# oval-group/GNN_branching

Measured on NVIDIA B200. Metric: gnn_subdomains_scored_per_sec, higher is better.
Workload: dtype fp16x3 (fp32 accumulate)

## Files before the change

gnn_branching_b200/csrc/gnnb_api.cu:

```cuda
#include <math.h>
#include <stdio.h>
#include <stdlib.h>
#include <string.h>

#include <map>
#include <string>
#include <vector>

#include "gnnb_common.cuh"
#include "gnnb_train.cuh"

using namespace gnnb;

struct gnnb_ctx {
    int device = 0;
    int last_status = 0;
    std::string err;
    int64_t launches = 0;
    int math = GNNB_MATH_TC_FP16X3;
    int chunk = 0;
    int snapshot = 0;
    int fuse = 1;
    int rescore = 0;
    int64_t rescored = 0;
    bool have_gnn = false;
    float* d_gnn = nullptr;
    uint16_t* d_tc = nullptr;
    GnnParams gp{};
    float* d_train = nullptr;
    int64_t n_params = 0;
    size_t po_w[N_LIN] = {0}, po_b[N_LIN] = {0};
    int adam_steps = 0;
    float* train_ws = nullptr;
    size_t train_ws_cap = 0;
    float* kw_ws = nullptr;
    size_t kw_ws_cap = 0;
    int32_t* kw_iscratch = nullptr;
    int kw_iscratch_cap = 0;
    bool have_net = false;
    float* d_net = nullptr;
    std::vector<LayerDev> layers;
    std::vector<PropPlan*> plan_fwd, plan_bwd;
    std::vector<PropPlan*> plan_kw_own;
    std::vector<PropPlan*> plan_kw;
    std::vector<int> n;
    int zero_tap_layer = 0;
    std::vector<LayerTiling> tiling;
    std::vector<RowMap> rowmap;
    int32_t* d_maps = nullptr;
    LayerDev* d_layers = nullptr;
    int32_t* d_hidden_off = nullptr;
    int32_t* d_random_order = nullptr;
    const float** d_ptrs = nullptr;
    std::vector<int> hidden_off;
    int n_hidden = 0;
    std::vector<struct gnnb_queue*> queues;
    int ws_cap = 0;
    bool ws_host_staging = false;
    float* d_ws = nullptr;
    std::vector<float*> mu, relax_f, relax_b;
    std::vector<int32_t*> amb_cnt, amb_base, amb_rows;
    float* nb = nullptr;
    float* ws_scores = nullptr;
    float* ws_best = nullptr;
    int32_t* ws_idx = nullptr;
    struct Staging {
        std::vector<float*> inputs;
        float* mask = nullptr;
        float* best = nullptr;
        int32_t* idx = nullptr;
        float* scores = nullptr;
    } stg[2];
    float* res_best = nullptr;
    int32_t* res_idx = nullptr;
    int64_t res_cap = 0;
    cudaStream_t copy_stream = nullptr;
    cudaEvent_t ev_copied[2] = {nullptr, nullptr}, ev_free[2] = {nullptr, nullptr};
    unsigned long long* d_nan = nullptr;
    int32_t* d_resc = nullptr;
    int resc_cap = 0;
    RowGather* d_gather = nullptr;
    size_t gather_cap = 0;
    std::map<std::string, std::pair<float*, int64_t>> snaps;
    int profile = 0;
    struct Pending { int klass; int64_t rows; cudaEvent_t a, b; };
    std::vector<Pending> pending;
    std::vector<cudaEvent_t> ev_pool;
    double prof_ms[GNNB_K_COUNT] = {0};
    int64_t prof_launches[GNNB_K_COUNT] = {0};
    int64_t prof_rows[GNNB_K_COUNT] = {0};
};

struct gnnb_queue {
    gnnb_ctx* ctx;
    DomainQueue* q;
};

namespace {

int fail(gnnb_ctx* c, int status, const std::string& msg) {
    if (c) { c->last_status = status; c->err = msg; }
    return status;
}

int axis_taps(int i, int ksize, int stride, int pad, int n_out) {
    int t = 0;
    for (int k = 0; k < ksize; ++k) {
        const int a = i + pad - k;
        if (a >= 0 && a % stride == 0 && a / stride < n_out) ++t;
    }
    return t;
}

int first_zero_tap_layer(const std::vector<LayerDev>& layers) {
    for (size_t k = 1; k < layers.size(); ++k) {
        const LayerDev& L = layers[k];
        if (L.kind != GNNB_LAYER_CONV) continue;
        for (int y = 0; y < L.h_in; ++y)
            if (axis_taps(y, L.ksize, L.stride, L.pad, L.h_out) == 0) return (int)k + 1;
        for (int x = 0; x < L.w_in; ++x)
            if (axis_taps(x, L.ksize, L.stride, L.pad, L.w_out) == 0) return (int)k + 1;
    }
    return 0;
}

int check_zero_taps(gnnb_ctx* c) {
    if (!c->zero_tap_layer) return GNNB_OK;
    return fail(c, GNNB_ERR_UNSUPPORTED, "layer " + std::to_string(c->zero_tap_layer) +
                " (conv, stride > kernel) has input positions no tap reaches: the GNN's tap-count normalisation divides by zero");
}

template <class F>
void walk_inputs(const gnnb_frontier& fr, GnnInputs& in, const std::vector<int>& n, F f) {
    const int L = (int)n.size() - 2;
    auto at = [](const float* const* table, int k) { return table ? table[k] : nullptr; };
    for (int k = 0; k <= L + 1; ++k) {
        f(at(fr.lb, k), in.lb[k], (int64_t)n[k]);
        f(at(fr.ub, k), in.ub[k], (int64_t)n[k]);
    }
    for (int k = 0; k < L; ++k) {
        f(at(fr.dual, k), in.dual[k], (int64_t)n[k + 1] * 3);
        f(at(fr.prim_pre, k), in.pre[k], (int64_t)n[k + 1]);
        f(at(fr.prim_post, k), in.post[k], (int64_t)n[k + 1]);
    }
    f(fr.prim_out, in.pout, (int64_t)1);
    f(fr.primal_input, in.pin, (int64_t)n[0]);
    f(fr.wp, in.wp, (int64_t)n[L]);
    f(fr.bp, in.bp, (int64_t)1);
}

int frontier_inputs(gnnb_ctx* ctx, const gnnb_frontier* fr, bool mask, GnnInputs* out) {
    bool ok = !mask || fr->mask;
    walk_inputs(*fr, *out, ctx->n, [&](const float* src, const float*& slot, int64_t) { slot = src; ok = ok && src; });
    return ok ? GNNB_OK : fail(ctx, GNNB_ERR_INVALID, "null frontier array");
}

#define CU(call)                                                                                          \
    do {                                                                                                  \
        cudaError_t e__ = (call);                                                                         \
        if (e__ != cudaSuccess)                                                                           \
            return fail(ctx, GNNB_ERR_CUDA, std::string(#call) + ": " + cudaGetErrorString(e__));         \
    } while (0)

size_t align4(size_t x) { return (x + 3) & ~size_t(3); }

void free_workspace(gnnb_ctx* c) {
    if (c->d_ws) cudaFree(c->d_ws);
    c->d_ws = nullptr;
    c->ws_cap = 0;
    for (auto& kv : c->snaps) cudaFree(kv.second.first);
    c->snaps.clear();
}

int ensure_workspace(gnnb_ctx* ctx, int Bc, bool host_staging) {
    if (ctx->d_ws && ctx->ws_cap >= Bc && (ctx->ws_host_staging || !host_staging)) return GNNB_OK;
    free_workspace(ctx);
    const int L = (int)ctx->layers.size();
    int nmax = 0;
    for (int k = 0; k <= L; ++k) nmax = ctx->n[k] > nmax ? ctx->n[k] : nmax;
    size_t total = 0;
    auto take = [&](size_t elems) { size_t off = total; total += (elems + 63) & ~size_t(63); return off; };
    std::vector<size_t> o_mu(L + 2), o_rf(L + 1), o_rb(L + 1), o_lb(L + 2), o_ub(L + 2), o_du(L), o_pr(L), o_po(L);
    auto wrows = [&](int k) { return (size_t)Bc * (k <= L ? (size_t)ctx->rowmap[k].nslots : 128); };
    for (int k = 0; k <= L + 1; ++k) o_mu[k] = take(wrows(k) * P);
    for (int k = 1; k <= L; ++k) { o_rf[k] = take(wrows(k) * P); o_rb[k] = take(wrows(k) * P); }
    std::vector<size_t> o_ac(L + 1), o_ab(L + 1), o_ar(L + 1);
    for (int k = 1; k <= L; ++k) {
        const size_t rows = wrows(k), nt = rows / 128;
        o_ac[k] = take(nt + 1); o_ab[k] = take(nt + 1); o_ar[k] = take(rows);
    }
    size_t nb_rows = 0;
    for (int k = 0; k <= L; ++k) nb_rows = wrows(k) > nb_rows ? wrows(k) : nb_rows;
    const size_t o_nb = take(nb_rows * P);
    const size_t o_sc = take((size_t)Bc * ctx->n_hidden);
    const size_t o_best = take(Bc), o_idx = take(Bc);
    struct StgOff { std::vector<size_t> inputs; size_t mask, best, idx, sc; } so[2];
    if (host_staging) {
        GnnInputs unused(L);
        for (StgOff& o : so) {
            walk_inputs(gnnb_frontier{}, unused, ctx->n, [&](const float*, const float*&, int64_t per) {
                o.inputs.push_back(take((size_t)Bc * per));
            });
            o.mask = take((size_t)Bc * ctx->n_hidden);
            o.best = take((size_t)Bc * GNNB_TOPK_MAX); o.idx = take((size_t)Bc * GNNB_TOPK_MAX);
            o.sc = take((size_t)Bc * ctx->n_hidden);
        }
    }
    CU(cudaMalloc(&ctx->d_ws, total * sizeof(float)));
    float* base = ctx->d_ws;
    ctx->mu.assign(L + 2, nullptr); ctx->relax_f.assign(L + 1, nullptr); ctx->relax_b.assign(L + 1, nullptr);
    for (int k = 0; k <= L + 1; ++k) ctx->mu[k] = base + o_mu[k];
    for (int k = 1; k <= L; ++k) { ctx->relax_f[k] = base + o_rf[k]; ctx->relax_b[k] = base + o_rb[k]; }
    ctx->amb_cnt.assign(L + 1, nullptr); ctx->amb_base.assign(L + 1, nullptr); ctx->amb_rows.assign(L + 1, nullptr);
    for (int k = 1; k <= L; ++k) {
        ctx->amb_cnt[k] = reinterpret_cast<int32_t*>(base + o_ac[k]);
        ctx->amb_base[k] = reinterpret_cast<int32_t*>(base + o_ab[k]);
        ctx->amb_rows[k] = reinterpret_cast<int32_t*>(base + o_ar[k]);
    }
    ctx->nb = base + o_nb; ctx->ws_scores = base + o_sc; ctx->ws_best = base + o_best;
    ctx->ws_idx = reinterpret_cast<int32_t*>(base + o_idx);
    if (host_staging) {
        for (int i = 0; i < 2; ++i) {
            gnnb_ctx::Staging& g = ctx->stg[i];
            const StgOff& o = so[i];
            g.inputs.clear();
            for (size_t off : o.inputs) g.inputs.push_back(base + off);
            g.mask = base + o.mask;
            g.best = base + o.best; g.idx = reinterpret_cast<int32_t*>(base + o.idx); g.scores = base + o.sc;
        }
        if (!ctx->copy_stream) {
            CU(cudaStreamCreateWithFlags(&ctx->copy_stream, cudaStreamNonBlocking));
            for (int i = 0; i < 2; ++i) {
                CU(cudaEventCreateWithFlags(&ctx->ev_copied[i], cudaEventDisableTiming));
                CU(cudaEventCreateWithFlags(&ctx->ev_free[i], cudaEventDisableTiming));
            }
        }
    }
    ctx->ws_cap = Bc;
    ctx->ws_host_staging = host_staging;
    return GNNB_OK;
}

#define TRY_(expr) do { int s__ = (expr); if (s__ != GNNB_OK) return s__; } while (0)

int snap(gnnb_ctx* ctx, bool on, const std::string& name, const float* src, int64_t numel, cudaStream_t st) {
    if (!on) return GNNB_OK;
    auto it = ctx->snaps.find(name);
    if (it == ctx->snaps.end() || it->second.second < numel) {
        if (it != ctx->snaps.end()) cudaFree(it->second.first);
        float* p = nullptr;
        CU(cudaMalloc(&p, (size_t)numel * sizeof(float)));
        ctx->snaps[name] = std::make_pair(p, numel);
        it = ctx->snaps.find(name);
    }
    it->second.second = numel;
    CU(cudaMemcpyAsync(it->second.first, src, (size_t)numel * sizeof(float), cudaMemcpyDeviceToDevice, st));
    return GNNB_OK;
}

cudaEvent_t prof_event(gnnb_ctx* ctx) {
    if (!ctx->ev_pool.empty()) { cudaEvent_t e = ctx->ev_pool.back(); ctx->ev_pool.pop_back(); return e; }
    cudaEvent_t e = nullptr;
    cudaEventCreate(&e);
    return e;
}

struct ProfScope {
    gnnb_ctx* ctx; cudaStream_t st; cudaEvent_t a = nullptr, b = nullptr; int klass; int64_t rows;
    ProfScope(gnnb_ctx* c, int k, int64_t r, cudaStream_t s) : ctx(c), st(s), klass(k), rows(r) {
        if (ctx->profile) { a = prof_event(ctx); b = prof_event(ctx); cudaEventRecord(a, st); }
    }
    ~ProfScope() {
        if (ctx->profile) { cudaEventRecord(b, st); ctx->pending.push_back({klass, rows, a, b}); }
    }
};

int prof_collect(gnnb_ctx* ctx) {
    if (ctx->pending.empty()) return GNNB_OK;
    CU(cudaDeviceSynchronize());
    for (auto& p : ctx->pending) {
        float ms = 0.f;
        if (cudaEventElapsedTime(&ms, p.a, p.b) == cudaSuccess) {
            ctx->prof_ms[p.klass] += ms;
            ctx->prof_launches[p.klass] += 1;
            ctx->prof_rows[p.klass] += p.rows;
        }
        ctx->ev_pool.push_back(p.a);
        ctx->ev_pool.push_back(p.b);
    }
    ctx->pending.clear();
    return GNNB_OK;
}

int snap_img(gnnb_ctx* ctx, bool on, const std::string& name, const float* img, int k, int Bc, bool piece_major, cudaStream_t st) {
    if (!on) return GNNB_OK;
    const int64_t numel = (int64_t)Bc * ctx->n[k] * P;
    if (ctx->math != GNNB_MATH_TC_FP16X3) return snap(ctx, on, name, img, numel, st);
    TRY_(snap(ctx, on, name, img, numel, st));
    tc_unpack_tile_image(img, ctx->snaps[name].first, ctx->rowmap[k], (int64_t)Bc * ctx->rowmap[k].nslots, piece_major, st);
    return GNNB_OK;
}

#define TRY(expr) do { int s__ = (expr); if (s__ != GNNB_OK) return s__; } while (0)

int run_chunk(gnnb_ctx* ctx, const GnnInputs& in, const float* mask, int Bc, int math, const NanDoms& nd, float* scores, int k,
              float* best_score, int32_t* best_idx, gnnb_winner* winners, cudaStream_t st) {
    const int L = (int)ctx->layers.size();
    const GnnParams& g = ctx->gp;
    const bool tc = math == GNNB_MATH_TC_FP16X3;
    const bool snaps = ctx->snapshot && math == ctx->math;
    int64_t* lc = &ctx->launches;
    auto name = [](const char* fmt, int a, int b) { char buf[64]; snprintf(buf, sizeof buf, fmt, a, b); return std::string(buf); };

    auto R = [&](int k) { return (int64_t)Bc * (tc ? ctx->rowmap[k].nslots : ctx->n[k]); };
    const RowMap nomap{nullptr, 0, 0};
    auto M = [&](int k) { return tc ? ctx->rowmap[k] : nomap; };
    const bool fused = tc && ctx->fuse;

    const bool amb_all = tc && L <= AMB_MAX_LAYERS;
    if (amb_all) {
        ProfScope ps(ctx, GNNB_K_RELAX, 0, st);
        AmbLayers al{};
        al.n = L;
        for (int k = 1; k <= L; ++k) {
            al.lb[k - 1] = in.lb[k]; al.ub[k - 1] = in.ub[k]; al.map[k - 1] = M(k); al.rows[k - 1] = R(k);
            al.cnt[k - 1] = ctx->amb_cnt[k]; al.base[k - 1] = ctx->amb_base[k]; al.out_rows[k - 1] = ctx->amb_rows[k];
        }
        amb_compact_all(al, st, lc);
    }
    {
        std::vector<NodeInputs> nis(L + 1);
        for (int k = 1; k <= L; ++k)
            nis[k] = NodeInputs{in.lb[k], in.ub[k], in.dual[k - 1], in.pre[k - 1], in.post[k - 1], ctx->layers[k - 1].bias_node,
                                ctx->n[k], R(k), ctx->amb_rows[k], ctx->amb_base[k], M(k)};
        if (tc) {
            for (int k0 = 1; k0 <= L; k0 += AMB_MAX_LAYERS) {
                const int nl = (L - k0 + 1) < AMB_MAX_LAYERS ? (L - k0 + 1) : AMB_MAX_LAYERS;
                int64_t nodes = 0;
                for (int k = k0; k < k0 + nl; ++k) {
                    nodes += (int64_t)Bc * ctx->n[k];
                    if (!amb_all) amb_compact(in.lb[k], in.ub[k], M(k), nis[k].rows, ctx->amb_cnt[k], ctx->amb_base[k], ctx->amb_rows[k], st, lc);
                }
                ProfScope ps(ctx, GNNB_K_RELAX, nodes, st);
                tc_relax(g, &nis[k0], &ctx->relax_f[k0], &ctx->relax_b[k0], nl, st, lc);
            }
        }
        for (int k = 1; k <= L; ++k) {
            if (!tc) {
                ProfScope ps(ctx, GNNB_K_RELAX, (int64_t)Bc * ctx->n[k], st);
                simt_relax(g, nis[k], ctx->relax_f[k], ctx->relax_b[k], st, lc);
            }
            TRY(snap(ctx, snaps, name(tc ? "relaxp_f%d" : "relax_f%d", k, 0), ctx->relax_f[k], (int64_t)Bc * ctx->n[k] * P, st));
            TRY(snap(ctx, snaps, name(tc ? "relaxp_b%d" : "relax_b%d", k, 0), ctx->relax_b[k], (int64_t)Bc * ctx->n[k] * P, st));
        }
    }
    {
        ProfScope ps(ctx, GNNB_K_INPUT_EMBED, (int64_t)Bc * ctx->n[0], st);
        if (tc) tc_input_embed(g, in.lb[0], in.pin, in.ub[0], ctx->mu[0], M(0), R(0), st, lc);
        else simt_input_embed(g, in.lb[0], in.pin, in.ub[0], ctx->mu[0], R(0), st, lc);
    }
    TRY(snap_img(ctx, snaps, "mu0_embed", ctx->mu[0], 0, Bc, false, st));

    for (int t = 0; t < g.T; ++t) {
        const bool last = (t == g.T - 1);
        for (int k = 1; k <= L; ++k) {
            const int64_t rows = R(k), nodes = (int64_t)Bc * ctx->n[k];
            if (fused) {
                ProfScope ps(ctx, GNNB_K_LAYER_FWD, nodes, st);
                tc_fused(g, ctx->plan_fwd[k - 1], ctx->mu[k - 1], false, in.lb[k], in.ub[k], ctx->relax_f[k], ctx->amb_base[k],
                         ctx->mu[k], nullptr, M(k), 0, 0, rows, ctx->d_nan, nd, ctx->snapshot ? ctx->nb : nullptr, false, st, lc);
            } else {
                ProfScope ps(ctx, GNNB_K_PROP_FWD, nodes, st);
                if (tc) prop_tc_run(ctx->plan_fwd[k - 1], ctx->mu[k - 1], ctx->nb, Bc, st, lc);
                else prop_forward(ctx->layers[k - 1], ctx->mu[k - 1], ctx->nb, Bc, st, lc);
            }
            TRY(snap_img(ctx, snaps, name("t%d_fwd_nb%d", t, k), ctx->nb, k, Bc, true, st));
            if (!fused) {
                ProfScope ps(ctx, GNNB_K_UPDATE_FWD, nodes, st);
                if (tc) tc_update(g, false, in.lb[k], in.ub[k], ctx->nb, ctx->relax_f[k], ctx->amb_base[k], ctx->mu[k], nullptr, M(k), 0, 0, rows, ctx->d_nan, nd, st, lc);
                else simt_update(g, false, in.lb[k], in.ub[k], ctx->nb, ctx->relax_f[k], ctx->mu[k], nullptr, ctx->n[k], 0, 0, rows, ctx->d_nan, st, lc);
            }
            TRY(snap_img(ctx, snaps, name("t%d_fwd_mu%d", t, k), ctx->mu[k], k, Bc, false, st));
        }
        {
            ProfScope ps(ctx, GNNB_K_OUTPUT, Bc, st);
            output_node(g, in.wp, in.bp, ctx->mu[L], tc, tc ? ctx->rowmap[L].nslots : ctx->n[L], in.lb[L + 1], in.ub[L + 1], in.pout,
                        ctx->mu[L + 1], ctx->n[L], Bc, st, lc);
        }
        TRY(snap(ctx, snaps, name("t%d_mu_out", t, 0), ctx->mu[L + 1], (int64_t)Bc * P, st));
        for (int k = L; k >= 1; --k) {
            const int64_t rows = R(k), nodes = (int64_t)Bc * ctx->n[k];
            float* sc = last ? scores : nullptr;
            float* mu_k = (last && k == 1 && tc && !ctx->snapshot) ? nullptr : ctx->mu[k];
            const bool fused_k = fused && k < L;
            if (fused_k) {
                ProfScope ps(ctx, last ? GNNB_K_LAYER_BWD_SCORE : GNNB_K_LAYER_BWD, nodes, st);
                tc_fused(g, ctx->plan_bwd[k], ctx->mu[k + 1], true, in.lb[k], in.ub[k], ctx->relax_b[k], ctx->amb_base[k],
                         mu_k, sc, M(k), ctx->n_hidden, ctx->hidden_off[k], rows, ctx->d_nan, nd, ctx->snapshot ? ctx->nb : nullptr, false, st, lc);
            } else {
                ProfScope ps(ctx, GNNB_K_PROP_BWD, nodes, st);
                if (k == L && tc) prop_tc_property_backward(in.wp, ctx->mu[L + 1], ctx->nb, ctx->n[L], ctx->rowmap[L].nslots, Bc, st, lc);
                else if (k == L) prop_property_backward(in.wp, ctx->mu[L + 1], ctx->nb, ctx->n[L], Bc, st, lc);
                else if (tc) prop_tc_run(ctx->plan_bwd[k], ctx->mu[k + 1], ctx->nb, Bc, st, lc);
                else prop_backward(ctx->layers[k], ctx->mu[k + 1], ctx->nb, Bc, true, st, lc);
            }
            TRY(snap_img(ctx, snaps, name("t%d_bwd_nb%d", t, k), ctx->nb, k, Bc, true, st));
            if (!fused_k) {
                ProfScope ps(ctx, last ? GNNB_K_UPDATE_BWD_SCORE : GNNB_K_UPDATE_BWD, nodes, st);
                if (tc) tc_update(g, true, in.lb[k], in.ub[k], ctx->nb, ctx->relax_b[k], ctx->amb_base[k], mu_k, sc, M(k), ctx->n_hidden, ctx->hidden_off[k], rows, ctx->d_nan, nd, st, lc);
                else simt_update(g, true, in.lb[k], in.ub[k], ctx->nb, ctx->relax_b[k], ctx->mu[k], sc, ctx->n[k], ctx->n_hidden, ctx->hidden_off[k], rows, ctx->d_nan, st, lc);
            }
            TRY(snap_img(ctx, snaps, name("t%d_bwd_mu%d", t, k), ctx->mu[k], k, Bc, false, st));
        }
        if (!last && fused) {
            ProfScope ps(ctx, GNNB_K_INPUT_UPDATE, (int64_t)Bc * ctx->n[0], st);
            tc_fused(g, ctx->plan_bwd[0], ctx->mu[1], true, in.lb[0], in.ub[0], nullptr, nullptr, ctx->mu[0], nullptr, M(0), 0, 0, R(0),
                     ctx->d_nan, nd, nullptr, true, st, lc);
            TRY(snap_img(ctx, snaps, name("t%d_mu0", t, 0), ctx->mu[0], 0, Bc, false, st));
        } else if (!last) {
            {
                ProfScope ps(ctx, GNNB_K_PROP_BWD, (int64_t)Bc * ctx->n[0], st);
                if (tc) prop_tc_run(ctx->plan_bwd[0], ctx->mu[1], ctx->nb, Bc, st, lc);
                else prop_backward(ctx->layers[0], ctx->mu[1], ctx->nb, Bc, false, st, lc);
            }
            {
                ProfScope ps(ctx, GNNB_K_INPUT_UPDATE, (int64_t)Bc * ctx->n[0], st);
                if (tc) tc_input_update(g, in.lb[0], in.ub[0], ctx->nb, ctx->mu[0], M(0), R(0), st, lc);
                else simt_input_update(g, in.lb[0], in.ub[0], ctx->nb, ctx->mu[0], R(0), st, lc);
            }
            TRY(snap_img(ctx, snaps, name("t%d_mu0", t, 0), ctx->mu[0], 0, Bc, false, st));
        }
    }
    {
        ProfScope ps(ctx, GNNB_K_ARGMAX, Bc, st);
        if (k == 1) masked_argmax(scores, mask, ctx->n_hidden, Bc, best_score, best_idx, winners, st, lc);
        else masked_topk(scores, mask, ctx->n_hidden, Bc, k, best_score, best_idx, st, lc);
    }
    CU(cudaGetLastError());
    return GNNB_OK;
}

int ensure_nan_doms(gnnb_ctx* ctx, int B) {
    if (ctx->resc_cap >= B) return GNNB_OK;
    if (ctx->d_resc) { cudaFree(ctx->d_resc); ctx->d_resc = nullptr; ctx->resc_cap = 0; }
    CU(cudaMalloc(&ctx->d_resc, (1 + 2 * (size_t)B) * sizeof(int32_t)));
    CU(cudaMemset(ctx->d_resc, 0, (1 + 2 * (size_t)B) * sizeof(int32_t)));
    ctx->resc_cap = B;
    return GNNB_OK;
}

int ensure_kw_iscratch(gnnb_ctx* ctx, int B, cudaStream_t st) {
    if (ctx->kw_iscratch_cap >= B) return GNNB_OK;
    if (ctx->kw_iscratch) { CU(cudaStreamSynchronize(st)); cudaFree(ctx->kw_iscratch); ctx->kw_iscratch = nullptr; ctx->kw_iscratch_cap = 0; }
    CU(cudaMalloc(&ctx->kw_iscratch, (3 * (size_t)B + 1) * sizeof(int32_t)));
    ctx->kw_iscratch_cap = B;
    return GNNB_OK;
}

NanDoms nan_doms(gnnb_ctx* ctx) { return NanDoms{ctx->d_resc, ctx->d_resc + 1, ctx->d_resc + 1 + ctx->resc_cap, 0}; }

void reset_nan_doms(gnnb_ctx* ctx, cudaStream_t st) {
    cudaStreamSynchronize(st);
    cudaMemset(ctx->d_resc, 0, (1 + 2 * (size_t)ctx->resc_cap) * sizeof(int32_t));
}

int rescore_flagged(gnnb_ctx* ctx, const gnnb_frontier* in, int chunk, int k, float* best, int32_t* idx, gnnb_winner* winners,
                    float* scores, cudaStream_t st) {
    const bool host = in->mem == GNNB_MEM_HOST;
    const int nh = ctx->n_hidden;
    const NanDoms nd = nan_doms(ctx);
    int32_t count = 0;
    CU(cudaMemcpyAsync(&count, nd.count, sizeof count, cudaMemcpyDeviceToHost, st));
    CU(cudaStreamSynchronize(st));
    ctx->rescored = count;
    if (count == 0) return GNNB_OK;
    std::vector<int32_t> rows;
    if (host) {
        rows.resize(count);
        CU(cudaMemcpyAsync(rows.data(), nd.list, (size_t)count * sizeof(int32_t), cudaMemcpyDeviceToHost, st));
        CU(cudaStreamSynchronize(st));
    }
    CU(cudaMemsetAsync(nd.count, 0, sizeof(int32_t), st));
    CU(cudaMemsetAsync(ctx->d_nan, 0, sizeof(unsigned long long), st));
    gnnb_ctx::Staging& sg = ctx->stg[0];
    std::vector<RowGather> tab;
    GnnInputs cp((int)ctx->layers.size());
    walk_inputs(*in, cp, ctx->n, [&](const float* src, const float*& slot, int64_t per) {
        float* dst = sg.inputs[tab.size()];
        tab.push_back(RowGather{src, dst, per});
        slot = dst;
    });
    tab.push_back(RowGather{in->mask, sg.mask, nh});
    if (!host) {
        if (ctx->gather_cap < tab.size()) {
            if (ctx->d_gather) cudaFree(ctx->d_gather);
            ctx->d_gather = nullptr; ctx->gather_cap = 0;
            CU(cudaMalloc(&ctx->d_gather, tab.size() * sizeof(RowGather)));
            ctx->gather_cap = tab.size();
        }
        CU(cudaMemcpyAsync(ctx->d_gather, tab.data(), tab.size() * sizeof(RowGather), cudaMemcpyHostToDevice, st));
    }
    for (int s0 = 0, Bs = 0; s0 < count; s0 += Bs) {
        Bs = (count - s0) < chunk ? (count - s0) : chunk;
        if (host) {
            for (int i = 0; i < Bs; ++i)
                for (const RowGather& t : tab)
                    CU(cudaMemcpyAsync(t.dst + i * t.per, t.src + rows[s0 + i] * t.per, t.per * sizeof(float), cudaMemcpyHostToDevice, st));
        } else {
            gather_rows(ctx->d_gather, (int)tab.size(), nd.list + s0, Bs, st, &ctx->launches);
        }
        TRY(run_chunk(ctx, cp, sg.mask, Bs, GNNB_MATH_SIMT_FP32, NanDoms{nullptr, nullptr, nullptr, 0}, sg.scores, k, sg.best, sg.idx, nullptr, st));
        scatter_rescored(nd.list + s0, Bs, k, sg.best, sg.idx, sg.scores, nh, best, idx, winners, host ? nullptr : scores, nd.flag, st,
                         &ctx->launches);
        if (host && scores)
            for (int i = 0; i < Bs; ++i)
                CU(cudaMemcpyAsync(scores + (size_t)rows[s0 + i] * nh, sg.scores + (size_t)i * nh, (size_t)nh * sizeof(float),
                                   cudaMemcpyDeviceToHost, st));
    }
    CU(cudaEventRecord(ctx->ev_free[0], st));
    CU(cudaGetLastError());
    return GNNB_OK;
}

int upload_gnn(gnnb_ctx* ctx, const float* const* tensors, int T) {
    std::vector<size_t> o_w(N_LIN), o_b(N_LIN);
    size_t total = 0;
    for (int l = 0; l < N_LIN; ++l) {
        o_w[l] = total; total += align4((size_t)lin_in(l) * lin_out(l));
        o_b[l] = total; total += align4(lin_out(l));
    }
    std::vector<float> blob(total, 0.f);
    for (int l = 0; l < N_LIN; ++l) {
        const int K = lin_in(l), N = lin_out(l);
        const float* W = tensors[2 * l];
        for (int nn = 0; nn < N; ++nn)
            for (int k = 0; k < K; ++k) blob[o_w[l] + (size_t)k * N + nn] = W[(size_t)nn * K + k];
        memcpy(&blob[o_b[l]], tensors[2 * l + 1], sizeof(float) * N);
    }
    std::vector<float> cw((size_t)N_TCLIN * P * P, 0.f), cb((size_t)N_TCLIN * P, 0.f);
    auto compose = [&](int id, int outer, int half, int inner, bool add_outer_bias) {
        const float* Wo = tensors[2 * outer];
        const float* bo = tensors[2 * outer + 1];
        const int Ko = lin_in(outer);
        for (int nn = 0; nn < P; ++nn) {
            double bacc = add_outer_bias ? (double)bo[nn] : 0.0;
            for (int k = 0; k < P; ++k) {
                double acc = 0.0;
                if (inner < 0) acc = Wo[(size_t)nn * Ko + half * P + k];
                else
                    for (int j = 0; j < P; ++j) acc += (double)Wo[(size_t)nn * Ko + half * P + j] * (double)tensors[2 * inner][(size_t)j * P + k];
                cw[((size_t)id * P + nn) * P + k] = (float)acc;
            }
            if (inner >= 0)
                for (int j = 0; j < P; ++j) bacc += (double)Wo[(size_t)nn * Ko + half * P + j] * (double)tensors[2 * inner + 1][j];
            cb[(size_t)id * P + nn] = (float)bacc;
        }
    };
    compose(T_FWD_R, FC4, 0, FC1_1, false);
    compose(T_FWD_C, FC4, 1, FC3_2, true);
    compose(T_BWD_R, BC4, 0, BC2_1, false);
    compose(T_BWD_C, BC4, 1, BC3_1, true);
    compose(T_INP_C, INP_B2, 0, INP_B_1, true);
    compose(T_INP_NB, INP_B2, 1, -1, false);
    std::vector<size_t> o_tc(N_LIN, 0);
    size_t tc_total = 0;
    for (int l = 0; l < N_LIN; ++l)
        if (lin_in(l) >= P && lin_out(l) == P) { o_tc[l] = tc_total; tc_total += (size_t)tc_packed_elems(lin_in(l)); }
    std::vector<size_t> o_tcx(N_TCLIN, 0);
    for (int i = 0; i < N_TCLIN; ++i) { o_tcx[i] = tc_total; tc_total += (size_t)tc_packed_elems(P); }
    std::vector<uint16_t> tcblob(tc_total ? tc_total : 1, 0);
    for (int l = 0; l < N_LIN; ++l)
        if (lin_in(l) >= P && lin_out(l) == P) tc_pack_weight(tensors[2 * l], lin_in(l), &tcblob[o_tc[l]]);
    for (int i = 0; i < N_TCLIN; ++i) tc_pack_weight(&cw[(size_t)i * P * P], P, &tcblob[o_tcx[i]]);
    const size_t o_cb = total;
    total += cb.size();
    blob.resize(total, 0.f);
    memcpy(&blob[o_cb], cb.data(), cb.size() * sizeof(float));
    CU(cudaDeviceSynchronize());
    if (!ctx->d_gnn) CU(cudaMalloc(&ctx->d_gnn, total * sizeof(float)));
    if (!ctx->d_tc) CU(cudaMalloc(&ctx->d_tc, tcblob.size() * sizeof(uint16_t)));
    CU(cudaMemcpy(ctx->d_gnn, blob.data(), total * sizeof(float), cudaMemcpyHostToDevice));
    CU(cudaMemcpy(ctx->d_tc, tcblob.data(), tcblob.size() * sizeof(uint16_t), cudaMemcpyHostToDevice));
    for (int l = 0; l < N_LIN; ++l) {
        ctx->gp.wt[l] = ctx->d_gnn + o_w[l];
        ctx->gp.bias[l] = ctx->d_gnn + o_b[l];
        ctx->gp.tc[l] = (lin_in(l) >= P && lin_out(l) == P) ? ctx->d_tc + o_tc[l] : nullptr;
    }
    for (int i = 0; i < N_TCLIN; ++i) {
        ctx->gp.tcx_w[i] = ctx->d_tc + o_tcx[i];
        ctx->gp.tcx_b[i] = ctx->d_gnn + o_cb + (size_t)i * P;
    }
    ctx->gp.T = T;
    if (!ctx->d_train) {
        size_t np = 0;
        for (int l = 0; l < N_LIN; ++l) {
            ctx->po_w[l] = np; np += align4((size_t)lin_in(l) * lin_out(l));
            ctx->po_b[l] = np; np += align4(lin_out(l));
        }
        ctx->n_params = (int64_t)np;
        CU(cudaMalloc(&ctx->d_train, 4 * np * sizeof(float)));
        CU(cudaMemset(ctx->d_train, 0, 4 * np * sizeof(float)));
        ctx->adam_steps = 0;
    }
    {
        std::vector<float> master((size_t)ctx->n_params, 0.f);
        for (int l = 0; l < N_LIN; ++l) {
            memcpy(&master[ctx->po_w[l]], tensors[2 * l], sizeof(float) * lin_in(l) * lin_out(l));
            memcpy(&master[ctx->po_b[l]], tensors[2 * l + 1], sizeof(float) * lin_out(l));
        }
        CU(cudaMemcpy(ctx->d_train, master.data(), master.size() * sizeof(float), cudaMemcpyHostToDevice));
    }
    ctx->have_gnn = true;
    return GNNB_OK;
}

TrainParams train_params(gnnb_ctx* ctx) {
    TrainParams tp;
    float* grad = ctx->d_train + ctx->n_params;
    for (int l = 0; l < N_LIN; ++l) {
        tp.w[l] = ctx->d_train + ctx->po_w[l]; tp.b[l] = ctx->d_train + ctx->po_b[l];
        tp.dw[l] = grad + ctx->po_w[l]; tp.db[l] = grad + ctx->po_b[l];
    }
    return tp;
}

int download_quarter(gnnb_ctx* ctx, int quarter, float* const* tensors, const int64_t* numels, int n_tensors) {
    if (!ctx || !tensors || !numels) return fail(ctx, GNNB_ERR_INVALID, "null argument");
    if (!ctx->have_gnn) return fail(ctx, GNNB_ERR_STATE, "gnnb_set_gnn_weights must be called first");
    if (n_tensors != 2 * N_LIN) return fail(ctx, GNNB_ERR_INVALID, "expected 52 tensors (weight, bias of 26 linears)");
    for (int l = 0; l < N_LIN; ++l)
        if (numels[2 * l] != (int64_t)lin_in(l) * lin_out(l) || numels[2 * l + 1] != lin_out(l))
            return fail(ctx, GNNB_ERR_INVALID, "tensor " + std::to_string(2 * l) + " has the wrong number of elements");
    CU(cudaSetDevice(ctx->device));
    CU(cudaDeviceSynchronize());
    std::vector<float> host((size_t)ctx->n_params);
    CU(cudaMemcpy(host.data(), ctx->d_train + (size_t)quarter * ctx->n_params, host.size() * sizeof(float), cudaMemcpyDeviceToHost));
    for (int l = 0; l < N_LIN; ++l) {
        memcpy(tensors[2 * l], &host[ctx->po_w[l]], sizeof(float) * lin_in(l) * lin_out(l));
        memcpy(tensors[2 * l + 1], &host[ctx->po_b[l]], sizeof(float) * lin_out(l));
    }
    return GNNB_OK;
}

}

extern "C" {

int gnnb_abi_version(void) { return 1; }

int gnnb_create(gnnb_ctx** out, int device) {
    if (!out) return GNNB_ERR_INVALID;
    *out = nullptr;
    gnnb_ctx* ctx = new gnnb_ctx();
    ctx->device = device;
    cudaError_t e = cudaSetDevice(device);
    if (e != cudaSuccess) { delete ctx; return GNNB_ERR_CUDA; }
    cudaDeviceProp prop;
    e = cudaGetDeviceProperties(&prop, device);
    if (e != cudaSuccess) { delete ctx; return GNNB_ERR_CUDA; }
    if (prop.major != 10) {
        fprintf(stderr, "libgnnb: device %d is sm_%d%d; this library is built for sm_100a (B200) only\n", device, prop.major, prop.minor);
        delete ctx;
        return GNNB_ERR_UNSUPPORTED;
    }
    if (cudaMalloc(&ctx->d_nan, sizeof(unsigned long long)) != cudaSuccess ||
        cudaMemset(ctx->d_nan, 0, sizeof(unsigned long long)) != cudaSuccess ||
        simt_init() != 0 || prop_init(64 * 1024) != 0 || tc_init() != 0 || prop_tc_init() != 0 || kw_init() != 0 || train_init() != 0) {
        fprintf(stderr, "libgnnb: initialisation failed: %s\n", cudaGetErrorString(cudaGetLastError()));
        if (ctx->d_nan) cudaFree(ctx->d_nan);
        delete ctx;
        return GNNB_ERR_CUDA;
    }
    *out = ctx;
    return GNNB_OK;
}

void gnnb_destroy(gnnb_ctx* ctx) {
    if (!ctx) return;
    cudaSetDevice(ctx->device);
    free_workspace(ctx);
    if (ctx->d_gnn) cudaFree(ctx->d_gnn);
    if (ctx->d_tc) cudaFree(ctx->d_tc);
    if (ctx->d_train) cudaFree(ctx->d_train);
    if (ctx->train_ws) cudaFree(ctx->train_ws);
    if (ctx->kw_ws) cudaFree(ctx->kw_ws);
    if (ctx->kw_iscratch) cudaFree(ctx->kw_iscratch);
    if (ctx->d_net) cudaFree(ctx->d_net);
    if (ctx->d_maps) cudaFree(ctx->d_maps);
    if (ctx->d_layers) cudaFree(ctx->d_layers);
    if (ctx->d_hidden_off) cudaFree(ctx->d_hidden_off);
    if (ctx->d_random_order) cudaFree(ctx->d_random_order);
    if (ctx->d_ptrs) cudaFree(ctx->d_ptrs);
    if (ctx->d_nan) cudaFree(ctx->d_nan);
    if (ctx->d_resc) cudaFree(ctx->d_resc);
    if (ctx->d_gather) cudaFree(ctx->d_gather);
    for (PropPlan* p : ctx->plan_fwd) prop_plan_free(p);
    for (PropPlan* p : ctx->plan_bwd) prop_plan_free(p);
    for (PropPlan* p : ctx->plan_kw_own) prop_plan_free(p);
    if (ctx->copy_stream) cudaStreamDestroy(ctx->copy_stream);
    if (ctx->res_best) cudaFree(ctx->res_best);
    if (ctx->res_idx) cudaFree(ctx->res_idx);
    for (int i = 0; i < 2; ++i) { if (ctx->ev_copied[i]) cudaEventDestroy(ctx->ev_copied[i]); if (ctx->ev_free[i]) cudaEventDestroy(ctx->ev_free[i]); }
    for (auto& p : ctx->pending) { cudaEventDestroy(p.a); cudaEventDestroy(p.b); }
    for (auto e : ctx->ev_pool) cudaEventDestroy(e);
    for (gnnb_queue* q : ctx->queues) q->ctx = nullptr;
    delete ctx;
}

int gnnb_set_gnn_weights(gnnb_ctx* ctx, const float* const* tensors, const int64_t* numels, int n_tensors, int T, int p) {
    if (!ctx || !tensors || !numels) return fail(ctx, GNNB_ERR_INVALID, "null argument");
    if (p != P) return fail(ctx, GNNB_ERR_UNSUPPORTED, "embedding size p must be 64");
    if (T < 1) return fail(ctx, GNNB_ERR_INVALID, "T must be >= 1");
    if (n_tensors != 2 * N_LIN) return fail(ctx, GNNB_ERR_INVALID, "expected 52 tensors (weight, bias of 26 linears)");
    for (int l = 0; l < N_LIN; ++l) {
        if (numels[2 * l] != (int64_t)lin_in(l) * lin_out(l) || numels[2 * l + 1] != lin_out(l))
            return fail(ctx, GNNB_ERR_INVALID, "tensor " + std::to_string(2 * l) + " has the wrong number of elements");
    }
    CU(cudaSetDevice(ctx->device));
    return upload_gnn(ctx, tensors, T);
}

int gnnb_set_network(gnnb_ctx* ctx, const gnnb_layer_desc* layers, int n_layers, int c0, int h0, int w0) {
    if (!ctx || !layers || n_layers < 1) return fail(ctx, GNNB_ERR_INVALID, "null argument");
    if (!ctx->queues.empty()) return fail(ctx, GNNB_ERR_STATE, "gnnb_set_network while domain queues of the previous network exist");
    CU(cudaSetDevice(ctx->device));
    std::vector<LayerDev> devs(n_layers);
    std::vector<int> n(n_layers + 2);
    n[0] = c0 * h0 * w0;
    int pc = c0, ph = h0, pw = w0;
    bool flat = false;
    size_t total = 0;
    std::vector<size_t> o_w(n_layers), o_b(n_layers);
    for (int k = 0; k < n_layers; ++k) {
        const gnnb_layer_desc& d = layers[k];
        LayerDev& L = devs[k];
        L.kind = d.kind;
        L.c_in = d.c_in; L.h_in = d.h_in; L.w_in = d.w_in; L.c_out = d.c_out; L.h_out = d.h_out; L.w_out = d.w_out;
        L.ksize = d.ksize; L.stride = d.stride; L.pad = d.pad;
        L.n_in = d.c_in * d.h_in * d.w_in;
        L.n_out = d.c_out * d.h_out * d.w_out;
        if (!d.weight || !d.bias) return fail(ctx, GNNB_ERR_INVALID, "layer weight/bias is null");
        if (L.n_in != n[k]) return fail(ctx, GNNB_ERR_INVALID, "layer " + std::to_string(k) + ": input size does not match the previous layer");
        size_t wn;
        if (d.kind == GNNB_LAYER_CONV) {
            if (flat || d.c_in != pc || d.h_in != ph || d.w_in != pw) return fail(ctx, GNNB_ERR_INVALID, "conv layer input shape mismatch");
            if (d.ksize < 1 || d.stride < 1 || d.pad < 0) return fail(ctx, GNNB_ERR_INVALID, "bad conv geometry");
            if (d.h_out != (d.h_in + 2 * d.pad - d.ksize) / d.stride + 1 || d.w_out != (d.w_in + 2 * d.pad - d.ksize) / d.stride + 1)
                return fail(ctx, GNNB_ERR_INVALID, "conv output shape mismatch");
            if ((d.h_out - 1) * d.stride - 2 * d.pad + d.ksize != d.h_in || (d.w_out - 1) * d.stride - 2 * d.pad + d.ksize != d.w_in)
                return fail(ctx, GNNB_ERR_UNSUPPORTED, "conv geometry needs output_padding in the backward pass");
            if ((size_t)d.c_in * d.ksize * d.ksize * d.c_out * sizeof(float) > 64 * 1024)
                return fail(ctx, GNNB_ERR_UNSUPPORTED, "conv weights exceed the 64 KB shared-memory staging buffer");
            wn = (size_t)d.c_out * d.c_in * d.ksize * d.ksize;
            pc = d.c_out; ph = d.h_out; pw = d.w_out;
        } else if (d.kind == GNNB_LAYER_LINEAR) {
            if (d.h_in != 1 || d.w_in != 1 || d.h_out != 1 || d.w_out != 1) return fail(ctx, GNNB_ERR_INVALID, "linear layers use c_in/c_out only");
            wn = (size_t)L.n_out * L.n_in;
            flat = true;
        } else {
            return fail(ctx, GNNB_ERR_INVALID, "unknown layer kind");
        }
        n[k + 1] = L.n_out;
        o_w[k] = total; total += align4(wn);
        o_b[k] = total; total += align4(L.n_out);
    }
    n[n_layers + 1] = 1;
    std::vector<float> blob(total, 0.f);
    for (int k = 0; k < n_layers; ++k) {
        const gnnb_layer_desc& d = layers[k];
        const LayerDev& L = devs[k];
        const size_t wn = d.kind == GNNB_LAYER_CONV ? (size_t)d.c_out * d.c_in * d.ksize * d.ksize : (size_t)L.n_out * L.n_in;
        memcpy(&blob[o_w[k]], d.weight, wn * sizeof(float));
        const int per = d.kind == GNNB_LAYER_CONV ? d.h_out * d.w_out : 1;
        for (int j = 0; j < L.n_out; ++j) blob[o_b[k] + j] = d.bias[j / per];
    }
    struct Staged {
        float* d_net = nullptr;
        int32_t* d_maps = nullptr;
        LayerDev* d_layers = nullptr;
        int32_t *d_hidden_off = nullptr, *d_random_order = nullptr;
        const float** d_ptrs = nullptr;
        std::vector<PropPlan*> plan_fwd, plan_bwd, plan_kw_own;
        bool keep = false;
        ~Staged() {
            if (keep) return;
            if (d_net) cudaFree(d_net);
            if (d_maps) cudaFree(d_maps);
            if (d_layers) cudaFree(d_layers);
            if (d_hidden_off) cudaFree(d_hidden_off);
            if (d_random_order) cudaFree(d_random_order);
            if (d_ptrs) cudaFree(d_ptrs);
            for (PropPlan* p : plan_fwd) prop_plan_free(p);
            for (PropPlan* p : plan_bwd) prop_plan_free(p);
            for (PropPlan* p : plan_kw_own) prop_plan_free(p);
        }
    } sg;
    CU(cudaMalloc(&sg.d_net, total * sizeof(float)));
    CU(cudaMemcpy(sg.d_net, blob.data(), total * sizeof(float), cudaMemcpyHostToDevice));
    for (int k = 0; k < n_layers; ++k) { devs[k].weight = sg.d_net + o_w[k]; devs[k].bias_node = sg.d_net + o_b[k]; }
    sg.plan_fwd.assign(n_layers, nullptr);
    sg.plan_bwd.assign(n_layers, nullptr);
    sg.plan_kw_own.assign(n_layers, nullptr);
    std::vector<LayerTiling> tiling(n_layers + 1);
    std::vector<RowMap> rowmap(n_layers + 1, RowMap{nullptr, 0, 0});
    tiling[0] = make_tiling(c0, h0, w0);
    for (int k = 0; k < n_layers; ++k)
        tiling[k + 1] = devs[k].kind == GNNB_LAYER_CONV ? make_tiling(devs[k].c_out, devs[k].h_out, devs[k].w_out)
                                                       : make_tiling(devs[k].n_out, 1, 1);
    {
        size_t total_slots = 0;
        for (const LayerTiling& t : tiling) total_slots += t.node_of_slot.size();
        CU(cudaMalloc(&sg.d_maps, total_slots * sizeof(int32_t)));
        size_t off = 0;
        for (int k = 0; k <= n_layers; ++k) {
            const LayerTiling& t = tiling[k];
            CU(cudaMemcpy(sg.d_maps + off, t.node_of_slot.data(), t.node_of_slot.size() * sizeof(int32_t), cudaMemcpyHostToDevice));
            rowmap[k] = RowMap{sg.d_maps + off, n[k], (int)t.node_of_slot.size()};
            off += t.node_of_slot.size();
        }
    }
    for (int k = 0; k < n_layers; ++k) {
        sg.plan_fwd[k] = prop_plan_build(devs[k], layers[k].weight, false, false, tiling[k + 1], tiling[k]);
        sg.plan_bwd[k] = prop_plan_build(devs[k], layers[k].weight, true, k > 0, tiling[k], tiling[k + 1]);
        if (!sg.plan_fwd[k] || !sg.plan_bwd[k]) return fail(ctx, GNNB_ERR_CUDA, "building the propagation plans failed");
        if (k > 0 && devs[k].kind == GNNB_LAYER_CONV) {
            sg.plan_kw_own[k] = prop_plan_build(devs[k], layers[k].weight, true, false, tiling[k], tiling[k + 1]);
            if (!sg.plan_kw_own[k]) return fail(ctx, GNNB_ERR_CUDA, "building the propagation plans failed");
        }
    }
    std::vector<int> hidden_off(n_layers + 2, 0);
    int n_hidden = 0;
    for (int k = 1; k <= n_layers; ++k) { hidden_off[k] = n_hidden; n_hidden += n[k]; }
    CU(cudaMalloc(&sg.d_layers, n_layers * sizeof(LayerDev)));
    CU(cudaMemcpy(sg.d_layers, devs.data(), n_layers * sizeof(LayerDev), cudaMemcpyHostToDevice));
    CU(cudaMalloc(&sg.d_hidden_off, (n_layers + 1) * sizeof(int32_t)));
    CU(cudaMemcpy(sg.d_hidden_off, hidden_off.data() + 1, (n_layers + 1) * sizeof(int32_t), cudaMemcpyHostToDevice));
    CU(cudaMalloc(&sg.d_random_order, n_layers * sizeof(int32_t)));
    CU(cudaMalloc(&sg.d_ptrs, 2 * (n_layers + 2) * sizeof(float*)));
    CU(cudaDeviceSynchronize());
    ctx->have_net = false;
    free_workspace(ctx);
    if (ctx->d_net) cudaFree(ctx->d_net);
    if (ctx->d_maps) cudaFree(ctx->d_maps);
    if (ctx->d_layers) cudaFree(ctx->d_layers);
    if (ctx->d_hidden_off) cudaFree(ctx->d_hidden_off);
    if (ctx->d_random_order) cudaFree(ctx->d_random_order);
    if (ctx->d_ptrs) cudaFree(ctx->d_ptrs);
    for (PropPlan* p : ctx->plan_fwd) prop_plan_free(p);
    for (PropPlan* p : ctx->plan_bwd) prop_plan_free(p);
    for (PropPlan* p : ctx->plan_kw_own) prop_plan_free(p);
    sg.keep = true;
    ctx->d_net = sg.d_net; ctx->d_maps = sg.d_maps; ctx->d_layers = sg.d_layers; ctx->d_hidden_off = sg.d_hidden_off;
    ctx->d_random_order = sg.d_random_order; ctx->d_ptrs = sg.d_ptrs;
    ctx->plan_fwd = sg.plan_fwd; ctx->plan_bwd = sg.plan_bwd; ctx->plan_kw_own = sg.plan_kw_own;
    ctx->plan_kw.assign(n_layers, nullptr);
    for (int k = 0; k < n_layers; ++k) ctx->plan_kw[k] = sg.plan_kw_own[k] ? sg.plan_kw_own[k] : sg.plan_bwd[k];
    ctx->tiling = tiling; ctx->rowmap = rowmap;
    ctx->layers = devs;
    ctx->n = n;
    ctx->zero_tap_layer = first_zero_tap_layer(devs);
    ctx->hidden_off = hidden_off;
    ctx->n_hidden = n_hidden;
    ctx->have_net = true;
    return GNNB_OK;
}

int gnnb_set_option(gnnb_ctx* ctx, const char* key, int64_t value) {
    if (!ctx || !key) return fail(ctx, GNNB_ERR_INVALID, "null argument");
    const std::string k(key);
    if (k == "math") {
        if (value != GNNB_MATH_TC_FP16X3 && value != GNNB_MATH_SIMT_FP32) return fail(ctx, GNNB_ERR_INVALID, "unknown math mode");
        if (value == GNNB_MATH_TC_FP16X3 && !tc_available()) return fail(ctx, GNNB_ERR_UNSUPPORTED, "tensor-core path not built");
        ctx->math = (int)value;
    } else if (k == "chunk") {
        if (value < 0) return fail(ctx, GNNB_ERR_INVALID, "chunk must be >= 0");
        ctx->chunk = (int)value;
    } else if (k == "fuse") {
        ctx->fuse = value ? 1 : 0;
    } else if (k == "snapshot") {
        ctx->snapshot = value ? 1 : 0;
    } else if (k == "profile") {
        ctx->profile = value ? 1 : 0;
    } else if (k == "rescore") {
        ctx->rescore = value ? 1 : 0;
    } else {
        return fail(ctx, GNNB_ERR_INVALID, "unknown option " + k);
    }
    return GNNB_OK;
}

int64_t gnnb_get_option(gnnb_ctx* ctx, const char* key) {
    if (!ctx || !key) return -1;
    const std::string k(key);
    if (k == "math") return ctx->math;
    if (k == "chunk") return ctx->chunk;
    if (k == "snapshot") return ctx->snapshot;
    if (k == "fuse") return ctx->fuse;
    if (k == "profile") return ctx->profile;
    if (k == "rescore") return ctx->rescore;
    if (k == "rescored") return ctx->rescored;
    if (k == "n_hidden") return ctx->n_hidden;
    if (k == "workspace_domains") return ctx->ws_cap;
    if (k.rfind("plan_density_pct_", 0) == 0) {
        const bool bwd = k[17] == 'b';
        const size_t i = (size_t)atoi(k.c_str() + 18);
        const auto& v = bwd ? ctx->plan_bwd : ctx->plan_fwd;
        return i < v.size() ? (int64_t)(100.0 * prop_plan_density(v[i])) : -1;
    }
    return -1;
}

static int score_impl(gnnb_ctx* ctx, const gnnb_frontier* in, int k, float* best_score, int32_t* best_idx, gnnb_winner* winners,
                      float* scores, void* stream) {
    if (!ctx || !in || ((!best_score || !best_idx) && !winners)) return fail(ctx, GNNB_ERR_INVALID, "null argument");
    if (!ctx->have_gnn || !ctx->have_net) return fail(ctx, GNNB_ERR_STATE, "gnnb_set_gnn_weights and gnnb_set_network must be called first");
    if (in->B < 0) return fail(ctx, GNNB_ERR_INVALID, "negative batch");
    ctx->rescored = 0;
    TRY(check_zero_taps(ctx));
    if (in->B == 0) return GNNB_OK;
    GnnInputs cp((int)ctx->layers.size());
    TRY(frontier_inputs(ctx, in, true, &cp));
    CU(cudaSetDevice(ctx->device));
    cudaStream_t st = (cudaStream_t)stream;
    const bool host = in->mem == GNNB_MEM_HOST;
    int chunk = ctx->chunk > 0 ? ctx->chunk : 1024;
    if (chunk > in->B) chunk = in->B;
    const bool resc = ctx->rescore && ctx->math == GNNB_MATH_TC_FP16X3;
    TRY(ensure_workspace(ctx, chunk, host || resc));
    NanDoms nd{nullptr, nullptr, nullptr, 0};
    if (resc) {
        TRY(ensure_nan_doms(ctx, in->B));
        nd = nan_doms(ctx);
    }
    const int64_t n_res = (int64_t)in->B * k;
    if (host && !winners && ctx->res_cap < n_res) {
        if (ctx->res_best) cudaFree(ctx->res_best);
        if (ctx->res_idx) cudaFree(ctx->res_idx);
        ctx->res_best = nullptr; ctx->res_idx = nullptr; ctx->res_cap = 0;
        CU(cudaMalloc(&ctx->res_best, (size_t)n_res * sizeof(float)));
        CU(cudaMalloc(&ctx->res_idx, (size_t)n_res * sizeof(int32_t)));
        ctx->res_cap = n_res;
    }

    int wave = 0, ramp = host ? (chunk < 128 ? chunk : 128) : chunk;
    for (int c0 = 0, Bc = 0; c0 < in->B; c0 += Bc, ++wave) {
        Bc = (in->B - c0) < ramp ? (in->B - c0) : ramp;
        ramp = ramp + ramp / 2 > chunk ? chunk : ramp + ramp / 2;
        gnnb_ctx::Staging& sg = ctx->stg[wave & 1];
        cudaStream_t cs = host ? ctx->copy_stream : st;
        if (host) CU(cudaStreamWaitEvent(cs, ctx->ev_free[wave & 1], 0));
        auto stage = [&](const float* src, float* dst, size_t per_domain) -> const float* {
            const float* p = src + (size_t)c0 * per_domain;
            if (!host) return p;
            cudaMemcpyAsync(dst, p, (size_t)Bc * per_domain * sizeof(float), cudaMemcpyHostToDevice, cs);
            return dst;
        };
        size_t a = 0;
        walk_inputs(*in, cp, ctx->n, [&](const float* src, const float*& slot, int64_t per) {
            slot = stage(src, host ? sg.inputs[a++] : nullptr, per);
        });
        const float* mask = stage(in->mask, sg.mask, ctx->n_hidden);
        CU(cudaGetLastError());
        if (host) {
            CU(cudaEventRecord(ctx->ev_copied[wave & 1], cs));
            CU(cudaStreamWaitEvent(st, ctx->ev_copied[wave & 1], 0));
        }

        float* d_scores = host ? sg.scores : (scores ? scores + (size_t)c0 * ctx->n_hidden : ctx->ws_scores);
        float* d_best = winners ? nullptr : (host ? ctx->res_best : best_score) + (size_t)c0 * k;
        int32_t* d_idx = winners ? nullptr : (host ? ctx->res_idx : best_idx) + (size_t)c0 * k;
        {
            nd.dom0 = c0;
            const int rc = run_chunk(ctx, cp, mask, Bc, ctx->math, nd, d_scores, k, d_best, d_idx, winners ? winners + c0 : nullptr, st);
            if (rc != GNNB_OK) {
                if (host) cudaStreamSynchronize(ctx->copy_stream);
                cudaStreamSynchronize(st);
                if (resc) reset_nan_doms(ctx, st);
                return rc;
            }
        }
        if (host) {
            if (scores)
                CU(cudaMemcpyAsync(scores + (size_t)c0 * ctx->n_hidden, d_scores, (size_t)Bc * ctx->n_hidden * sizeof(float),
                                   cudaMemcpyDeviceToHost, st));
            CU(cudaEventRecord(ctx->ev_free[wave & 1], st));
        }
    }
    if (resc) {
        const int rc = rescore_flagged(ctx, in, chunk, k, winners ? nullptr : (host ? ctx->res_best : best_score),
                                       winners ? nullptr : (host ? ctx->res_idx : best_idx), winners, scores, st);
        if (rc != GNNB_OK) {
            reset_nan_doms(ctx, st);
            return rc;
        }
    }
    if (host) {
        if (!winners) {
            CU(cudaMemcpyAsync(best_score, ctx->res_best, (size_t)n_res * sizeof(float), cudaMemcpyDeviceToHost, st));
            CU(cudaMemcpyAsync(best_idx, ctx->res_idx, (size_t)n_res * sizeof(int32_t), cudaMemcpyDeviceToHost, st));
        }
        return gnnb_check(ctx, stream, nullptr);
    }
    return GNNB_OK;
}

int gnnb_score(gnnb_ctx* ctx, const gnnb_frontier* in, float* best_score, int32_t* best_idx, float* scores, void* stream) {
    if (!best_score || !best_idx) return fail(ctx, GNNB_ERR_INVALID, "null argument");
    return score_impl(ctx, in, 1, best_score, best_idx, nullptr, scores, stream);
}

int gnnb_score_winners(gnnb_ctx* ctx, const gnnb_frontier* in, gnnb_winner* winners, float* scores, void* stream) {
    if (!winners) return fail(ctx, GNNB_ERR_INVALID, "null argument");
    if (in && in->mem == GNNB_MEM_HOST && scores) return fail(ctx, GNNB_ERR_INVALID, "dense scores of a HOST frontier: use gnnb_score");
    return score_impl(ctx, in, 1, nullptr, nullptr, winners, scores, stream);
}

int gnnb_score_topk(gnnb_ctx* ctx, const gnnb_frontier* in, int32_t k, float* top_score, int32_t* top_idx, float* scores, void* stream) {
    if (k < 1 || k > GNNB_TOPK_MAX) return fail(ctx, GNNB_ERR_INVALID, "k must be in [1, GNNB_TOPK_MAX]");
    if (!top_score || !top_idx) return fail(ctx, GNNB_ERR_INVALID, "null argument");
    return score_impl(ctx, in, k, top_score, top_idx, nullptr, scores, stream);
}

int gnnb_topk(gnnb_ctx* ctx, int32_t B, int32_t n, const float* scores, const float* mask, int32_t k, float* top_score,
              int32_t* top_idx, void* stream) {
    if (!ctx) return GNNB_ERR_INVALID;
    if (k < 1 || k > GNNB_TOPK_MAX) return fail(ctx, GNNB_ERR_INVALID, "k must be in [1, GNNB_TOPK_MAX]");
    if (!scores || !top_score || !top_idx) return fail(ctx, GNNB_ERR_INVALID, "null argument");
    if (B < 0 || n < 0) return fail(ctx, GNNB_ERR_INVALID, "negative size");
    if (B == 0) return GNNB_OK;
    CU(cudaSetDevice(ctx->device));
    cudaStream_t st = (cudaStream_t)stream;
    {
        ProfScope ps(ctx, GNNB_K_ARGMAX, B, st);
        masked_topk(scores, mask, n, B, k, top_score, top_idx, st, &ctx->launches);
    }
    CU(cudaGetLastError());
    return GNNB_OK;
}

int gnnb_babsr(gnnb_ctx* ctx, const gnnb_frontier* in, int32_t sparsest_layer, float decision_threshold,
               const int32_t* random_order, const int32_t* icp_counter_in, int32_t* decision, int32_t* icp_counter_out,
               int32_t* kind, float* scores, void* stream) {
    if (!ctx || !in || !random_order || !decision || !icp_counter_out) return fail(ctx, GNNB_ERR_INVALID, "null argument");
    if (!ctx->have_net) return fail(ctx, GNNB_ERR_STATE, "gnnb_set_network must be called first");
    if (in->B < 0) return fail(ctx, GNNB_ERR_INVALID, "negative batch");
    if (in->B == 0) return GNNB_OK;
    if (!in->lb || !in->ub || !in->wp || !in->mask) return fail(ctx, GNNB_ERR_INVALID, "null frontier field");
    const int L = (int)ctx->layers.size(), B = in->B;
    if (L > babsr_max_layers()) return fail(ctx, GNNB_ERR_UNSUPPORTED, "too many layers for the BaBSR kernel");
    CU(cudaSetDevice(ctx->device));
    cudaStream_t st = (cudaStream_t)stream;
    const bool host = in->mem == GNNB_MEM_HOST;
    const std::vector<int>& n = ctx->n;
    int nmax = 0;
    for (int k = 0; k <= L; ++k) nmax = n[k] > nmax ? n[k] : nmax;
    float* tmp = nullptr;
    std::vector<const float*> ptrs(2 * (L + 2), nullptr);
    const float *d_wp = in->wp, *d_mask = in->mask;
    const int32_t* d_cin = icp_counter_in;
    int32_t *d_dec = decision, *d_cout = icp_counter_out, *d_kind = kind;
    float* d_scores = scores;
    if (host) {
        size_t total = 0;
        auto take = [&](size_t elems) { size_t o = total; total += align4(elems); return o; };
        std::vector<size_t> o_lb(L + 2), o_ub(L + 2);
        for (int k = 1; k <= L; ++k) { o_lb[k] = take((size_t)B * n[k]); o_ub[k] = take((size_t)B * n[k]); }
        const size_t o_wp = take((size_t)B * n[L]), o_mask = take((size_t)B * ctx->n_hidden), o_cin = take(B), o_dec = take(2 * (size_t)B),
                     o_cout = take(B), o_kind = take(B), o_sc = take(scores ? (size_t)B * ctx->n_hidden : 0);
        CU(cudaMalloc(&tmp, total * sizeof(float)));
        auto up = [&](size_t off, const void* src, size_t elems) {
            cudaMemcpyAsync(tmp + off, src, elems * sizeof(float), cudaMemcpyHostToDevice, st);
            return tmp + off;
        };
        for (int k = 1; k <= L; ++k) {
            if (!in->lb[k] || !in->ub[k]) { cudaFree(tmp); return fail(ctx, GNNB_ERR_INVALID, "null bound array"); }
            ptrs[k] = up(o_lb[k], in->lb[k], (size_t)B * n[k]);
            ptrs[L + 2 + k] = up(o_ub[k], in->ub[k], (size_t)B * n[k]);
        }
        d_wp = up(o_wp, in->wp, (size_t)B * n[L]);
        d_mask = up(o_mask, in->mask, (size_t)B * ctx->n_hidden);
        d_cin = icp_counter_in ? reinterpret_cast<const int32_t*>(up(o_cin, icp_counter_in, B)) : nullptr;
        d_dec = reinterpret_cast<int32_t*>(tmp + o_dec); d_cout = reinterpret_cast<int32_t*>(tmp + o_cout);
        d_kind = kind ? reinterpret_cast<int32_t*>(tmp + o_kind) : nullptr;
        d_scores = scores ? tmp + o_sc : nullptr;
    } else {
        for (int k = 1; k <= L; ++k) {
            if (!in->lb[k] || !in->ub[k]) return fail(ctx, GNNB_ERR_INVALID, "null bound array");
            ptrs[k] = in->lb[k];
            ptrs[L + 2 + k] = in->ub[k];
        }
    }
    cudaError_t e = cudaMemcpyAsync(ctx->d_ptrs, ptrs.data(), ptrs.size() * sizeof(float*), cudaMemcpyHostToDevice, st);
    if (e == cudaSuccess) e = cudaMemcpyAsync(ctx->d_random_order, random_order, L * sizeof(int32_t), cudaMemcpyHostToDevice, st);
    int rc = 0;
    if (e == cudaSuccess)
        rc = babsr_run(ctx->d_layers, L, ctx->n_hidden, nmax, ctx->d_ptrs, ctx->d_ptrs + (L + 2), d_wp, d_mask, ctx->d_hidden_off,
                       ctx->d_random_order, d_cin, sparsest_layer, decision_threshold, d_dec, d_cout, d_kind, d_scores, B, st,
                       &ctx->launches);
    if (e == cudaSuccess && rc == 0 && host) {
        cudaMemcpyAsync(decision, d_dec, 2 * (size_t)B * sizeof(int32_t), cudaMemcpyDeviceToHost, st);
        cudaMemcpyAsync(icp_counter_out, d_cout, (size_t)B * sizeof(int32_t), cudaMemcpyDeviceToHost, st);
        if (kind) cudaMemcpyAsync(kind, d_kind, (size_t)B * sizeof(int32_t), cudaMemcpyDeviceToHost, st);
        if (scores) cudaMemcpyAsync(scores, d_scores, (size_t)B * ctx->n_hidden * sizeof(float), cudaMemcpyDeviceToHost, st);
        e = cudaStreamSynchronize(st);
    }
    if (tmp) { cudaStreamSynchronize(st); cudaFree(tmp); }
    if (e != cudaSuccess) return fail(ctx, GNNB_ERR_CUDA, std::string("gnnb_babsr: ") + cudaGetErrorString(e));
    if (rc != 0) return fail(ctx, GNNB_ERR_UNSUPPORTED, "a layer is too large for the BaBSR kernel's shared-memory buffers");
    CU(cudaGetLastError());
    return GNNB_OK;
}

int gnnb_score_grad(gnnb_ctx* ctx, const gnnb_frontier* in, int32_t n_terms, const int32_t* term_domain, const int32_t* term_index,
                    const float* term_coeff, float* term_scores, void* stream) {
    if (!ctx || !in || !term_domain || !term_index || !term_coeff) return fail(ctx, GNNB_ERR_INVALID, "null argument");
    if (!ctx->have_gnn || !ctx->have_net) return fail(ctx, GNNB_ERR_STATE, "gnnb_set_gnn_weights and gnnb_set_network must be called first");
    if (in->B < 1 || n_terms < 1) return fail(ctx, GNNB_ERR_INVALID, "need at least one subdomain and one term");
    TRY(check_zero_taps(ctx));
    GnnInputs ti((int)ctx->layers.size());
    TRY(frontier_inputs(ctx, in, false, &ti));
    for (int i = 0; i < n_terms; ++i)
        if (term_domain[i] < 0 || term_domain[i] >= in->B || term_index[i] < 0 || term_index[i] >= ctx->n_hidden)
            return fail(ctx, GNNB_ERR_INVALID, "term " + std::to_string(i) + " is out of range");
    CU(cudaSetDevice(ctx->device));
    cudaStream_t st = (cudaStream_t)stream;
    const int B = in->B;
    float* tmp = nullptr;
    if (in->mem == GNNB_MEM_HOST) {
        size_t total = 0;
        walk_inputs(*in, ti, ctx->n, [&](const float*, const float*&, int64_t per) { total += align4((size_t)B * per); });
        CU(cudaMalloc(&tmp, total * sizeof(float)));
        float* dst = tmp;
        walk_inputs(*in, ti, ctx->n, [&](const float* src, const float*& slot, int64_t per) {
            cudaMemcpyAsync(dst, src, (size_t)B * per * sizeof(float), cudaMemcpyHostToDevice, st);
            slot = dst;
            dst += align4((size_t)B * per);
        });
    }
    cudaMemsetAsync(ctx->d_train + ctx->n_params, 0, (size_t)ctx->n_params * sizeof(float), st);
    std::string err;
    const int rc = train_backward(ctx->gp, train_params(ctx), ctx->layers, ctx->n, ctx->hidden_off, ti, B, n_terms, term_domain, term_index,
                                  term_coeff, term_scores, &ctx->train_ws, &ctx->train_ws_cap, st, &ctx->launches, &err);
    if (tmp) { cudaStreamSynchronize(st); cudaFree(tmp); }
    if (rc != GNNB_OK) return fail(ctx, rc, err);
    return GNNB_OK;
}

// ... 299 lines not shown
```

gnn_branching_b200/csrc/gnnb_common.cuh:

```cuda
#pragma once

#include <cuda_runtime.h>
#include <stdint.h>

#include <string>
#include <vector>

#include "../../include/gnnb.h"

namespace gnnb {

constexpr int P = 64;

enum Lin : int {
    INP_F = 0, INP_F_1, INP_B, INP_B_1, INP_B2, INP_B2_2, FC1, FC1_1, FC3, FC3_2, FC4, FC4_2,
    OUT1, OUT2, OUT3, BC1, BC1_1, BC1_2, BC2, BC2_1, BC3, BC3_1, BC4, BC4_1, FNODE, FSCORE, N_LIN
};

__host__ __device__ constexpr int lin_in(int l) {
    return l == INP_F ? 3 : l == INP_B ? 2 : (l == FC1 || l == BC1) ? 7 : l == OUT1 ? 4
         : (l == INP_B2 || l == FC3 || l == FC4 || l == OUT2 || l == BC3 || l == BC4) ? 2 * P
         : l == BC2 ? 3 * P : P;
}
__host__ __device__ constexpr int lin_out(int l) { return l == FSCORE ? 1 : P; }

enum TcLin : int {
    T_FWD_R = 0,
    T_FWD_C,
    T_BWD_R,
    T_BWD_C,
    T_INP_C,
    T_INP_NB,
    N_TCLIN
};

struct GnnParams {
    const float* wt[N_LIN];
    const float* bias[N_LIN];
    const uint16_t* tc[N_LIN];
    const uint16_t* tcx_w[N_TCLIN];
    const float* tcx_b[N_TCLIN];
    int T;
};

struct LayerDev {
    int kind;
    int c_in, h_in, w_in, c_out, h_out, w_out, ksize, stride, pad;
    int n_in, n_out;
    const float* weight;
    const float* bias_node;
};

struct RowMap {
    const int32_t* node_of_slot;
    int n;
    int nslots;
};
__device__ __forceinline__ int64_t natural_row(const RowMap& m, int64_t grow) {
    const int64_t b = grow / m.nslots;
    const int node = __ldg(m.node_of_slot + (grow - b * m.nslots));
    return node < 0 ? -1 : b * m.n + node;
}
struct LayerTiling {
    std::vector<int32_t> node_of_slot, slot_of_node;
    int ntiles = 0;
};
LayerTiling make_tiling(int C, int H, int W);

struct NodeInputs {
    const float* lb;
    const float* ub;
    const float* dual;
    const float* prim_pre;
    const float* prim_post;
    const float* bias_node;
    int n;
    int64_t rows;
    const int32_t* amb_rows;
    const int32_t* amb_base;
    RowMap map;
};

struct NanDoms {
    int32_t* count;
    int32_t* flag;
    int32_t* list;
    int dom0;
};

void simt_relax(const GnnParams& g, const NodeInputs& in, float* relax_f, float* relax_b, cudaStream_t st, int64_t* launches);
void simt_update(const GnnParams& g, bool backward, const float* lb, const float* ub, const float* nb, const float* relax,
                 float* mu_out, float* scores , int n, int64_t score_stride, int64_t score_off, int64_t rows,
                 unsigned long long* nan_count, cudaStream_t st, int64_t* launches);
void simt_input_embed(const GnnParams& g, const float* lb0, const float* x, const float* ub0, float* mu0, int64_t rows,
                      cudaStream_t st, int64_t* launches);
void simt_input_update(const GnnParams& g, const float* lb0, const float* ub0, const float* nb, float* mu0, int64_t rows,
                       cudaStream_t st, int64_t* launches);

int simt_init();

void tc_relax(const GnnParams& g, const NodeInputs* in, float* const* relax_f, float* const* relax_b, int n_layers, cudaStream_t st,
              int64_t* launches);
void tc_update(const GnnParams& g, bool backward, const float* lb, const float* ub, const float* nb, const float* relax,
               const int32_t* amb_base, float* mu_out, float* scores, RowMap map, int64_t score_stride, int64_t score_off, int64_t rows,
               unsigned long long* nan_count, const NanDoms& nan_doms, cudaStream_t st, int64_t* launches);
struct PropPlan;
void tc_fused(const GnnParams& g, const PropPlan* plan, const float* mu_in, bool backward, const float* lb, const float* ub,
              const float* relax, const int32_t* amb_base, float* mu_out, float* scores, RowMap map, int64_t score_stride, int64_t score_off,
              int64_t rows, unsigned long long* nan_count, const NanDoms& nan_doms, float* nb_dbg, bool input_layer, cudaStream_t st,
              int64_t* launches);
void amb_compact(const float* lb, const float* ub, RowMap map, int64_t rows, int32_t* cnt, int32_t* amb_base, int32_t* amb_rows,
                 cudaStream_t st, int64_t* launches);
constexpr int AMB_MAX_LAYERS = 16;
struct AmbLayers {
    const float* lb[AMB_MAX_LAYERS];
    const float* ub[AMB_MAX_LAYERS];
    RowMap map[AMB_MAX_LAYERS];
    int64_t rows[AMB_MAX_LAYERS];
    int32_t* cnt[AMB_MAX_LAYERS];
    int32_t* base[AMB_MAX_LAYERS];
    int32_t* out_rows[AMB_MAX_LAYERS];
    int tile0[AMB_MAX_LAYERS + 1];
    int n;
};
void amb_compact_all(AmbLayers a, cudaStream_t st, int64_t* launches);
void tc_input_embed(const GnnParams& g, const float* lb0, const float* x, const float* ub0, float* mu0, RowMap map, int64_t rows,
                    cudaStream_t st, int64_t* launches);
void tc_input_update(const GnnParams& g, const float* lb0, const float* ub0, const float* nb, float* mu0, RowMap map, int64_t rows,
                     cudaStream_t st, int64_t* launches);
int64_t tc_pack_weight(const float* w_host, int K, uint16_t* dst_host);
int64_t tc_packed_elems(int K);
int tc_init();
bool tc_available();
void tc_unpack_tile_image(const float* img, float* out, RowMap map, int64_t rows, bool piece_major, cudaStream_t st);

int prop_init(int max_smem_bytes);
void prop_forward(const LayerDev& L, const float* mu_prev, float* nb, int Bc, cudaStream_t st, int64_t* launches);
void prop_backward(const LayerDev& L, const float* mu_next, float* nb, int Bc, bool normalise, cudaStream_t st, int64_t* launches);
void prop_property_backward(const float* wp, const float* mu_out, float* nb, int nL, int Bc, cudaStream_t st, int64_t* launches);
void output_node(const GnnParams& g, const float* wp, const float* bp, const float* mu_L, bool mu_image, int mu_stride, const float* lb_out,
                 const float* ub_out, const float* prim_out, float* mu_out, int nL, int Bc, cudaStream_t st, int64_t* launches);
void masked_argmax(const float* scores, const float* mask, int n_hidden, int Bc, float* best_score, int32_t* best_idx,
                   gnnb_winner* winners, cudaStream_t st, int64_t* launches);
void masked_topk(const float* scores, const float* mask, int n, int Bc, int k, float* top_score, int32_t* top_idx, cudaStream_t st,
                 int64_t* launches);
struct RowGather { const float* src; float* dst; int64_t per; };
struct GnnInputs {
    std::vector<const float*> lb, ub;
    std::vector<const float*> dual, pre, post;
    const float *pout = nullptr, *pin = nullptr, *wp = nullptr, *bp = nullptr;
    explicit GnnInputs(int L) : lb(L + 2), ub(L + 2), dual(L), pre(L), post(L) {}
};
void gather_rows(const RowGather* tab, int n_arrays, const int32_t* rows, int n, cudaStream_t st, int64_t* launches);
void scatter_rescored(const int32_t* rows, int n, int k, const float* sub_best, const int32_t* sub_idx, const float* sub_scores,
                      int n_hidden, float* best_score, int32_t* best_idx, gnnb_winner* winners, float* scores, int32_t* flag,
                      cudaStream_t st, int64_t* launches);

struct PropPlan;
int prop_tc_init();
PropPlan* prop_plan_build(const LayerDev& L, const float* host_weight, bool backward, bool normalise, const LayerTiling& out,
                          const LayerTiling& in);
void prop_plan_free(PropPlan* p);
double prop_plan_density(const PropPlan* p);
void prop_tc_run(const PropPlan* plan, const float* mu_in, float* nb_img, int Bc, cudaStream_t st, int64_t* launches);
void prop_tc_property_backward(const float* wp, const float* mu_out, float* nb_img, int nL, int nslots, int Bc, cudaStream_t st, int64_t* launches);

int babsr_max_layers();
int babsr_run(const LayerDev* d_layers, int L, int n_hidden, int nmax, const float* const* d_lb, const float* const* d_ub,
              const float* wp, const float* mask, const int32_t* d_hidden_off, const int32_t* d_random_order,
              const int32_t* counter_in, int sparsest_layer, float threshold, int32_t* decision, int32_t* counter_out,
              int32_t* kind, float* scores, int B, cudaStream_t st, int64_t* launches);

struct DomainQueue;
int queue_create(int device, const std::vector<int>& n, int n_hidden, int64_t capacity, DomainQueue** out, std::string* err);
void queue_destroy(DomainQueue* q);
const std::string& queue_error(const DomainQueue* q);
int64_t queue_size(const DomainQueue* q);
int64_t queue_capacity(const DomainQueue* q);
int queue_global_lb(DomainQueue* q, float* out, cudaStream_t st);
int queue_add(DomainQueue* q, int B, const float* lower, const float* upper, const float* const* lb, const float* const* ub,
              const int8_t* mask, const int32_t* decision, const uint8_t* keep, int32_t* added, cudaStream_t st, int64_t* launches);
int queue_pick(DomainQueue* q, int max_B, float threshold, bool discard, int32_t* picked, float* lower, float* upper, float* const* lb,
               float* const* ub, int8_t* mask, int32_t* decision, cudaStream_t st, int64_t* launches);
int queue_prune(DomainQueue* q, float threshold, cudaStream_t st, int64_t* launches);
float* queue_stage(DomainQueue* q, size_t bytes);

struct KwTc { const std::vector<PropPlan*>* plans; const std::vector<RowMap>* maps; };
int kw_init();
int kw_bounds(const std::vector<LayerDev>& layers, const std::vector<int>& n, int B, const float* x, float eps, const float* wp, const float* bp,
              const float* const* prov_lb, const float* const* prov_ub, float* const* out_lb, float* const* out_ub, const KwTc* tc, float** ws,
              size_t* ws_cap, cudaStream_t st, int64_t* launches, std::string* err);
int child_bounds(const std::vector<LayerDev>& layers, const std::vector<int>& n, int B, const float* x, float eps, const float* wp, const float* bp,
                 const float* const* parent_lb, const float* const* parent_ub, const int32_t* dec_layer, const int32_t* dec_index,
                 const int32_t* choice, float* const* out_lb, float* const* out_ub, int8_t* const* out_mask, int32_t* second_pass,
                 int32_t* iscratch, const KwTc* tc, float** ws, size_t* ws_cap, cudaStream_t st, int64_t* launches, std::string* err);

int root_bounds(const std::vector<LayerDev>& layers, const std::vector<int>& n, int B, const float* x, float eps, const float* wp, const float* bp,
                float* const* out_lb, float* const* out_ub, int8_t* const* out_mask, int32_t* second_pass, int32_t* iscratch, const KwTc* tc,
                float** ws, size_t* ws_cap, cudaStream_t st, int64_t* launches, std::string* err);

struct Ratio { float r0, r1, beta, amb; };
__device__ __forceinline__ Ratio compute_ratio(float l, float u) {
    Ratio r;
    float lt = l - fmaxf(l, 0.0f);
    float ut = fmaxf(u, 0.0f);
    if (u != u) ut = u;
    if (l != l) lt = l;
    r.r0 = __fdiv_rn(ut, __fsub_rn(ut, lt));
    r.beta = __fmul_rn(__fmul_rn(-1.0f, lt), r.r0);
    r.amb = (r.beta > 0.0f) ? 1.0f : 0.0f;
    r.r1 = __fadd_rn(__fmul_rn(__fsub_rn(1.0f, __fmul_rn(2.0f, __fmul_rn(r.r0, r.amb))), r.amb), r.r0);
    return r;
}

}
```

gnn_branching_b200/csrc/gnnb_prop_tc.cu:

```cuda
#include <algorithm>
#include <functional>
#include <map>
#include <vector>

#include "gnnb_prop_body.cuh"
#include "gnnb_umma.cuh"

namespace gnnb {

using namespace tcx;

struct PropPlan {
    PropPlanDev dev{};
    void* blob = nullptr;
    int nksteps = 0;
    double density = 0.0;
};

namespace prop {

constexpr int PD = 4;
constexpr int W_STAGES = 3, B_STAGES = 4;
constexpr int CHUNK_KS = 4;
constexpr uint32_t W_KS = 8192;
// ... 113 lines not shown
                __syncwarp();
                if (++ws == W_STAGES) { ws = 0; wph ^= 1u; }
#ifdef GNNB_TRACE
                ++n_chunks;
#endif
            }
            if (elect_one()) umma_commit(smem_u32(&tail->acc_full[a]));
            __syncwarp();
        }
#ifdef GNNB_TRACE
        if (rank == 1 && lane == 0) printf("TRACE prop-mma: items %u chunks %d total %lld | wait acc_empty %lld, w_full %lld, b_full %lld\n", it, n_chunks,
                                           clock64() - t_all, t_acc, t_w, t_b);
#endif
    } else if (warp < EPI_WARP0) {
        const int g = warp - GATHER_WARP0;
        const unsigned char* mu_bytes = reinterpret_cast<const unsigned char*>(mu_img);
        uint32_t bs = 0, bph = 0;
#ifdef GNNB_TRACE
        long long g_wait = 0, g_all = clock64(), g0_;
#endif
        for (int64_t item = rank; item < nitems; item += nranks) {
            const int tile = (int)(item % plan.ntiles);
            const int d = (int)(item / plan.ntiles) * PD + g;
            const bool dom_ok = d < Bc;
            const int64_t drow = (int64_t)d * plan.nslots_in;
            const int ks0 = plan.tile_ks0[tile], ks1 = plan.tile_ks0[tile + 1];
            for (int ks = ks0; ks < ks1; ks += 2) {
                const int krow = ks * 16 + lane;
                const int idx = krow < ks1 * 16 ? __ldg(plan.ks_rows + krow) : -1;
#ifdef GNNB_TRACE
                g0_ = clock64();
#endif
                mbar_wait(smem_u32(&tail->b_empty[bs]), bph ^ 1u);
#ifdef GNNB_TRACE
                g_wait += clock64() - g0_;
#endif
                const uint32_t dst0 = b_ring + bs * B_STAGE_BYTES + (uint32_t)g * B_DOM_BYTES;
#pragma unroll
                for (int i = 0; i < 8; ++i) {
                    const int k = i * 4 + (lane >> 3);
                    const int node = __shfl_sync(0xffffffffu, idx, k);
                    const bool ok = dom_ok && node >= 0;
                    const int64_t grow = ok ? drow + node : 0;
                    const uint32_t r = (uint32_t)(grow & (TILE - 1));
                    const uint32_t jp = (uint32_t)(lane & 7);
                    const unsigned char* src = mu_bytes + (grow >> 7) * (int64_t)ABUF + (r >> 3) * 1024u + (r & 7u) * 128u + jp * 16u;
                    const uint32_t dst = dst0 + swz((uint32_t)k, jp ^ (r & 7u));
                    cp_async16(dst, src, ok);
                    cp_async16(dst + B_PLANE_BYTES, src + APLANE, ok);
                }
                cp_async_arrive(smem_u32(&tail->b_full[bs]));
                if (++bs == B_STAGES) { bs = 0; bph ^= 1u; }
            }
        }
#ifdef GNNB_TRACE
        if (rank == 1 && g == 0 && lane == 0) printf("TRACE prop-gather: total %lld, wait b_empty %lld\n", clock64() - g_all, g_wait);
#endif
    } else if (warp < EPI_WARP0 + 8) {
        const int ew = (warp - EPI_WARP0) >> 2;
        const int m = (warp & 3) * 32 + lane;
        const uint32_t tmem = tmem_base + ((uint32_t)((warp & 3) * 32) << 16) + (uint32_t)ew * 256u;
        const uint32_t full = smem_u32(&tail->acc_full[ew]), empty = smem_u32(&tail->acc_empty[ew]);
        uint32_t aph = 0, it = 0;
#ifdef GNNB_TRACE
        long long e_wait = 0, e_work = 0, e0_;
#endif
        for (int64_t item = rank; item < nitems; item += nranks, ++it) {
            if ((int)(it & 1u) != ew) continue;
            const int tile = (int)(item % plan.ntiles);
            const int d0 = (int)(item / plan.ntiles) * PD;
#ifdef GNNB_TRACE
            e0_ = clock64();
#endif
            mbar_wait(full, aph);
            aph ^= 1u;
            tc_fence_after();
#ifdef GNNB_TRACE
            e_wait += clock64() - e0_; e0_ = clock64();
#endif
#pragma unroll 1
            for (int dom = 0; dom < PD; ++dom) {
                if (d0 + dom >= Bc) break;
                unsigned char* img = reinterpret_cast<unsigned char*>(nb_img) +
                                     ((int64_t)(d0 + dom) * plan.ntiles + tile) * (int64_t)ABUF + (uint32_t)m * 16u;
#pragma unroll
                for (int q = 0; q < 4; ++q) {
                    float x[16];
                    tmem_ld16_sync(tmem + (uint32_t)(dom * 64 + q * 16), x);
#pragma unroll
                    for (int h = 0; h < 2; ++h) {
                        uint4 hi, lo;
                        split2(x[h * 8 + 0], x[h * 8 + 1], hi.x, lo.x);
                        split2(x[h * 8 + 2], x[h * 8 + 3], hi.y, lo.y);
                        split2(x[h * 8 + 4], x[h * 8 + 5], hi.z, lo.z);
                        split2(x[h * 8 + 6], x[h * 8 + 7], hi.w, lo.w);
                        const uint32_t off = (uint32_t)(q * 2 + h) * NB_PIECE;
                        *reinterpret_cast<uint4*>(img + off) = hi;
                        *reinterpret_cast<uint4*>(img + APLANE + off) = lo;
                    }
                }
            }
            tc_fence_before();
            mbar_arrive(empty);
#ifdef GNNB_TRACE
            e_work += clock64() - e0_;
#endif
        }
#ifdef GNNB_TRACE
        if (rank == 1 && m == 0) printf("TRACE prop-epi wg %d: wait acc_full %lld, work %lld\n", ew, e_wait, e_work);
#endif
    }
    tc_fence_before();
    __syncthreads();
    if (warp == 0) tmem_dealloc(tmem_base, 512);
}

struct Edge { int in; float w; };
using EdgeFn = std::function<void(int, std::vector<Edge>&)>;

std::vector<std::vector<int>> grid_tiles(int C, int H, int W) {
    const int Cb = std::min(C, TILE), Pp = std::max(1, TILE / Cb);
    int bestY = 1, bestX = 1;
    long bestTiles = -1;
    for (int Yb = 1; Yb <= std::min(H, Pp); ++Yb)
        for (int Xb = 1; Xb <= std::min(W, Pp / Yb); ++Xb) {
            const long tiles = (long)((H + Yb - 1) / Yb) * ((W + Xb - 1) / Xb);
            const bool better = bestTiles < 0 || tiles < bestTiles ||
                                (tiles == bestTiles && std::abs(Yb - Xb) < std::abs(bestY - bestX));
            if (better) { bestTiles = tiles; bestY = Yb; bestX = Xb; }
        }
    std::vector<std::vector<int>> tiles;
    for (int c0 = 0; c0 < C; c0 += Cb)
        for (int y0 = 0; y0 < H; y0 += bestY)
            for (int x0 = 0; x0 < W; x0 += bestX) {
                std::vector<int> rows;
                for (int c = c0; c < std::min(C, c0 + Cb); ++c)
                    for (int y = y0; y < std::min(H, y0 + bestY); ++y)
                        for (int x = x0; x < std::min(W, x0 + bestX); ++x) rows.push_back((c * H + y) * W + x);
                tiles.push_back(rows);
            }
    return tiles;
}

std::vector<std::vector<int>> range_tiles(int n) {
    std::vector<std::vector<int>> tiles;
    for (int r0 = 0; r0 < n; r0 += TILE) {
        std::vector<int> rows;
        for (int r = r0; r < std::min(n, r0 + TILE); ++r) rows.push_back(r);
        tiles.push_back(rows);
    }
    return tiles;
}

PropPlan* build_plan(const LayerTiling& out, const LayerTiling& in, const EdgeFn& edges) {
    std::vector<int32_t> tile_ks0, ks_rows;
    std::vector<uint16_t> ks_w;
    std::vector<Edge> ev;
    std::vector<float> dense;
    double useful = 0.0, issued = 0.0;
    for (int t = 0; t < out.ntiles; ++t) {
        const int32_t* rows = &out.node_of_slot[(size_t)t * TILE];
        std::vector<std::vector<Edge>> row_edges(TILE);
        std::map<int, int> col;
        for (int m = 0; m < TILE; ++m) {
            if (rows[m] < 0) continue;
            ev.clear();
            edges(rows[m], ev);
            for (Edge& e : ev) { e.in = in.slot_of_node[e.in]; col[e.in] = 0; }
            row_edges[m] = ev;
            useful += (double)ev.size();
        }
        int K = 0;
        for (auto& kv : col) kv.second = K++;
        dense.assign((size_t)TILE * K, 0.f);
        for (int m = 0; m < TILE; ++m)
            for (const Edge& e : row_edges[m]) dense[(size_t)m * K + col[e.in]] += e.w;
        const int nks = std::max(1, (K + 15) / 16);
        issued += 128.0 * 16.0 * nks;
        tile_ks0.push_back((int32_t)(ks_rows.size() / 16));
        const size_t r0 = ks_rows.size(), w0 = ks_w.size();
        ks_rows.resize(r0 + (size_t)nks * 16, -1);
        for (const auto& kv : col) ks_rows[r0 + kv.second] = kv.first;
        ks_w.resize(w0 + (size_t)nks * 4096, 0);
        for (int m = 0; m < TILE; ++m)
            for (int k = 0; k < K; ++k) {
                const float x = dense[(size_t)m * K + k];
                if (x == 0.f) continue;
                uint16_t hi, lo;
                split_host(x, hi, lo);
                const int j = k / 16, pce = (k % 16) / 8, e = k % 8;
                const size_t el = w0 + (size_t)j * 4096 + (size_t)pce * 1024 + (size_t)m * 8 + e;
                ks_w[el] = hi;
                ks_w[el + 2048] = lo;
            }
    }
    tile_ks0.push_back((int32_t)(ks_rows.size() / 16));
    PropPlan* p = new PropPlan();
    p->nksteps = (int)(ks_rows.size() / 16);
    p->density = issued > 0 ? useful / issued : 0.0;
    const size_t b_tk = tile_ks0.size() * 4, b_kr = ks_rows.size() * 4, b_kw = ks_w.size() * sizeof(uint16_t);
    auto up = [](size_t x) { return (x + 255) & ~size_t(255); };
    const size_t total = up(b_tk) + up(b_kr) + up(b_kw);
    if (cudaMalloc(&p->blob, total) != cudaSuccess) { delete p; return nullptr; }
    unsigned char* d = reinterpret_cast<unsigned char*>(p->blob);
    size_t off = 0;
    auto put = [&](const void* src, size_t bytes) {
        void* dst = d + off;
        cudaMemcpy(dst, src, bytes, cudaMemcpyHostToDevice);
        off += up(bytes);
        return dst;
    };
    p->dev.ks_w = reinterpret_cast<const uint16_t*>(put(ks_w.data(), b_kw));
    p->dev.tile_ks0 = reinterpret_cast<const int32_t*>(put(tile_ks0.data(), b_tk));
    p->dev.ks_rows = reinterpret_cast<const int32_t*>(put(ks_rows.data(), b_kr));
    p->dev.ntiles = out.ntiles;
    p->dev.nslots_in = (int)in.node_of_slot.size();
    p->dev.nslots_out = (int)out.node_of_slot.size();
    if (cudaGetLastError() != cudaSuccess) { cudaFree(p->blob); delete p; return nullptr; }
    return p;
}

}

LayerTiling make_tiling(int C, int H, int W) {
    const std::vector<std::vector<int>> tiles = (H == 1 && W == 1) ? range_tiles(C) : grid_tiles(C, H, W);
    LayerTiling t;
    t.ntiles = (int)tiles.size();
    t.node_of_slot.assign((size_t)t.ntiles * TILE, -1);
    t.slot_of_node.assign((size_t)C * H * W, -1);
    for (int i = 0; i < t.ntiles; ++i)
        for (size_t m = 0; m < tiles[i].size(); ++m) {
            t.node_of_slot[(size_t)i * TILE + m] = tiles[i][m];
            t.slot_of_node[tiles[i][m]] = i * TILE + (int)m;
        }
    return t;
}

int prop_tc_init() {
    return cudaFuncSetAttribute(k_tc_prop, cudaFuncAttributeMaxDynamicSharedMemorySize, (int)prop::PROP_SMEM);
}

PropPlan* prop_plan_build(const LayerDev& L, const float* w, bool backward, bool normalise, const LayerTiling& out,
                          const LayerTiling& in) {
    const int k = L.ksize, s = L.stride, p = L.pad;
    if (L.kind == GNNB_LAYER_CONV) {
        const int hw_in = L.h_in * L.w_in, hw_out = L.h_out * L.w_out;
        if (!backward) {
            EdgeFn f = [=](int node, std::vector<Edge>& ev) {
                const int co = node / hw_out, y = (node % hw_out) / L.w_out, x = node % L.w_out;
                for (int ci = 0; ci < L.c_in; ++ci)
                    for (int ky = 0; ky < k; ++ky) {
                        const int yy = y * s + ky - p;
                        if (yy < 0 || yy >= L.h_in) continue;
                        for (int kx = 0; kx < k; ++kx) {
                            const int xx = x * s + kx - p;
                            if (xx < 0 || xx >= L.w_in) continue;
                            ev.push_back({ci * hw_in + yy * L.w_in + xx, w[((co * L.c_in + ci) * k + ky) * k + kx]});
                        }
                    }
            };
            return build_plan(out, in, f);
        }
        EdgeFn f = [=](int node, std::vector<Edge>& ev) {
            const int ci = node / hw_in, yi = (node % hw_in) / L.w_in, xi = node % L.w_in;
            int taps = 0;
            const size_t first = ev.size();
            for (int ky = 0; ky < k; ++ky) {
                const int ty = yi + p - ky;
                if (ty < 0 || ty % s != 0 || ty / s >= L.h_out) continue;
                for (int kx = 0; kx < k; ++kx) {
                    const int tx = xi + p - kx;
                    if (tx < 0 || tx % s != 0 || tx / s >= L.w_out) continue;
                    ++taps;
                    for (int co = 0; co < L.c_out; ++co)
                        ev.push_back({co * hw_out + (ty / s) * L.w_out + tx / s, w[((co * L.c_in + ci) * k + ky) * k + kx]});
                }
            }
            if (normalise && taps > 0)
                for (size_t i = first; i < ev.size(); ++i) ev[i].w = ev[i].w / (float)taps;
        };
        return build_plan(out, in, f);
    }
    if (!backward) {
        EdgeFn f = [=](int node, std::vector<Edge>& ev) {
            for (int i = 0; i < L.n_in; ++i) ev.push_back({i, w[(size_t)node * L.n_in + i]});
        };
        return build_plan(out, in, f);
    }
    EdgeFn f = [=](int node, std::vector<Edge>& ev) {
        for (int o = 0; o < L.n_out; ++o) ev.push_back({o, w[(size_t)o * L.n_in + node]});
    };
    return build_plan(out, in, f);
}

void prop_plan_free(PropPlan* p) {
    if (!p) return;
    if (p->blob) cudaFree(p->blob);
    delete p;
}

double prop_plan_density(const PropPlan* p) { return p ? p->density : 0.0; }
const PropPlanDev& prop_plan_dev(const PropPlan* p) { return p->dev; }
double prop_plan_ksteps_per_tile(const PropPlan* p) { return p->dev.ntiles > 0 ? (double)p->nksteps / p->dev.ntiles : 1.0; }

void prop_tc_run(const PropPlan* plan, const float* mu_img, float* nb_img, int Bc, cudaStream_t st, int64_t* launches) {
    const int64_t nitems = (int64_t)plan->dev.ntiles * ((Bc + prop::PD - 1) / prop::PD);
    const int grid = (int)(nitems < 1 ? 1 : (nitems < 148 ? nitems : 148));
    launch_pdl(k_tc_prop, grid, prop::PROP_THREADS, prop::PROP_SMEM, st, plan->dev,
               reinterpret_cast<const uint16_t*>(mu_img), reinterpret_cast<uint16_t*>(nb_img), Bc);
    ++*launches;
}

namespace {
__global__ void k_property_backward_img(const float* __restrict__ wp, const float* __restrict__ mu_out,
                                        uint16_t* __restrict__ nb_img, int nL, int nslots, int64_t total8) {
    for (int64_t i = (int64_t)blockIdx.x * blockDim.x + threadIdx.x; i < total8; i += (int64_t)gridDim.x * blockDim.x) {
        const int chunk = (int)(i & 7);
        const int64_t row = i >> 3;
        const int64_t b = row / nslots;
        const int node = (int)(row - b * nslots);
        const float w = node < nL ? wp[b * nL + node] * ASCALE : 0.f;
        const float4 m0 = *reinterpret_cast<const float4*>(mu_out + b * P + chunk * 8);
        const float4 m1 = *reinterpret_cast<const float4*>(mu_out + b * P + chunk * 8 + 4);
        uint4 hi, lo;
        split2(w * m0.x, w * m0.y, hi.x, lo.x);
        split2(w * m0.z, w * m0.w, hi.y, lo.y);
        split2(w * m1.x, w * m1.y, hi.z, lo.z);
        split2(w * m1.z, w * m1.w, hi.w, lo.w);
        unsigned char* img = reinterpret_cast<unsigned char*>(nb_img) + (row / TILE) * (int64_t)ABUF;
        const uint32_t off = (uint32_t)chunk * NB_PIECE + (uint32_t)(row % TILE) * 16u;
        *reinterpret_cast<uint4*>(img + off) = hi;
        *reinterpret_cast<uint4*>(img + APLANE + off) = lo;
    }
}
}

void prop_tc_property_backward(const float* wp, const float* mu_out, float* nb_img, int nL, int nslots, int Bc, cudaStream_t st, int64_t* launches) {
    const int64_t total8 = (int64_t)Bc * nslots * 8;
    const int64_t blocks = (total8 + 255) / 256;
    k_property_backward_img<<<(unsigned)(blocks < 1 ? 1 : (blocks < 148 * 16 ? blocks : 148 * 16)), 256, 0, st>>>(
        wp, mu_out, reinterpret_cast<uint16_t*>(nb_img), nL, nslots, total8);
    ++*launches;
}

}
```

gnn_branching_b200/csrc/gnnb_tc.cu:

```cuda
#include "gnnb_prop_body.cuh"
#include "gnnb_umma.cuh"

namespace gnnb {
namespace {

using namespace tcx;

constexpr uint32_t ACOL = 0, DCOL = 64, WG_COLS = 128;

struct WG {
    uint32_t land;
    uint32_t mbar_mma, mbar_tma;
    uint32_t ph_mma, ph_tma;
    uint32_t tmem;
    uint32_t tmem0;
    uint32_t acol;
    int t;
    int bar_threads;
    int wg;
    bool lead_warp;
};

__device__ __forceinline__ void wg_barrier(const WG& c) { named_bar(1 + c.wg, c.bar_threads); }

// ... 319 lines not shown
    auto fetch_row = [&](int64_t it) {
        nrow_n = -1; l_n = 0.f; u_n = 1.f; slot0_n = 0;
        if (it >= nitems) return;
        const int d = (int)(it / tiles_per_dom) * NWG + c.wg;
        if (d >= a.Bc) return;
        const int64_t tl_ = (int64_t)d * tiles_per_dom + it % tiles_per_dom;
        nrow_n = natural_row(map, tl_ * TILE + c.t);
        if (nrow_n >= 0) { l_n = ldg1_now(lb + nrow_n); u_n = ldg1_now(ub + nrow_n); }
        slot0_n = __ldg(amb_base + tl_);
    };
    fetch_row(rank);
    for (int64_t item = rank; item < nitems; item += nranks) {
        const int dom = (int)(item / tiles_per_dom) * NWG + c.wg;
        const int64_t nrow = nrow_n;
        const float l = l_n, u = u_n;
        const int slot0 = slot0_n;
        if (dom >= a.Bc) {
            fetch_row(item + nranks);
            continue;
        }
        const int64_t tile = (int64_t)dom * tiles_per_dom + item % tiles_per_dom;
        const int64_t row0 = tile * TILE, grow = row0 + c.t;
        request_nb(c, nb_img + (size_t)tile * (ABUF / 2));
        fetch_row(item + nranks);
        const Ratio q = compute_ratio(l, u);
        const float gate = (q.r0 != 0.0f) ? 1.0f : 0.0f;
        const bool amb = (q.amb != 0.0f) && nrow >= 0;
        const unsigned bal = __ballot_sync(0xffffffffu, amb);
        if ((c.t & 31) == 0) tl.wcnt[c.wg][c.t >> 5] = __popc(bal);
        GNNB_TR(0);
        gemm_ss(c, W + UPD_W3, W + UPD_W3 + 2 * WPLANE, 128, 0);
        GNNB_TR(1);
        if (c.t == 0 && item + nranks < nitems) {
            const int64_t nitem = item + nranks;
            const int ndom = (int)(nitem / tiles_per_dom) * NWG + c.wg;
            if (ndom < a.Bc) prefetch_l2(nb_img + (size_t)((int64_t)ndom * tiles_per_dom + nitem % tiles_per_dom) * (ABUF / 2), ABUF);
        }
        int slot = slot0 + __popc(bal & ((1u << (c.t & 31)) - 1u));
#pragma unroll
        for (int w = 0; w < 3; ++w) slot += (w < (c.t >> 5)) ? tl.wcnt[c.wg][w] : 0;
        const float* rt = rlx + (size_t)(slot >> 7) * (TILE * P) + (size_t)(slot & (TILE - 1)) * 4;
        if (amb) {
#pragma unroll
            for (int i = 0; i < 16; ++i) asm volatile("prefetch.global.L2 [%0];" ::"l"(rt + (size_t)i * (TILE * 4)));
        }
#pragma unroll
        for (int qd = 0; qd < 4; ++qd) {
            float a[16], b[16], bb[16];
            {
                uint32_t ra[16], rb[16];
                tmem_ld16(c.tmem + qd * 16, ra);
                tmem_ld16(c.tmem + 64 + qd * 16, rb);
                tmem_wait16(ra, a);
                tmem_wait16(rb, b);
            }
            lds16(tl.bias[0] + qd * 16, bb);
#pragma unroll
            for (int j = 0; j < 16; ++j) a[j] = relu_nan(fmaf(q.r0, a[j], fmaf(q.r1, b[j], bb[j])));
            a_store16(c, qd, a);
        }
        GNNB_TR(2);
        gemm_ts_start(c, W + UPD_WC, W + UPD_WC + WPLANE, 64, DCOL);
        float4 rx[16];
        {
#pragma unroll
            for (int i = 0; i < 16; ++i) rx[i] = amb ? ldg4_now(rt + (size_t)i * (TILE * 4)) : make_float4(0.f, 0.f, 0.f, 0.f);
        }
        gemm_finish(c);
        GNNB_TR(3);
#pragma unroll
        for (int qd = 0; qd < 4; ++qd) {
            float v[16], bb[16];
            tmem_ld16_sync(c.tmem + DCOL + qd * 16, v);
            lds16(tl.bias[1] + qd * 16, bb);
#pragma unroll
            for (int h = 0; h < 4; ++h) {
                const float4 x = rx[qd * 4 + h];
                v[h * 4 + 0] = relu_nan(v[h * 4 + 0] + x.x + bb[h * 4 + 0]);
                v[h * 4 + 1] = relu_nan(v[h * 4 + 1] + x.y + bb[h * 4 + 1]);
                v[h * 4 + 2] = relu_nan(v[h * 4 + 2] + x.z + bb[h * 4 + 2]);
                v[h * 4 + 3] = relu_nan(v[h * 4 + 3] + x.w + bb[h * 4 + 3]);
            }
            a_store16(c, qd, v);
        }
        GNNB_TR(4);
        gemm_ts(c, W + UPD_W42, W + UPD_W42 + WPLANE, 64, DCOL);
        GNNB_TR(5);
        if (scores == nullptr) {
            bad |= nan_watch(a.nan_doms, dom, epilogue_to_mu<false>(c, DCOL, tl.bias[2], gate, nrow >= 0));
            commit_tile(c, mu_out + (size_t)tile * (ABUF / 2));
        } else {
            bad |= nan_watch(a.nan_doms, dom, epilogue_to_mu<true>(c, DCOL, tl.bias[2], gate, nrow >= 0, mu_out != nullptr));
            if (mu_out != nullptr) commit_tile(c, mu_out + (size_t)tile * (ABUF / 2));
            gemm_ts(c, W + UPD_FN, W + UPD_FN + WPLANE, 64, DCOL);
            float sc = 0.f;
#pragma unroll
            for (int qd = 0; qd < 4; ++qd) {
                float v[16], bb[16], ww[16];
                tmem_ld16_sync(c.tmem + DCOL + qd * 16, v);
                lds16(tl.bias[3] + qd * 16, bb);
                lds16(tl.vec + qd * 16, ww);
#pragma unroll
                for (int j = 0; j < 16; ++j) sc = fmaf(relu_nan(v[j] + bb[j]), ww[j], sc);
            }
            if (nrow >= 0) scores[(nrow / map.n) * score_stride + score_off + (nrow % map.n)] = fmaf(sc, AINV, bscore);
        }
        GNNB_TR(6);
        GNNB_TR_NEXT();
    }
    GNNB_TR_PRINT("update[top gemm1 epi1 gemm2 epi2 gemm3 epi3]", 7);
    if (bad) atomicAdd(a.nan_count, 1ULL);
    if (c.t == 0) bulk_wait_all();
    cta_teardown(s);
}

__global__ void __launch_bounds__(128 * NWG, 1) k_tc_update(UpdArgs a) {
    update_body(a, smem_dyn(), (int)blockIdx.x, (int)gridDim.x, true);
}

namespace fz {
constexpr int PD = 2;
constexpr int CW = 2;
constexpr int NS_MAX = 8;
constexpr uint32_t W_KS = 8192;
constexpr uint32_t B_ROWS = 16;
constexpr uint32_t B_DOM = B_ROWS * 128;
constexpr uint32_t B_PLANE = PD * B_DOM;
constexpr uint32_t B_STAGE = 2 * B_PLANE;
constexpr uint32_t STAGE = W_KS + B_STAGE;
constexpr uint32_t STG_PLANE = 32 * 128;
constexpr uint32_t STG_WARP = 2 * STG_PLANE;
constexpr uint32_t STG_BYTES = CW * 4 * STG_WARP;
constexpr uint32_t INF_WN = 0, INF_WI = 2 * WPLANE, INF_B22 = 4 * WPLANE;
constexpr int THREADS = 768;
constexpr int GATHER_WARP0 = 2, GATHER_WARPS = 6, CHAIN_WARP0 = 8;
constexpr uint32_t ACC_COL = 0, ACC_WIN = PD * 64, D_COL = 256, D_WIN = 128;

struct Tail {
    float bias[4][P];
    float vec[P];
    uint64_t wts, full[NS_MAX], empty[NS_MAX], acc_full[2], acc_empty[2], mma[CW];
    uint32_t tmem_slot;
    int32_t wcnt[2 * CW][4];
};
constexpr size_t smem_for(uint32_t wbytes, int staging, int n_stages) {
    return 1024 + wbytes + (size_t)staging * (STG_BYTES / 2) + (size_t)n_stages * STAGE + sizeof(Tail);
}
constexpr size_t SMEM_MAX = 232448;
}

struct FusedArgs {
    UpdArgs u;
    PropPlanDev plan;
    const uint16_t* mu_in;
    uint16_t* nb_dbg;
    int n_stages;
    int mma_group;
    int input_layer;
};

__device__ __forceinline__ void tmem_ld32_sync(uint32_t taddr, float (&v0)[16], float (&v1)[16]) {
    uint32_t r0[16], r1[16];
    tmem_ld16(taddr, r0);
    tmem_ld16(taddr + 16, r1);
    tmem_wait16(r0, v0);
    tmem_wait16(r1, v1);
}

__device__ __forceinline__ void split16(const float (&v)[16], uint32_t (&w)[16]) {
#pragma unroll
    for (int i = 0; i < 8; ++i) split2(v[2 * i], v[2 * i + 1], w[i], w[8 + i]);
}
__device__ __forceinline__ void sts128(uint32_t addr, uint32_t a, uint32_t b, uint32_t c, uint32_t d) {
    asm volatile("st.shared.v4.b32 [%0], {%1, %2, %3, %4};" ::"r"(addr), "r"(a), "r"(b), "r"(c), "r"(d) : "memory");
}

#ifdef GNNB_TRACE
__device__ long long g_e3_trace[4];
#define E3TR(i) do { if (blockIdx.x == 1 && threadIdx.x == fz::CHAIN_WARP0 * 32) { const long long n_ = clock64(); g_e3_trace[i] += n_ - e3t_; e3t_ = n_; } } while (0)
#else
#define E3TR(i) do {} while (0)
#endif
struct NoOp { __device__ __forceinline__ void operator()() const {} };
template <bool TO_A, class Between = NoOp>
__device__ __forceinline__ bool epilogue_to_mu_pair(const WG& c, int h, int pair_bar, uint32_t dcol, const float* __restrict__ bias_s,
                                                    float rowscale, bool valid, unsigned char* img, uint32_t stage, Between between = Between()) {
    bool bad = false;
#ifdef GNNB_TRACE
    long long e3t_ = clock64();
#endif
    const uint32_t rl = (uint32_t)c.t & 31u;
    const bool issuer = h == 0 && rl == 0;
    unsigned char* dst = img + ((uint32_t)c.t >> 5) * fz::STG_PLANE;
    uint32_t lo[TO_A ? 16 : 1];
    if (img != nullptr) {
        if (issuer) bulk_wait_read();
        named_bar(pair_bar, 64);
    }
    E3TR(0);
    {
        float v0[16], v1[16];
        tmem_ld32_sync(c.tmem + dcol + h * 32, v0, v1);
        E3TR(1);
#pragma unroll
        for (int qq = 0; qq < 2; ++qq) {
            float (&v)[16] = qq ? v1 : v0;
            const int q = 2 * h + qq;
            float bb[16];
            lds16(bias_s + q * 16, bb);
#pragma unroll
            for (int j = 0; j < 16; ++j) {
                v[j] = (v[j] + bb[j]) * rowscale;
                bad |= (v[j] != v[j]);
            }
            uint32_t w[16];
            split16(v, w);
            if (img != nullptr) {
                const uint32_t o0 = stage + swz(rl, (uint32_t)(2 * q)), o1 = stage + swz(rl, (uint32_t)(2 * q + 1));
                sts128(o0, w[0], w[1], w[2], w[3]);
                sts128(o1, w[4], w[5], w[6], w[7]);
                if (!TO_A) {
                    sts128(o0 + fz::STG_PLANE, w[8], w[9], w[10], w[11]);
                    sts128(o1 + fz::STG_PLANE, w[12], w[13], w[14], w[15]);
                }
            }
            if (TO_A) {
#pragma unroll
                for (int i = 0; i < 8; ++i) lo[qq * 8 + i] = w[8 + i];
                tmem_st16(c.tmem + c.acol + 16 * q, w);
            }
        }
    }
    E3TR(2);
    if (!TO_A) between();
    if (img != nullptr) {
        fence_proxy_async();
        named_bar(pair_bar, 64);
        if (!TO_A) {
            if (issuer) {
                bulk_s2g_nocommit(dst, stage, fz::STG_PLANE);
                bulk_s2g_nocommit(dst + APLANE, stage + fz::STG_PLANE, fz::STG_PLANE);
                bulk_commit();
            }
        } else {
            if (issuer) { bulk_s2g(dst, stage, fz::STG_PLANE); bulk_wait_read(); }
            named_bar(pair_bar, 64);
#pragma unroll
            for (int qq = 0; qq < 2; ++qq) {
                const int q = 2 * h + qq;
                sts128(stage + swz(rl, (uint32_t)(2 * q)), lo[qq * 8], lo[qq * 8 + 1], lo[qq * 8 + 2], lo[qq * 8 + 3]);
                sts128(stage + swz(rl, (uint32_t)(2 * q + 1)), lo[qq * 8 + 4], lo[qq * 8 + 5], lo[qq * 8 + 6], lo[qq * 8 + 7]);
            }
            fence_proxy_async();
            named_bar(pair_bar, 64);
            if (issuer) bulk_s2g(dst + APLANE, stage, fz::STG_PLANE);
        }
    }
    E3TR(3);
    return bad && valid;
}

struct ItemCursor {
    int pair, tile, dq, dr, ntiles, npairs;
    __device__ __forceinline__ ItemCursor(int rank, int nranks, int ntiles_, int npairs_)
        : pair(rank / ntiles_), tile(rank % ntiles_), dq(nranks / ntiles_), dr(nranks % ntiles_), ntiles(ntiles_), npairs(npairs_) {}
    __device__ __forceinline__ bool valid() const { return pair < npairs; }
    __device__ __forceinline__ void next() {
        tile += dr; pair += dq;
        if (tile >= ntiles) { tile -= ntiles; ++pair; }
    }
};

template <bool INPUT_LAYER>
__device__ __forceinline__ void fused_body(const FusedArgs& fa) {
    using namespace fz;
    const UpdArgs& a = fa.u;
    const GnnParams& g = a.g;
    const PropPlanDev& plan = fa.plan;
    const bool with_score = a.scores != nullptr;
    const uint32_t wbytes = with_score ? UPD_WBYTES : UPD_FN;
    const int NS = fa.n_stages;
    unsigned char* base = smem_dyn();
    base += (1024u - (smem_u32(base) & 1023u)) & 1023u;
    const uint32_t stg_warp = a.mu_out == nullptr ? 0u : (with_score ? STG_PLANE : STG_WARP), stg_bytes = CW * 4 * stg_warp;
    const uint32_t W = smem_u32(base), stg = W + wbytes, ring = stg + stg_bytes;
    fz::Tail* tl = reinterpret_cast<fz::Tail*>(base + wbytes + stg_bytes + (size_t)NS * STAGE);
    const int warp = uniform((int)(threadIdx.x >> 5)), lane = threadIdx.x & 31;
    if (threadIdx.x == 0) {
        mbar_init(smem_u32(&tl->wts), 1);
        for (int i = 0; i < NS; ++i) { mbar_init(smem_u32(&tl->full[i]), 1 + 32); mbar_init(smem_u32(&tl->empty[i]), 1); }
        for (int i = 0; i < 2; ++i) { mbar_init(smem_u32(&tl->acc_full[i]), 1); mbar_init(smem_u32(&tl->acc_empty[i]), PD); }
        for (int i = 0; i < CW; ++i) mbar_init(smem_u32(&tl->mma[i]), 1);
        fence_mbar_init();
    }
    __syncwarp();
    if (warp == 0) tmem_alloc(smem_u32(&tl->tmem_slot), 512);
    tc_fence_before();
    __syncthreads();
    tc_fence_after();
    const uint32_t tmem_base = tl->tmem_slot;
    const int l3 = a.backward ? BC3 : FC3, l4b = a.backward ? BC4_1 : FC4_2, lc = a.backward ? T_BWD_C : T_FWD_C;
    constexpr bool inp = INPUT_LAYER;
    if (threadIdx.x == 0) {
        const uint32_t mb = smem_u32(&tl->wts);
        if (!inp) {
            mbar_expect_tx(mb, wbytes);
            bulk_g2s(W + UPD_W3, g.tc[l3], 4 * WPLANE, mb);
            bulk_g2s(W + UPD_WC, g.tcx_w[lc], 2 * WPLANE, mb);
            bulk_g2s(W + UPD_W42, g.tc[l4b], 2 * WPLANE, mb);
            if (with_score) bulk_g2s(W + UPD_FN, g.tc[FNODE], 2 * WPLANE, mb);
        } else {
            mbar_expect_tx(mb, 6 * WPLANE);
            bulk_g2s(W + INF_WN, g.tcx_w[T_INP_NB], 2 * WPLANE, mb);
            bulk_g2s(W + INF_WI, g.tcx_w[T_INP_C], 2 * WPLANE, mb);
            bulk_g2s(W + INF_B22, g.tc[INP_B2_2], 2 * WPLANE, mb);
        }
    }
    if (!inp) {
        copy_vec(tl->bias[0], g.bias[l3], P); copy_vec(tl->bias[1], g.tcx_b[lc], P); copy_vec(tl->bias[2], g.bias[l4b], P);
        copy_vec(tl->bias[3], g.bias[FNODE], P); copy_vec(tl->vec, g.wt[FSCORE], P, 1.0f);
    } else {
        copy_vec(tl->bias[0], g.tcx_b[T_INP_C], P); copy_vec(tl->bias[1], g.bias[INP_B2_2], P); copy_vec(tl->bias[2], g.bias[INP_B], P);
        copy_vec(tl->bias[3], g.wt[INP_B], 2 * P);
    }
    __syncthreads();
    pdl_trigger(); pdl_wait();

    const int ntiles = plan.ntiles, npairs = (a.Bc + PD - 1) / PD;
    const int rank = (int)blockIdx.x, nranks = (int)gridDim.x;

    if (warp == 0) {
        if (lane == 0) {
            uint32_t slot = 0, ph = 0;
            for (ItemCursor cur(rank, nranks, ntiles, npairs); cur.valid(); cur.next()) {
                const int ks0 = plan.tile_ks0[cur.tile], ks1 = plan.tile_ks0[cur.tile + 1];
                for (int ks = ks0; ks < ks1; ++ks) {
                    mbar_wait(smem_u32(&tl->empty[slot]), ph ^ 1u);
                    const uint32_t full = smem_u32(&tl->full[slot]);
                    mbar_expect_tx(full, W_KS);
                    bulk_g2s(ring + slot * STAGE, plan.ks_w + (size_t)ks * (W_KS / 2), W_KS, full);
                    if (++slot == (uint32_t)NS) { slot = 0; ph ^= 1u; }
                }
            }
        }
    } else if (warp == 1) {
        const uint32_t idesc = (1u << 4) | (1u << 16) | ((uint32_t)(PD * 64 >> 3) << 17) | ((uint32_t)(TILE >> 4) << 24);
        uint32_t t = 0, it = 0, slot = 0, ph = 0;
        const int group = fa.mma_group;
        const uint64_t d_a_hi = make_desc_nosw(ring, NB_PIECE, 128u), d_a_lo = make_desc_nosw(ring + W_KS / 2, NB_PIECE, 128u);
        const uint64_t d_b_hi = make_desc_mn(ring + W_KS, B_DOM), d_b_lo = make_desc_mn(ring + W_KS + B_PLANE, B_DOM);
        uint32_t lag_slot0 = 0, lag_slot1 = 0, lag_ph0 = 0, lag_ph1 = 0;
        bool have_lag = false, have_prev = false;
#ifdef GNNB_TRACE
        long long t_acc = 0, t_b = 0, t_lag = 0, t_all = clock64(), t0_;
#define FTR_BEGIN() t0_ = clock64()
#define FTR_END(x) x += clock64() - t0_
#else
#define FTR_BEGIN()
#define FTR_END(x)
#endif
        for (ItemCursor cur(rank, nranks, ntiles, npairs); cur.valid(); cur.next(), ++it) {
            const int ks0 = uniform(plan.tile_ks0[cur.tile]), ks1 = uniform(plan.tile_ks0[cur.tile + 1]);
            const uint32_t buf = it & 1u, bufph = (it >> 1) & 1u;
            FTR_BEGIN();
            mbar_wait(smem_u32(&tl->acc_empty[buf]), bufph ^ 1u);
            FTR_END(t_acc);
            tc_fence_after();
            const uint32_t d = (tmem_base & 0x0000FFFFu) + ACC_COL + buf * ACC_WIN;
            uint32_t accum = 0;
            for (int ks = ks0; ks < ks1;) {
                const int n = ks1 - ks < group ? ks1 - ks : group;
                FTR_BEGIN();
                if (have_lag) mbar_wait(smem_u32(&tl->empty[lag_slot0]), lag_ph0);
                FTR_END(t_lag);
                lag_slot0 = lag_slot1; lag_ph0 = lag_ph1; have_lag = have_prev;
                for (int i = 0; i < n; ++i, ++t) {
                    FTR_BEGIN();
                    mbar_wait(smem_u32(&tl->full[slot]), ph);
                    FTR_END(t_b);
                    tc_fence_after();
                    const uint64_t soff = (uint64_t)(slot * (STAGE >> 4));
                    const uint64_t a_hi = d_a_hi + soff, a_lo = d_a_lo + soff, b_hi = d_b_hi + soff, b_lo = d_b_lo + soff;
                    if (elect_one()) {
                        umma(d, a_hi, b_hi, idesc, accum);
                        umma(d, a_lo, b_hi, idesc, 1u);
                        umma(d, a_hi, b_lo, idesc, 1u);
                        umma_commit(smem_u32(&tl->empty[slot]));
                    }
                    __syncwarp();
                    accum = 1u;
                    lag_slot1 = slot; lag_ph1 = ph;
                    if (++slot == (uint32_t)NS) { slot = 0; ph ^= 1u; }
                }
                have_prev = true;
                ks += n;
            }
            if (elect_one()) umma_commit(smem_u32(&tl->acc_full[buf]));
            __syncwarp();
        }
#ifdef GNNB_TRACE
        if (rank == 1 && lane == 0) printf("TRACE fused-mma: items %u ksteps %u total %lld | wait acc_empty %lld, lag %lld, stage full %lld\n", it, t,
                                           clock64() - t_all, t_acc, t_lag, t_b);
#endif
    } else if (warp >= GATHER_WARP0 && warp < GATHER_WARP0 + GATHER_WARPS) {
        const int gw = warp - GATHER_WARP0;
        const int GW = GATHER_WARPS < NS ? GATHER_WARPS : NS;
        const unsigned char* mu_bytes = reinterpret_cast<const unsigned char*>(fa.mu_in);
#ifdef GNNB_TRACE
        long long g_wait = 0, g_all = clock64();
#endif
        uint32_t slot = 0, ph = 0;
        int turn = 0;
        for (ItemCursor cur(rank, nranks, ntiles, npairs); cur.valid(); cur.next()) {
            const int ks0 = __ldg(plan.tile_ks0 + cur.tile), ks1 = __ldg(plan.tile_ks0 + cur.tile + 1);
            const int dm0 = cur.pair * PD;
            const uint32_t jp = (uint32_t)(lane & 7);
            const unsigned char* base0 = mu_bytes + (int64_t)dm0 * (plan.nslots_in >> 7) * (int64_t)ABUF + jp * 16u;
            const uint32_t sz0 = dm0 < a.Bc ? 16u : 0u, sz1 = dm0 + 1 < a.Bc ? 16u : 0u;
            const unsigned char* base1 = sz1 ? base0 + (int64_t)(plan.nslots_in >> 7) * (int64_t)ABUF : base0;
            for (int ks = ks0; ks < ks1; ++ks) {
                const uint32_t slot_ = slot, ph_ = ph;
                const bool mine = turn == gw;
                if (++slot == (uint32_t)NS) { slot = 0; ph ^= 1u; }
                if (++turn == GW) turn = 0;
                if (!mine) continue;
                const int idx = __ldg(plan.ks_rows + (size_t)ks * 16 + (lane & 15));
                const int off = idx < 0 ? -1 : (idx << 7) + ((idx >> 7) << 14);
#ifdef GNNB_TRACE
                const long long g0_ = clock64();
#endif
                mbar_wait(smem_u32(&tl->empty[slot_]), ph_ ^ 1u);
#ifdef GNNB_TRACE
                g_wait += clock64() - g0_;
#endif
                const uint32_t dst0 = ring + slot_ * STAGE + W_KS;
#pragma unroll
                for (int q = 0; q < 4; ++q) {
                    const int k = q * 4 + (lane >> 3);
                    const int o = __shfl_sync(0xffffffffu, off, k);
                    const bool ok = o >= 0;
                    const uint32_t oo = ok ? (uint32_t)o : 0u, r7 = (oo >> 7) & 7u;
                    const uint32_t dst = dst0 + swz((uint32_t)k, jp ^ r7);
                    const uint32_t z0 = ok ? sz0 : 0u, z1 = ok ? sz1 : 0u;
                    cp_async16_sz(dst, base0 + oo, z0);
                    cp_async16_sz(dst + B_PLANE, base0 + oo + APLANE, z0);
                    cp_async16_sz(dst + B_DOM, base1 + oo, z1);
                    cp_async16_sz(dst + B_DOM + B_PLANE, base1 + oo + APLANE, z1);
                }
                cp_async_arrive(smem_u32(&tl->full[slot_]));
            }
        }
#ifdef GNNB_TRACE
        if (rank == 1 && gw == 0 && lane == 0) printf("TRACE fused-gather: total %lld, wait stage empty %lld\n", clock64() - g_all, g_wait);
#endif
    } else if (warp >= CHAIN_WARP0) {
        const float* __restrict__ lb = a.lb;
        const float* __restrict__ ub = a.ub;
        const float* __restrict__ rlx = a.rlx;
        const int32_t* __restrict__ amb_base = a.amb_base;
        float* __restrict__ scores = a.scores;
        const RowMap map = a.map;
        const float bscore = g.bias[FSCORE][0];
        const int cw = warp - CHAIN_WARP0;
        const int j = uniform(cw >> 3), h = uniform((cw >> 2) & 1);
        WG c;
        c.wg = j;
        c.bar_threads = 256;
        c.lead_warp = (cw & 7) == 0;
        c.t = threadIdx.x & 127;
        c.land = 0;
        c.mbar_mma = smem_u32(&tl->mma[j]);
        c.mbar_tma = 0;
        c.ph_mma = 0;
        c.ph_tma = 0;
        c.acol = ACC_COL;
        c.tmem0 = (uint32_t)uniform((int)tmem_base) & 0x0000FFFFu;
        c.tmem = tmem_base + ((uint32_t)((c.t >> 5) * 32) << 16);
        const uint32_t D = D_COL + D_WIN * (uint32_t)j;
        const int pw = j * 4 + (cw & 3);
        const uint32_t stage = stg + (uint32_t)pw * stg_warp;
        const int pair_bar = 3 + pw;
        const int Q0 = 2 * h;
        mbar_wait(smem_u32(&tl->wts), 0);
        bool bad = false;
        int node_n = -1, node_nn = -1;
        float l_n = 0.f, u_n = 1.f;
        int slot0_n = 0;
        auto fetch_node = [&](const ItemCursor& cu) -> int {
            if (!cu.valid() || cu.pair * PD + j >= a.Bc) return -1;
            return ldgi_now(map.node_of_slot + cu.tile * TILE + c.t);
        };
        auto fetch_bounds = [&](const ItemCursor& cu, int node_) {
            node_n = node_; l_n = 0.f; u_n = 1.f; slot0_n = 0;
            if (!cu.valid()) return;
            const int d_ = cu.pair * PD + j;
            if (d_ >= a.Bc) return;
            if (node_ >= 0) { l_n = ldg1_now(lb + (int64_t)d_ * map.n + node_); u_n = ldg1_now(ub + (int64_t)d_ * map.n + node_); }
            if (amb_base != nullptr) slot0_n = ldgi_now(amb_base + (int64_t)d_ * ntiles + cu.tile);
        };
        ItemCursor cur(rank, nranks, ntiles, npairs), cur1 = cur, cur2 = cur;
        cur1.next();
        cur2.next(); cur2.next();
        fetch_bounds(cur, fetch_node(cur));
        node_nn = fetch_node(cur1);
        uint32_t it = 0;
#ifdef GNNB_TRACE
        long long c_wait = 0, c_ph[8] = {0, 0, 0, 0, 0, 0, 0, 0}, c_all = clock64(), c0_;
        int c_tiles = 0;
#define CTR(i) do { const long long n_ = clock64(); c_ph[i] += n_ - c0_; c0_ = n_; } while (0)
#else
#define CTR(i) do {} while (0)
#endif
        auto start_item = [&](const ItemCursor& cu, uint32_t it_, int node_, float l_, float u_) -> bool {
            const uint32_t buf = it_ & 1u, bufph = (it_ >> 1) & 1u;
            const int dom_ = cu.pair * PD + j;
#ifdef GNNB_TRACE
            const long long w0_ = clock64();
#endif
            mbar_wait(smem_u32(&tl->acc_full[buf]), bufph);
#ifdef GNNB_TRACE
            c_wait += clock64() - w0_;
#endif
            tc_fence_after();
            if (dom_ >= a.Bc) {
                if (h == 0 && c.t == 0) mbar_arrive(smem_u32(&tl->acc_empty[buf]));
                return false;
            }
            const int64_t tile = (int64_t)dom_ * ntiles + cu.tile;
            c.acol = ACC_COL + buf * ACC_WIN + 64u * (uint32_t)j;
            {
                unsigned char* dbg = fa.nb_dbg ? reinterpret_cast<unsigned char*>(fa.nb_dbg) + tile * (int64_t)ABUF + (uint32_t)c.t * 16u : nullptr;
                float v0[16], v1[16];
                tmem_ld32_sync(c.tmem + c.acol + h * 32, v0, v1);
#pragma unroll
                for (int qq = 0; qq < 2; ++qq) {
                    const int qd = Q0 + qq;
                    uint32_t w[16];
                    split16(qq ? v1 : v0, w);
                    tmem_st16(c.tmem + c.acol + 16 * qd, w);
                    if (dbg != nullptr) {
#pragma unroll
                        for (int hh = 0; hh < 2; ++hh) {
                            const uint32_t off = (uint32_t)(qd * 2 + hh) * NB_PIECE;
                            *reinterpret_cast<uint4*>(dbg + off) = make_uint4(w[4 * hh], w[4 * hh + 1], w[4 * hh + 2], w[4 * hh + 3]);
                            *reinterpret_cast<uint4*>(dbg + APLANE + off) = make_uint4(w[8 + 4 * hh], w[8 + 4 * hh + 1], w[8 + 4 * hh + 2], w[8 + 4 * hh + 3]);
                        }
                    }
                }
            }
            if (inp) {
                {
                    const float* w0 = &tl->bias[3][0];
#pragma unroll
                    for (int qq = 0; qq < 2; ++qq) {
                        const int qd = Q0 + qq;
                        float o[16], wl[16], wu[16];
                        lds16(tl->bias[2] + qd * 16, o);
                        lds16(w0 + qd * 16, wl);
                        lds16(w0 + P + qd * 16, wu);
#pragma unroll
                        for (int i = 0; i < 16; ++i) o[i] = relu_nan(fmaf(node_ >= 0 ? l_ : 0.f, wl[i], fmaf(node_ >= 0 ? u_ : 0.f, wu[i], o[i])));
                        uint32_t w[16];
                        split16(o, w);
                        tmem_st16(c.tmem + D + 64 + 16 * qd, w);
                    }
                }
                gemm_sync(c);
                if (c.lead_warp) {
                    tc_fence_after();
                    if (elect_one()) {
                        WG c2 = c;
                        c2.acol = D + 64;
                        issue_ts(c, W + INF_WN, W + INF_WN + WPLANE, 64, D, false);
                        issue_ts(c2, W + INF_WI, W + INF_WI + WPLANE, 64, D, true);
                        umma_commit(c.mbar_mma);
                    }
                    __syncwarp();
                }
            } else {
                gemm_ts_start(c, W + UPD_W3, W + UPD_W3 + 2 * WPLANE, 128, D);
            }
            return true;
        };
        bool have = cur.valid() ? start_item(cur, 0, node_n, l_n, u_n) : false;
        for (; cur.valid(); cur.next(), cur1.next(), cur2.next(), ++it) {
            const uint32_t buf = it & 1u;
            const uint32_t acc_empty = smem_u32(&tl->acc_empty[buf]);
            const int dom = cur.pair * PD + j;
            const int node = node_n;
            const float l = l_n, u = u_n;
            const int slot0 = slot0_n;
            fetch_bounds(cur1, node_nn);
            node_nn = fetch_node(cur2);
            auto advance = [&]() { have = cur1.valid() ? start_item(cur1, it + 1, node_n, l_n, u_n) : false; };
            if (!have) {
                advance();
                continue;
            }
            const int64_t tile = (int64_t)dom * ntiles + cur.tile;
#ifdef GNNB_TRACE
            c0_ = clock64(); ++c_tiles;
#endif
            const Ratio q = compute_ratio(l, u);
            const float gate = (q.r0 != 0.0f) ? 1.0f : 0.0f;
            const bool amb = (q.amb != 0.0f) && node >= 0;
            const unsigned bal = __ballot_sync(0xffffffffu, amb);
            if ((c.t & 31) == 0) tl->wcnt[j * 2 + h][c.t >> 5] = __popc(bal);
            unsigned char* img = a.mu_out ? reinterpret_cast<unsigned char*>(a.mu_out) + tile * (int64_t)ABUF : nullptr;
            if (inp) {
                gemm_finish(c);
                if (h == 0 && c.t == 0) mbar_arrive(acc_empty);
                c.acol = D + 64;
                CTR(1);
                {
                    float v0[16], v1[16];
                    tmem_ld32_sync(c.tmem + D + h * 32, v0, v1);
#pragma unroll
                    for (int qq = 0; qq < 2; ++qq) {
                        float (&v)[16] = qq ? v1 : v0;
                        const int qd = Q0 + qq;
                        float bb[16];
                        lds16(tl->bias[0] + qd * 16, bb);
#pragma unroll
                        for (int i = 0; i < 16; ++i) v[i] = relu_nan(v[i] + bb[i]);
                        a_store16(c, qd, v);
                    }
                }
                CTR(2);
                gemm_ts_start(c, W + INF_B22, W + INF_B22 + WPLANE, 64, D);
                gemm_finish(c);
                CTR(3);
                bad |= nan_watch(a.nan_doms, dom, epilogue_to_mu_pair<false>(c, h, pair_bar, D, tl->bias[1], 1.0f, node >= 0, img, stage, advance));
                CTR(6);
                continue;
            }
            gemm_finish(c);
            if (h == 0 && c.t == 0) mbar_arrive(acc_empty);
            c.acol = D + 64;
            CTR(1);
#pragma unroll
            for (int qq = 0; qq < 2; ++qq) {
                const int qd = Q0 + qq;
                float x[16], y[16], bb[16];
                {
                    uint32_t ra[16], rb[16];
                    tmem_ld16(c.tmem + D + qd * 16, ra);
                    tmem_ld16(c.tmem + D + 64 + qd * 16, rb);
                    tmem_wait16(ra, x);
                    tmem_wait16(rb, y);
                }
                lds16(tl->bias[0] + qd * 16, bb);
#pragma unroll
                for (int i = 0; i < 16; ++i) x[i] = relu_nan(fmaf(q.r0, x[i], fmaf(q.r1, y[i], bb[i])));
                a_store16(c, qd, x);
            }
            CTR(2);
            gemm_ts_start(c, W + UPD_WC, W + UPD_WC + WPLANE, 64, D);
            int slot = slot0 + __popc(bal & ((1u << (c.t & 31)) - 1u));
#pragma unroll
            for (int w = 0; w < 3; ++w) slot += (w < (c.t >> 5)) ? tl->wcnt[j * 2 + h][w] : 0;
            const float* rt = rlx + (size_t)(slot >> 7) * (TILE * P) + (size_t)(slot & (TILE - 1)) * 4 + (size_t)(8 * h) * (TILE * 4);
            float4 rx[8];
#pragma unroll
            for (int i = 0; i < 8; ++i) rx[i] = amb ? ldg4_now(rt + (size_t)i * (TILE * 4)) : make_float4(0.f, 0.f, 0.f, 0.f);
            gemm_finish(c);
            CTR(3);
            {
                float v0[16], v1[16];
                tmem_ld32_sync(c.tmem + D + h * 32, v0, v1);
#pragma unroll
                for (int qq = 0; qq < 2; ++qq) {
                    float (&v)[16] = qq ? v1 : v0;
                    const int qd = Q0 + qq;
                    float bb[16];
                    lds16(tl->bias[1] + qd * 16, bb);
#pragma unroll
                    for (int hh = 0; hh < 4; ++hh) {
                        const float4 x = rx[qq * 4 + hh];
                        v[hh * 4 + 0] = relu_nan(v[hh * 4 + 0] + x.x + bb[hh * 4 + 0]);
                        v[hh * 4 + 1] = relu_nan(v[hh * 4 + 1] + x.y + bb[hh * 4 + 1]);
                        v[hh * 4 + 2] = relu_nan(v[hh * 4 + 2] + x.z + bb[hh * 4 + 2]);
                        v[hh * 4 + 3] = relu_nan(v[hh * 4 + 3] + x.w + bb[hh * 4 + 3]);
                    }
                    a_store16(c, qd, v);
                }
            }
            CTR(4);
            gemm_ts_start(c, W + UPD_W42, W + UPD_W42 + WPLANE, 64, D);
            gemm_finish(c);
            CTR(5);
            if (!with_score) {
                bad |= nan_watch(a.nan_doms, dom, epilogue_to_mu_pair<false>(c, h, pair_bar, D, tl->bias[2], gate, node >= 0, img, stage, advance));
            } else {
                bad |= nan_watch(a.nan_doms, dom, epilogue_to_mu_pair<true>(c, h, pair_bar, D, tl->bias[2], gate, node >= 0, img, stage));
                gemm_ts_start(c, W + UPD_FN, W + UPD_FN + WPLANE, 64, D);
                gemm_finish(c);
                float sc = 0.f;
                {
                    float v0[16], v1[16];
                    tmem_ld32_sync(c.tmem + D + h * 32, v0, v1);
#pragma unroll
                    for (int qq = 0; qq < 2; ++qq) {
                        const int qd = Q0 + qq;
                        float bb[16], ww[16];
                        lds16(tl->bias[3] + qd * 16, bb);
                        lds16(tl->vec + qd * 16, ww);
#pragma unroll
                        for (int i = 0; i < 16; ++i) sc = fmaf(relu_nan((qq ? v1 : v0)[i] + bb[i]), ww[i], sc);
                    }
                }
                if (h == 1) {
                    tmem_st1(c.tmem + D + 64, __float_as_uint(sc));
                    tmem_st_wait();
                }
                tc_fence_before();
                wg_barrier(c);
                tc_fence_after();
                if (h == 0) {
                    sc += __uint_as_float(tmem_ld1_sync(c.tmem + D + 64));
                    if (node >= 0) scores[(int64_t)dom * a.score_stride + a.score_off + node] = fmaf(sc, AINV, bscore);
                }
                advance();
            }
            CTR(6);
        }
#ifdef GNNB_TRACE
        if (rank == 1 && threadIdx.x == CHAIN_WARP0 * 32)
            printf("TRACE fused-chain wg0: tiles %d total %lld | wait acc_full %lld | per tile: convert %lld gemm1 %lld epi1 %lld gemm2 %lld epi2 %lld gemm3 %lld epi3 %lld\n",
                   c_tiles, clock64() - c_all, c_wait, c_ph[0] / max(c_tiles, 1), c_ph[1] / max(c_tiles, 1), c_ph[2] / max(c_tiles, 1), c_ph[3] / max(c_tiles, 1),
                   c_ph[4] / max(c_tiles, 1), c_ph[5] / max(c_tiles, 1), c_ph[6] / max(c_tiles, 1));
        if (rank == 1 && threadIdx.x == CHAIN_WARP0 * 32) {
            printf("TRACE fused-e3 (cumulative over launches): wait prev store %lld, tmem load %lld, compute + stage %lld, fence + issue %lld\n",
                   g_e3_trace[0], g_e3_trace[1], g_e3_trace[2], g_e3_trace[3]);
        }
#endif
        if (bad) atomicAdd(a.nan_count, 1ULL);
        if (h == 0 && (c.t & 31) == 0) bulk_wait_all();
    }
    tc_fence_before();
    __syncthreads();
    if (warp == 0) tmem_dealloc(tmem_base, 512);
}

__global__ void __launch_bounds__(fz::THREADS, 1) k_tc_fused(FusedArgs fa) { fused_body<false>(fa); }
__global__ void __launch_bounds__(fz::THREADS, 1) k_tc_fused_input(FusedArgs fa) { fused_body<true>(fa); }

constexpr uint32_t RLX_FR = 0, RLX_BC11 = 2 * WPLANE, RLX_BC12 = 4 * WPLANE, RLX_BC2 = 6 * WPLANE, RLX_BR = 12 * WPLANE;
constexpr uint32_t RLX_WBYTES = 14 * WPLANE;

struct RelaxLayers {
    NodeInputs in[AMB_MAX_LAYERS];
    float* rlx_f[AMB_MAX_LAYERS];
    float* rlx_b[AMB_MAX_LAYERS];
    int n;
};

__global__ void __launch_bounds__(128 * NWG, 1) k_tc_relax(GnnParams g, const __grid_constant__ RelaxLayers rl) {
    const uint16_t* const wsrc[5] = {g.tcx_w[T_FWD_R], g.tc[BC1_1], g.tc[BC1_2], g.tc[BC2], g.tcx_w[T_BWD_R]};
    const uint32_t woff[5] = {RLX_FR, RLX_BC11, RLX_BC12, RLX_BC2, RLX_BR};
    const uint32_t wlen[5] = {2 * WPLANE, 2 * WPLANE, 2 * WPLANE, 6 * WPLANE, 2 * WPLANE};
    CtaSetup s = cta_setup<false, 5>(smem_dyn(), RLX_WBYTES, wsrc, woff, wlen);
    Tail& tl = *s.tail;
    copy_vec(tl.bias[0], g.tcx_b[T_FWD_R], P); copy_vec(tl.bias[1], g.bias[BC1_1], P); copy_vec(tl.bias[2], g.bias[BC1_2], P);
    copy_vec(tl.bias[3], g.bias[BC2], P); copy_vec(tl.bias[4], g.tcx_b[T_BWD_R], P);
    copy_vec(tl.w_small[0], g.wt[FC1], 7 * P); copy_vec(tl.w_small[1], g.wt[BC1], 7 * P);
    copy_vec(tl.bias[5], g.bias[FC1], P); copy_vec(tl.vec, g.bias[BC1], P);
    __syncthreads();
    mbar_wait(smem_u32(&tl.mbar[0]), 0);
    pdl_trigger(); pdl_wait();
    WG c = make_wg(s, RLX_WBYTES);
    const uint32_t W = s.w;
    int tile0[AMB_MAX_LAYERS + 1];
    tile0[0] = 0;
#pragma unroll 1
    for (int k = 0; k < rl.n; ++k) {
        const int namb_k = __ldg(rl.in[k].amb_base + (rl.in[k].rows + TILE - 1) / TILE);
        tile0[k + 1] = tile0[k] + (namb_k + TILE - 1) / TILE;
    }
    const int total_tiles = tile0[rl.n];
    int k = 0;
    for (int gt = (int)blockIdx.x * NWG + c.wg; gt < total_tiles; gt += (int)gridDim.x * NWG) {
        while (gt >= tile0[k + 1]) ++k;
        const NodeInputs& in = rl.in[k];
        float* __restrict__ rlx_f = rl.rlx_f[k];
        float* __restrict__ rlx_b = rl.rlx_b[k];
        const int64_t tile = gt - tile0[k];
        const int64_t namb = __ldg(in.amb_base + (in.rows + TILE - 1) / TILE);
        const int64_t slot = tile * TILE + c.t;
        float l = 0.f, u = 1.f, d1 = 0.f, d2 = 0.f, pp = 0.f, po = 0.f, bs = 0.f;
        if (slot < namb) {
            const int64_t grow = natural_row(in.map, __ldg(in.amb_rows + slot));
            l = in.lb[grow]; u = in.ub[grow];
            d1 = in.dual[grow * 3 + 1]; d2 = in.dual[grow * 3 + 2];
            pp = in.prim_pre[grow]; po = in.prim_post[grow];
            bs = in.bias_node[grow % in.map.n];
        }
        const Ratio q = compute_ratio(l, u);
        {
            const float feat[7] = {q.beta, l, u, d1 - d2, pp, po, bs};
            first_layer_to_a<7>(c, feat, tl.w_small[0], tl.bias[5]);
        }
        gemm_ts(c, W + RLX_FR, W + RLX_FR + WPLANE, 64, DCOL);
        epilogue_to_rlx(c, DCOL, tl.bias[0], q.amb, rlx_f + (size_t)tile * (TILE * P));
        {
            const float feat[7] = {l, u, q.beta, -d2 + d1, po, pp, bs};
            first_layer_to_a<7>(c, feat, tl.w_small[1], tl.vec);
        }
        gemm_ts(c, W + RLX_BC11, W + RLX_BC11 + WPLANE, 64, DCOL);
        epilogue_to_a<true>(c, DCOL, tl.bias[1]);
        gemm_ts(c, W + RLX_BC12, W + RLX_BC12 + WPLANE, 64, DCOL);
        epilogue_to_a<false>(c, DCOL, tl.bias[2]);
        float acc[64];
        gemm_ts(c, W + RLX_BC2, W + RLX_BC2 + 3 * WPLANE, 64, DCOL);
#pragma unroll
        for (int qd = 0; qd < 4; ++qd) {
            float v[16], bb[16];
            tmem_ld16_sync(c.tmem + DCOL + qd * 16, v);
            lds16(tl.bias[3] + qd * 16, bb);
#pragma unroll
            for (int j = 0; j < 16; ++j) acc[qd * 16 + j] = v[j] + bb[j];
        }
        gemm_ts(c, W + RLX_BC2 + WPLANE, W + RLX_BC2 + 4 * WPLANE, 64, DCOL);
        {
            const float nd2 = -d2;
#pragma unroll
            for (int qd = 0; qd < 4; ++qd) {
                float v[16];
                tmem_ld16_sync(c.tmem + DCOL + qd * 16, v);
#pragma unroll
                for (int j = 0; j < 16; ++j) acc[qd * 16 + j] = fmaf(nd2, v[j], acc[qd * 16 + j]);
            }
        }
        gemm_ts(c, W + RLX_BC2 + 2 * WPLANE, W + RLX_BC2 + 5 * WPLANE, 64, DCOL);
#pragma unroll
        for (int qd = 0; qd < 4; ++qd) {
            float v[16];
            tmem_ld16_sync(c.tmem + DCOL + qd * 16, v);
#pragma unroll
            for (int j = 0; j < 16; ++j) v[j] = relu_nan(fmaf(d1, v[j], acc[qd * 16 + j]));
            a_store16(c, qd, v);
        }
        gemm_ts(c, W + RLX_BR, W + RLX_BR + WPLANE, 64, DCOL);
        epilogue_to_rlx(c, DCOL, tl.bias[4], q.amb, rlx_b + (size_t)tile * (TILE * P));
    }
    cta_teardown(s);
}

constexpr uint32_t EMB_WBYTES = 2 * WPLANE;

__global__ void __launch_bounds__(128 * NWG, 1) k_tc_input_embed(GnnParams g, const float* __restrict__ lb0,
                                                                 const float* __restrict__ x, const float* __restrict__ ub0,
                                                                 uint16_t* __restrict__ mu0, RowMap map, int64_t rows) {
    const uint16_t* const wsrc[1] = {g.tc[INP_F_1]};
    const uint32_t woff[1] = {0};
    const uint32_t wlen[1] = {2 * WPLANE};
    CtaSetup s = cta_setup<true, 1>(smem_dyn(), EMB_WBYTES, wsrc, woff, wlen);
    Tail& tl = *s.tail;
    copy_vec(tl.bias[0], g.bias[INP_F_1], P); copy_vec(tl.bias[5], g.bias[INP_F], P); copy_vec(tl.w_small[0], g.wt[INP_F], 3 * P);
    __syncthreads();
    mbar_wait(smem_u32(&tl.mbar[0]), 0);
    pdl_trigger(); pdl_wait();
    WG c = make_wg(s, EMB_WBYTES);
    const int64_t ntiles = (rows + TILE - 1) / TILE;
    for (int64_t tile = (int64_t)blockIdx.x * NWG + c.wg; tile < ntiles; tile += (int64_t)gridDim.x * NWG) {
        const int64_t row0 = tile * TILE, grow = row0 + c.t;
        float feat[3] = {0.f, 0.f, 0.f};
        const int64_t nrow = grow < rows ? natural_row(map, grow) : -1;
        if (nrow >= 0) { feat[0] = lb0[nrow]; feat[1] = x[nrow]; feat[2] = ub0[nrow]; }
        first_layer_to_a<3>(c, feat, tl.w_small[0], tl.bias[5]);
        if (c.t == 0) bulk_wait_read();
        gemm_ts(c, s.w, s.w + WPLANE, 64, DCOL);
        epilogue_to_mu<false>(c, DCOL, tl.bias[0], 1.0f, nrow >= 0);
        commit_tile(c, mu0 + (size_t)tile * (ABUF / 2));
    }
    if (c.t == 0) bulk_wait_all();
    cta_teardown(s);
}

constexpr uint32_t INU_WI = 0, INU_WN = 2 * WPLANE, INU_B22 = 4 * WPLANE, INU_WBYTES = 6 * WPLANE;

__global__ void __launch_bounds__(128 * NWG, 1) k_tc_input_update(GnnParams g, const float* __restrict__ lb0,
                                                                  const float* __restrict__ ub0, const uint16_t* __restrict__ nb_img,
                                                                  uint16_t* __restrict__ mu0, RowMap map, int64_t rows) {
    const uint16_t* const wsrc[3] = {g.tcx_w[T_INP_C], g.tcx_w[T_INP_NB], g.tc[INP_B2_2]};
    const uint32_t woff[3] = {INU_WI, INU_WN, INU_B22};
    const uint32_t wlen[3] = {2 * WPLANE, 2 * WPLANE, 2 * WPLANE};
    CtaSetup s = cta_setup<true, 3>(smem_dyn(), INU_WBYTES, wsrc, woff, wlen);
    Tail& tl = *s.tail;
    copy_vec(tl.bias[0], g.tcx_b[T_INP_C], P); copy_vec(tl.bias[1], g.bias[INP_B2_2], P);
    copy_vec(tl.bias[5], g.bias[INP_B], P); copy_vec(tl.w_small[0], g.wt[INP_B], 2 * P);
    __syncthreads();
    mbar_wait(smem_u32(&tl.mbar[0]), 0);
    pdl_trigger(); pdl_wait();
    WG c = make_wg(s, INU_WBYTES);
    const uint32_t W = s.w;
// ... 51 lines not shown
    const __half* lo = hi + APLANE / 2;
    for (int j = 0; j < 8; ++j) out[nrow * P + chunk * 8 + j] = (__half2float(hi[j]) + __half2float(lo[j])) * AINV;
}

__device__ __forceinline__ bool row_is_ambiguous(const float* __restrict__ lb, const float* __restrict__ ub, const RowMap& map,
                                                 int64_t row, int64_t rows) {
    const int64_t nrow = row < rows ? natural_row(map, row) : -1;
    return nrow >= 0 && compute_ratio(lb[nrow], ub[nrow]).amb != 0.0f;
}
__global__ void __launch_bounds__(TILE) k_amb_count(const float* __restrict__ lb, const float* __restrict__ ub, RowMap map,
                                                    int64_t rows, int32_t* __restrict__ cnt) {
    const int64_t row = (int64_t)blockIdx.x * TILE + threadIdx.x;
    const bool amb = row_is_ambiguous(lb, ub, map, row, rows);
    const int total = __syncthreads_count(amb);
    if (threadIdx.x == 0) cnt[blockIdx.x] = total;
}
__global__ void __launch_bounds__(1024) k_amb_scan(const int32_t* __restrict__ cnt, int32_t* __restrict__ base, int n) {
    __shared__ int32_t part[1024];
    const int per = (n + 1023) / 1024, lo = threadIdx.x * per, hi = min(n, lo + per);
    int32_t sum = 0;
    for (int i = lo; i < hi; ++i) sum += cnt[i];
    part[threadIdx.x] = sum;
    __syncthreads();
    for (int off = 1; off < 1024; off <<= 1) {
        const int32_t v = threadIdx.x >= off ? part[threadIdx.x - off] : 0;
        __syncthreads();
        part[threadIdx.x] += v;
        __syncthreads();
    }
    int32_t run = part[threadIdx.x] - sum;
    for (int i = lo; i < hi; ++i) { base[i] = run; run += cnt[i]; }
    if (threadIdx.x == 1023) base[n] = part[1023];
}
__global__ void __launch_bounds__(TILE) k_amb_fill(const float* __restrict__ lb, const float* __restrict__ ub, RowMap map,
                                                   int64_t rows, const int32_t* __restrict__ base, int32_t* __restrict__ amb_rows) {
    __shared__ int32_t wc[4];
    const int64_t row = (int64_t)blockIdx.x * TILE + threadIdx.x;
    const bool amb = row_is_ambiguous(lb, ub, map, row, rows);
    const unsigned bal = __ballot_sync(0xffffffffu, amb);
    const int lane = threadIdx.x & 31, warp = threadIdx.x >> 5;
    if (lane == 0) wc[warp] = __popc(bal);
    __syncthreads();
    int slot = base[blockIdx.x] + __popc(bal & ((1u << lane) - 1u));
    for (int w = 0; w < warp; ++w) slot += wc[w];
    if (amb) amb_rows[slot] = (int32_t)row;
}

__device__ __forceinline__ int amb_layer_of(const AmbLayers& a, int tile) {
    int k = 0;
    while (k + 1 < a.n && tile >= a.tile0[k + 1]) ++k;
    return k;
}
__global__ void __launch_bounds__(TILE) k_amb_count_all(AmbLayers a) {
    const int k = amb_layer_of(a, (int)blockIdx.x), tile = (int)blockIdx.x - a.tile0[k];
    const int64_t row = (int64_t)tile * TILE + threadIdx.x;
    const bool amb = row_is_ambiguous(a.lb[k], a.ub[k], a.map[k], row, a.rows[k]);
    const int total = __syncthreads_count(amb);
    if (threadIdx.x == 0) a.cnt[k][tile] = total;
}
__global__ void __launch_bounds__(1024) k_amb_scan_all(AmbLayers a) {
    __shared__ int32_t part[1024];
    const int k = blockIdx.x, n = a.tile0[k + 1] - a.tile0[k];
    const int32_t* __restrict__ cnt = a.cnt[k];
    int32_t* __restrict__ base = a.base[k];
    const int per = (n + 1023) / 1024, lo = threadIdx.x * per, hi = min(n, lo + per);
    int32_t sum = 0;
    for (int i = lo; i < hi; ++i) sum += cnt[i];
    part[threadIdx.x] = sum;
    __syncthreads();
    for (int off = 1; off < 1024; off <<= 1) {
        const int32_t v = threadIdx.x >= off ? part[threadIdx.x - off] : 0;
        __syncthreads();
        part[threadIdx.x] += v;
        __syncthreads();
    }
    int32_t run = part[threadIdx.x] - sum;
    for (int i = lo; i < hi; ++i) { base[i] = run; run += cnt[i]; }
    if (threadIdx.x == 1023) base[n] = part[1023];
}
__global__ void __launch_bounds__(TILE) k_amb_fill_all(AmbLayers a) {
    __shared__ int32_t wc[4];
    const int k = amb_layer_of(a, (int)blockIdx.x), tile = (int)blockIdx.x - a.tile0[k];
    const int64_t row = (int64_t)tile * TILE + threadIdx.x;
    const bool amb = row_is_ambiguous(a.lb[k], a.ub[k], a.map[k], row, a.rows[k]);
    const unsigned bal = __ballot_sync(0xffffffffu, amb);
    const int lane = threadIdx.x & 31, warp = threadIdx.x >> 5;
    if (lane == 0) wc[warp] = __popc(bal);
    __syncthreads();
    int slot = a.base[k][tile] + __popc(bal & ((1u << lane) - 1u));
    for (int w = 0; w < warp; ++w) slot += wc[w];
    if (amb) a.out_rows[k][slot] = (int32_t)row;
}

}

void amb_compact_all(AmbLayers a, cudaStream_t st, int64_t* launches) {
    a.tile0[0] = 0;
    for (int k = 0; k < a.n; ++k) a.tile0[k + 1] = a.tile0[k] + (int)((a.rows[k] + TILE - 1) / TILE);
    k_amb_count_all<<<a.tile0[a.n], TILE, 0, st>>>(a);
    k_amb_scan_all<<<a.n, 1024, 0, st>>>(a);
    k_amb_fill_all<<<a.tile0[a.n], TILE, 0, st>>>(a);
    *launches += 3;
}

void amb_compact(const float* lb, const float* ub, RowMap map, int64_t rows, int32_t* cnt, int32_t* amb_base, int32_t* amb_rows,
                 cudaStream_t st, int64_t* launches) {
    const int ntiles = (int)((rows + TILE - 1) / TILE);
    k_amb_count<<<ntiles, TILE, 0, st>>>(lb, ub, map, rows, cnt);
    k_amb_scan<<<1, 1024, 0, st>>>(cnt, amb_base, ntiles);
    k_amb_fill<<<ntiles, TILE, 0, st>>>(lb, ub, map, rows, amb_base, amb_rows);
    *launches += 3;
}

bool tc_available() { return true; }

int tc_init() {
    cudaError_t e;
    if ((e = cudaFuncSetAttribute(k_tc_update, cudaFuncAttributeMaxDynamicSharedMemorySize, (int)smem_bytes(UPD_WBYTES, true))) != cudaSuccess) return e;
    if ((e = cudaFuncSetAttribute(k_tc_fused, cudaFuncAttributeMaxDynamicSharedMemorySize, (int)fz::SMEM_MAX)) != cudaSuccess) return e;
    if ((e = cudaFuncSetAttribute(k_tc_fused_input, cudaFuncAttributeMaxDynamicSharedMemorySize, (int)fz::SMEM_MAX)) != cudaSuccess) return e;
    if ((e = cudaFuncSetAttribute(k_tc_relax, cudaFuncAttributeMaxDynamicSharedMemorySize, (int)smem_bytes(RLX_WBYTES, false))) != cudaSuccess) return e;
    if ((e = cudaFuncSetAttribute(k_tc_input_embed, cudaFuncAttributeMaxDynamicSharedMemorySize, (int)smem_bytes(EMB_WBYTES, true))) != cudaSuccess) return e;
    if ((e = cudaFuncSetAttribute(k_tc_input_update, cudaFuncAttributeMaxDynamicSharedMemorySize, (int)smem_bytes(INU_WBYTES, true))) != cudaSuccess) return e;
    return 0;
}

int64_t tc_packed_elems(int K) { return (int64_t)2 * (K / 64) * 64 * 64; }

int64_t tc_pack_weight(const float* w, int K, uint16_t* dst) {
    const int nblk = K / 64;
    for (int n = 0; n < 64; ++n)
        for (int k = 0; k < K; ++k) {
            uint16_t hi, lo;
            split_host(w[(size_t)n * K + k], hi, lo);
            const int kb = k / 64, kk = k % 64;
            const size_t e = (size_t)(swz((uint32_t)n, (uint32_t)(kk / 8)) + (kk % 8) * 2) / 2;
            dst[(size_t)kb * 4096 + e] = hi;
            dst[(size_t)(nblk + kb) * 4096 + e] = lo;
        }
    return tc_packed_elems(K);
}

void tc_relax(const GnnParams& g, const NodeInputs* in, float* const* relax_f, float* const* relax_b, int n_layers, cudaStream_t st,
              int64_t* launches) {
    RelaxLayers rl;
    rl.n = n_layers;
    int64_t rows = 0;
    for (int k = 0; k < n_layers; ++k) { rl.in[k] = in[k]; rl.rlx_f[k] = relax_f[k]; rl.rlx_b[k] = relax_b[k]; rows += in[k].rows; }
    launch_pdl(k_tc_relax, grid_for(rows), 128 * NWG, smem_bytes(RLX_WBYTES, false), st, g, rl);
    ++*launches;
}

namespace {
UpdArgs make_upd_args(const GnnParams& g, bool backward, const float* lb, const float* ub, const float* nb, const float* relax,
                      const int32_t* amb_base, float* mu_out, float* scores, RowMap map, int64_t score_stride, int64_t score_off,
                      int64_t rows, unsigned long long* nan_count, const NanDoms& nan_doms) {
    UpdArgs a;
    a.g = g; a.backward = backward ? 1 : 0; a.lb = lb; a.ub = ub; a.nb_img = reinterpret_cast<const uint16_t*>(nb); a.rlx = relax;
    a.amb_base = amb_base; a.mu_out = reinterpret_cast<uint16_t*>(mu_out); a.scores = scores; a.map = map;
    a.score_stride = score_stride; a.score_off = score_off; a.Bc = (int)(rows / map.nslots); a.nan_count = nan_count;
    a.nan_doms = nan_doms;
    return a;
}
}

void tc_update(const GnnParams& g, bool backward, const float* lb, const float* ub, const float* nb, const float* relax,
               const int32_t* amb_base, float* mu_out, float* scores, RowMap map, int64_t score_stride, int64_t score_off, int64_t rows,
               unsigned long long* nan_count, const NanDoms& nan_doms, cudaStream_t st, int64_t* launches) {
    const UpdArgs a = make_upd_args(g, backward, lb, ub, nb, relax, amb_base, mu_out, scores, map, score_stride, score_off, rows, nan_count,
                                    nan_doms);
    const int64_t nitems = (int64_t)(map.nslots / TILE) * ((a.Bc + NWG - 1) / NWG);
    launch_pdl(k_tc_update, (int)(nitems < 1 ? 1 : (nitems < 148 ? nitems : 148)), 128 * NWG, smem_bytes(UPD_WBYTES, true), st, a);
    ++*launches;
}

void tc_fused(const GnnParams& g, const PropPlan* plan, const float* mu_in, bool backward, const float* lb, const float* ub,
              const float* relax, const int32_t* amb_base, float* mu_out, float* scores, RowMap map, int64_t score_stride, int64_t score_off,
              int64_t rows, unsigned long long* nan_count, const NanDoms& nan_doms, float* nb_dbg, bool input_layer, cudaStream_t st,
              int64_t* launches) {
    FusedArgs fa;
    fa.input_layer = input_layer ? 1 : 0;
    fa.u = make_upd_args(g, backward, lb, ub, nullptr, relax, amb_base, mu_out, scores, map, score_stride, score_off, rows, nan_count,
                         nan_doms);
    fa.plan = prop_plan_dev(plan);
    fa.mu_in = reinterpret_cast<const uint16_t*>(mu_in);
    fa.nb_dbg = reinterpret_cast<uint16_t*>(nb_dbg);
    const uint32_t wbytes = scores ? UPD_WBYTES : UPD_FN;
    const int staging = mu_out == nullptr ? 0 : (scores ? 1 : 2);
    const int ns = (int)((fz::SMEM_MAX - fz::smem_for(wbytes, staging, 0)) / fz::STAGE);
    fa.n_stages = ns > fz::NS_MAX ? fz::NS_MAX : ns;
    fa.mma_group = prop_plan_ksteps_per_tile(plan) >= 48.0 ? 4 : 2;
    if (fa.mma_group > fa.n_stages / 2) fa.mma_group = fa.n_stages / 2;
    const int64_t nitems = (int64_t)fa.plan.ntiles * ((fa.u.Bc + fz::PD - 1) / fz::PD);
    launch_pdl(input_layer ? k_tc_fused_input : k_tc_fused, (int)(nitems < 1 ? 1 : (nitems < 148 ? nitems : 148)), fz::THREADS,
               fz::smem_for(wbytes, staging, fa.n_stages), st, fa);
    ++*launches;
}

void tc_input_embed(const GnnParams& g, const float* lb0, const float* x, const float* ub0, float* mu0, RowMap map, int64_t rows,
                    cudaStream_t st, int64_t* launches) {
    launch_pdl(k_tc_input_embed, grid_for(rows), 128 * NWG, smem_bytes(EMB_WBYTES, true), st, g, lb0, x, ub0, reinterpret_cast<uint16_t*>(mu0), map, rows);
    ++*launches;
}

void tc_input_update(const GnnParams& g, const float* lb0, const float* ub0, const float* nb, float* mu0, RowMap map, int64_t rows,
                     cudaStream_t st, int64_t* launches) {
    launch_pdl(k_tc_input_update, grid_for(rows), 128 * NWG, smem_bytes(INU_WBYTES, true), st,
               g, lb0, ub0, reinterpret_cast<const uint16_t*>(nb), reinterpret_cast<uint16_t*>(mu0), map, (int64_t)rows);
    ++*launches;
}

void tc_unpack_tile_image(const float* img, float* out, RowMap map, int64_t rows, bool piece_major, cudaStream_t st) {
    const int64_t n = rows * 8;
    k_unpack_tile_image<<<(unsigned)((n + 255) / 256), 256, 0, st>>>(reinterpret_cast<const uint16_t*>(img), out, map, rows, piece_major ? 1 : 0);
}

}
```

Measured before the change: 274,400.

## Specialise propagation plans to skip hidden nodes observed dead across batches

Adds a dead-node guard kernel that, on every chunk, checks which hidden nodes have a zero relaxation ratio in all domains. The dead set is read back asynchronously and used to build specialised live-only propagation plans and row maps. The fused kernels switch to the reduced plan unless the guard sees a node come alive, in which case they fall back to the full plan. Dead nodes get a constant score written directly. This cuts MMA work on inactive nodes but adds a guard kernel, host readback, plan rebuilds and extra workspace rows, and its correctness depends on the guard fallback behaving properly.

```diff
diff --git a/gnn_branching_b200/csrc/gnnb_api.cu b/gnn_branching_b200/csrc/gnnb_api.cu
--- a/gnn_branching_b200/csrc/gnnb_api.cu
+++ b/gnn_branching_b200/csrc/gnnb_api.cu
@@ -3,6 +3,7 @@
 #include <stdlib.h>
 #include <string.h>
 
+#include <algorithm>
 #include <map>
 #include <string>
 #include <vector>
@@ -48,6 +49,23 @@
     std::vector<LayerTiling> tiling;
     std::vector<RowMap> rowmap;
     int32_t* d_maps = nullptr;
+    std::vector<float> host_net;
+    std::vector<size_t> host_w_off;
+    struct Spec {
+        std::vector<RowMap> rowmap;
+        int32_t* d_maps = nullptr;
+        uint8_t* d_dead = nullptr;
+        std::vector<uint8_t> dead;
+        std::vector<PropPlan*> fwd, bwd, fwd_live, bwd_live;
+    };
+    Spec* spec = nullptr;
+    int64_t spec_gen = 0;
+    int32_t* d_guard = nullptr;
+    int32_t* h_guard = nullptr;
+    int guard_cap = 0;
+    cudaEvent_t ev_guard = nullptr;
+    int64_t rb_gen = -2;
+    int rb_waves = 0;
     LayerDev* d_layers = nullptr;
     int32_t* d_hidden_off = nullptr;
     int32_t* d_random_order = nullptr;
@@ -103,6 +121,73 @@
     return status;
 }
 
+void free_spec(gnnb_ctx* c) {
+    if (!c->spec) return;
+    gnnb_ctx::Spec* s = c->spec;
+    for (auto* v : {&s->fwd, &s->bwd, &s->fwd_live, &s->bwd_live})
+        for (PropPlan* p : *v) prop_plan_free(p);
+    if (s->d_maps) cudaFree(s->d_maps);
+    if (s->d_dead) cudaFree(s->d_dead);
+    delete s;
+    c->spec = nullptr;
+}
+
+bool build_spec(gnnb_ctx* ctx, std::vector<uint8_t> dead) {
+    const int L = (int)ctx->layers.size();
+    for (int k = 1; k < L; ++k) {
+        uint8_t* d = dead.data() + ctx->hidden_off[k];
+        int live = 0;
+        for (int i = 0; i < ctx->n[k]; ++i) live += d[i] ? 0 : 1;
+        if ((live + 127) / 128 >= ctx->tiling[k].ntiles) std::fill(d, d + ctx->n[k], 0);
+    }
+    std::vector<LayerTiling> full(L + 1), live(L + 1);
+    full[0] = live[0] = ctx->tiling[0];
+    full[L] = live[L] = ctx->tiling[L];
+    for (int k = 1; k < L; ++k) {
+        const LayerDev& d = ctx->layers[k - 1];
+        const bool conv = d.kind == GNNB_LAYER_CONV;
+        if (std::none_of(dead.begin() + ctx->hidden_off[k], dead.begin() + ctx->hidden_off[k] + ctx->n[k], [](uint8_t x) { return x != 0; })) {
+            full[k] = live[k] = ctx->tiling[k];
+            continue;
+        }
+        make_live_tiling(conv ? d.c_out : d.n_out, conv ? d.h_out : 1, conv ? d.w_out : 1, dead.data() + ctx->hidden_off[k], &full[k], &live[k]);
+    }
+    gnnb_ctx::Spec* s = new gnnb_ctx::Spec();
+    s->dead = dead;
+    s->rowmap = ctx->rowmap;
+    s->fwd.assign(L, nullptr); s->bwd.assign(L, nullptr); s->fwd_live.assign(L, nullptr); s->bwd_live.assign(L, nullptr);
+    auto bad = [&]() { for (auto* v : {&s->fwd, &s->bwd, &s->fwd_live, &s->bwd_live}) for (PropPlan* p : *v) prop_plan_free(p);
+                             if (s->d_maps) cudaFree(s->d_maps); if (s->d_dead) cudaFree(s->d_dead); delete s;
+                             cudaGetLastError(); return false; };
+    size_t slots = 0;
+    for (int k = 1; k < L; ++k) slots += full[k].node_of_slot.size();
+    if (cudaMalloc(&s->d_maps, slots * sizeof(int32_t)) != cudaSuccess || cudaMalloc(&s->d_dead, dead.size()) != cudaSuccess ||
+        cudaMemcpy(s->d_dead, dead.data(), dead.size(), cudaMemcpyHostToDevice) != cudaSuccess)
+        return bad();
+    size_t off = 0;
+    for (int k = 1; k < L; ++k) {
+        const std::vector<int32_t>& m = full[k].node_of_slot;
+        if (cudaMemcpy(s->d_maps + off, m.data(), m.size() * sizeof(int32_t), cudaMemcpyHostToDevice) != cudaSuccess)
+            return bad();
+        s->rowmap[k] = RowMap{s->d_maps + off, ctx->n[k], (int)m.size()};
+        off += m.size();
+    }
+    for (int k = 0; k < L; ++k) {
+        const float* w = ctx->host_net.data() + ctx->host_w_off[k];
+        const LayerTiling &t0 = ctx->tiling[k], &t1 = ctx->tiling[k + 1];
+        s->fwd[k] = prop_plan_build(ctx->layers[k], w, false, false, full[k + 1], full[k], t1, t0);
+        s->fwd_live[k] = prop_plan_build(ctx->layers[k], w, false, false, live[k + 1], live[k], t1, t0);
+        s->bwd[k] = prop_plan_build(ctx->layers[k], w, true, k > 0, full[k], full[k + 1], t0, t1);
+        s->bwd_live[k] = prop_plan_build(ctx->layers[k], w, true, k > 0, live[k], live[k + 1], t0, t1);
+        if (!s->fwd[k] || !s->fwd_live[k] || !s->bwd[k] || !s->bwd_live[k])
+            return bad();
+    }
+    free_spec(ctx);
+    ctx->spec = s;
+    ++ctx->spec_gen;
+    return true;
+}
+
 int axis_taps(int i, int ksize, int stride, int pad, int n_out) {
     int t = 0;
     for (int k = 0; k < ksize; ++k) {
@@ -181,7 +266,7 @@
     size_t total = 0;
     auto take = [&](size_t elems) { size_t off = total; total += (elems + 63) & ~size_t(63); return off; };
     std::vector<size_t> o_mu(L + 2), o_rf(L + 1), o_rb(L + 1), o_lb(L + 2), o_ub(L + 2), o_du(L), o_pr(L), o_po(L);
-    auto wrows = [&](int k) { return (size_t)Bc * (k <= L ? (size_t)ctx->rowmap[k].nslots : 128); };
+    auto wrows = [&](int k) { return (size_t)Bc * (k <= L ? (size_t)ctx->rowmap[k].nslots + (k >= 1 && k < L ? 128 : 0) : 128); };
     for (int k = 0; k <= L + 1; ++k) o_mu[k] = take(wrows(k) * P);
     for (int k = 1; k <= L; ++k) { o_rf[k] = take(wrows(k) * P); o_rb[k] = take(wrows(k) * P); }
     std::vector<size_t> o_ac(L + 1), o_ab(L + 1), o_ar(L + 1);
@@ -303,6 +388,11 @@
 
 #define TRY(expr) do { int s__ = (expr); if (s__ != GNNB_OK) return s__; } while (0)
 
+bool guarded(const gnnb_ctx* ctx) {
+    const int L = (int)ctx->layers.size();
+    return ctx->math == GNNB_MATH_TC_FP16X3 && ctx->fuse && !ctx->snapshot && L >= 2 && L - 1 <= AMB_MAX_LAYERS;
+}
+
 int run_chunk(gnnb_ctx* ctx, const GnnInputs& in, const float* mask, int Bc, int math, const NanDoms& nd, float* scores, int k,
               float* best_score, int32_t* best_idx, gnnb_winner* winners, cudaStream_t st) {
     const int L = (int)ctx->layers.size();
@@ -312,10 +402,32 @@
     int64_t* lc = &ctx->launches;
     auto name = [](const char* fmt, int a, int b) { char buf[64]; snprintf(buf, sizeof buf, fmt, a, b); return std::string(buf); };
 
-    auto R = [&](int k) { return (int64_t)Bc * (tc ? ctx->rowmap[k].nslots : ctx->n[k]); };
+    const bool guard = math == ctx->math && guarded(ctx);
+    const gnnb_ctx::Spec* sp = guard ? ctx->spec : nullptr;
+    const std::vector<RowMap>& maps = sp ? sp->rowmap : ctx->rowmap;
+    auto R = [&](int k) { return (int64_t)Bc * (tc ? maps[k].nslots : ctx->n[k]); };
     const RowMap nomap{nullptr, 0, 0};
-    auto M = [&](int k) { return tc ? ctx->rowmap[k] : nomap; };
+    auto M = [&](int k) { return tc ? maps[k] : nomap; };
     const bool fused = tc && ctx->fuse;
+    auto PF = [&](int k) { return sp ? sp->fwd[k] : ctx->plan_fwd[k]; };
+    auto PB = [&](int k) { return sp ? sp->bwd[k] : ctx->plan_bwd[k]; };
+    auto PFL = [&](int k) { return sp ? sp->fwd_live[k] : nullptr; };
+    auto PBL = [&](int k) { return sp ? sp->bwd_live[k] : nullptr; };
+
+    if (guard) {
+        ProfScope ps(ctx, GNNB_K_RELAX, 0, st);
+        CU(cudaMemsetAsync(ctx->d_guard, 0, sizeof(int32_t), st));
+        DeadGuard dg{};
+        dg.g = g;
+        dg.nl = L - 1;
+        for (int k = 1; k < L; ++k) { dg.lb[k - 1] = in.lb[k]; dg.ub[k - 1] = in.ub[k]; dg.off[k - 1] = ctx->hidden_off[k]; }
+        dg.off[L - 1] = ctx->hidden_off[L];
+        dg.Bc = Bc;
+        dg.dead = sp ? sp->d_dead : nullptr;
+        dg.guard = ctx->d_guard; dg.failed = ctx->d_guard + 1; dg.acc = ctx->d_guard + 2;
+        dg.scores = scores; dg.score_stride = ctx->n_hidden;
+        tc_dead_guard(dg, st, lc);
+    }
 
     const bool amb_all = tc && L <= AMB_MAX_LAYERS;
     if (amb_all) {
@@ -367,7 +479,7 @@
             const int64_t rows = R(k), nodes = (int64_t)Bc * ctx->n[k];
             if (fused) {
                 ProfScope ps(ctx, GNNB_K_LAYER_FWD, nodes, st);
-                tc_fused(g, ctx->plan_fwd[k - 1], ctx->mu[k - 1], false, in.lb[k], in.ub[k], ctx->relax_f[k], ctx->amb_base[k],
+                tc_fused(g, PF(k - 1), PFL(k - 1), ctx->d_guard, ctx->mu[k - 1], false, in.lb[k], in.ub[k], ctx->relax_f[k], ctx->amb_base[k],
                          ctx->mu[k], nullptr, M(k), 0, 0, rows, ctx->d_nan, nd, ctx->snapshot ? ctx->nb : nullptr, false, st, lc);
             } else {
                 ProfScope ps(ctx, GNNB_K_PROP_FWD, nodes, st);
@@ -384,7 +496,7 @@
         }
         {
             ProfScope ps(ctx, GNNB_K_OUTPUT, Bc, st);
-            output_node(g, in.wp, in.bp, ctx->mu[L], tc, tc ? ctx->rowmap[L].nslots : ctx->n[L], in.lb[L + 1], in.ub[L + 1], in.pout,
+            output_node(g, in.wp, in.bp, ctx->mu[L], tc, tc ? maps[L].nslots : ctx->n[L], in.lb[L + 1], in.ub[L + 1], in.pout,
                         ctx->mu[L + 1], ctx->n[L], Bc, st, lc);
         }
         TRY(snap(ctx, snaps, name("t%d_mu_out", t, 0), ctx->mu[L + 1], (int64_t)Bc * P, st));
@@ -395,11 +507,11 @@
             const bool fused_k = fused && k < L;
             if (fused_k) {
                 ProfScope ps(ctx, last ? GNNB_K_LAYER_BWD_SCORE : GNNB_K_LAYER_BWD, nodes, st);
-                tc_fused(g, ctx->plan_bwd[k], ctx->mu[k + 1], true, in.lb[k], in.ub[k], ctx->relax_b[k], ctx->amb_base[k],
+                tc_fused(g, PB(k), PBL(k), ctx->d_guard, ctx->mu[k + 1], true, in.lb[k], in.ub[k], ctx->relax_b[k], ctx->amb_base[k],
                          mu_k, sc, M(k), ctx->n_hidden, ctx->hidden_off[k], rows, ctx->d_nan, nd, ctx->snapshot ? ctx->nb : nullptr, false, st, lc);
             } else {
                 ProfScope ps(ctx, GNNB_K_PROP_BWD, nodes, st);
-                if (k == L && tc) prop_tc_property_backward(in.wp, ctx->mu[L + 1], ctx->nb, ctx->n[L], ctx->rowmap[L].nslots, Bc, st, lc);
+                if (k == L && tc) prop_tc_property_backward(in.wp, ctx->mu[L + 1], ctx->nb, ctx->n[L], maps[L].nslots, Bc, st, lc);
                 else if (k == L) prop_property_backward(in.wp, ctx->mu[L + 1], ctx->nb, ctx->n[L], Bc, st, lc);
                 else if (tc) prop_tc_run(ctx->plan_bwd[k], ctx->mu[k + 1], ctx->nb, Bc, st, lc);
                 else prop_backward(ctx->layers[k], ctx->mu[k + 1], ctx->nb, Bc, true, st, lc);
@@ -414,7 +526,7 @@
         }
         if (!last && fused) {
             ProfScope ps(ctx, GNNB_K_INPUT_UPDATE, (int64_t)Bc * ctx->n[0], st);
-            tc_fused(g, ctx->plan_bwd[0], ctx->mu[1], true, in.lb[0], in.ub[0], nullptr, nullptr, ctx->mu[0], nullptr, M(0), 0, 0, R(0),
+            tc_fused(g, PB(0), PBL(0), ctx->d_guard, ctx->mu[1], true, in.lb[0], in.ub[0], nullptr, nullptr, ctx->mu[0], nullptr, M(0), 0, 0, R(0),
                      ctx->d_nan, nd, nullptr, true, st, lc);
             TRY(snap_img(ctx, snaps, name("t%d_mu0", t, 0), ctx->mu[0], 0, Bc, false, st));
         } else if (!last) {
@@ -697,6 +809,10 @@
     for (PropPlan* p : ctx->plan_fwd) prop_plan_free(p);
     for (PropPlan* p : ctx->plan_bwd) prop_plan_free(p);
     for (PropPlan* p : ctx->plan_kw_own) prop_plan_free(p);
+    free_spec(ctx);
+    if (ctx->d_guard) cudaFree(ctx->d_guard);
+    if (ctx->h_guard) cudaFreeHost(ctx->h_guard);
+    if (ctx->ev_guard) cudaEventDestroy(ctx->ev_guard);
     if (ctx->copy_stream) cudaStreamDestroy(ctx->copy_stream);
     if (ctx->res_best) cudaFree(ctx->res_best);
     if (ctx->res_idx) cudaFree(ctx->res_idx);
@@ -820,11 +936,11 @@
         }
     }
     for (int k = 0; k < n_layers; ++k) {
-        sg.plan_fwd[k] = prop_plan_build(devs[k], layers[k].weight, false, false, tiling[k + 1], tiling[k]);
-        sg.plan_bwd[k] = prop_plan_build(devs[k], layers[k].weight, true, k > 0, tiling[k], tiling[k + 1]);
+        sg.plan_fwd[k] = prop_plan_build(devs[k], layers[k].weight, false, false, tiling[k + 1], tiling[k], tiling[k + 1], tiling[k]);
+        sg.plan_bwd[k] = prop_plan_build(devs[k], layers[k].weight, true, k > 0, tiling[k], tiling[k + 1], tiling[k], tiling[k + 1]);
         if (!sg.plan_fwd[k] || !sg.plan_bwd[k]) return fail(ctx, GNNB_ERR_CUDA, "building the propagation plans failed");
         if (k > 0 && devs[k].kind == GNNB_LAYER_CONV) {
-            sg.plan_kw_own[k] = prop_plan_build(devs[k], layers[k].weight, true, false, tiling[k], tiling[k + 1]);
+            sg.plan_kw_own[k] = prop_plan_build(devs[k], layers[k].weight, true, false, tiling[k], tiling[k + 1], tiling[k], tiling[k + 1]);
             if (!sg.plan_kw_own[k]) return fail(ctx, GNNB_ERR_CUDA, "building the propagation plans failed");
         }
     }
@@ -849,6 +965,9 @@
     for (PropPlan* p : ctx->plan_fwd) prop_plan_free(p);
     for (PropPlan* p : ctx->plan_bwd) prop_plan_free(p);
     for (PropPlan* p : ctx->plan_kw_own) prop_plan_free(p);
+    if (ctx->d_guard) cudaFree(ctx->d_guard);
+    if (ctx->h_guard) cudaFreeHost(ctx->h_guard);
+    ctx->d_guard = nullptr; ctx->h_guard = nullptr; ctx->guard_cap = 0;
     sg.keep = true;
     ctx->d_net = sg.d_net; ctx->d_maps = sg.d_maps; ctx->d_layers = sg.d_layers; ctx->d_hidden_off = sg.d_hidden_off;
     ctx->d_random_order = sg.d_random_order; ctx->d_ptrs = sg.d_ptrs;
@@ -856,6 +975,10 @@
     ctx->plan_kw.assign(n_layers, nullptr);
     for (int k = 0; k < n_layers; ++k) ctx->plan_kw[k] = sg.plan_kw_own[k] ? sg.plan_kw_own[k] : sg.plan_bwd[k];
     ctx->tiling = tiling; ctx->rowmap = rowmap;
+    free_spec(ctx);
+    ctx->rb_gen = -2;
+    ctx->host_net = std::move(blob);
+    ctx->host_w_off = o_w;
     ctx->layers = devs;
     ctx->n = n;
     ctx->zero_tap_layer = first_zero_tap_layer(devs);
@@ -899,6 +1022,11 @@
     if (k == "profile") return ctx->profile;
     if (k == "rescore") return ctx->rescore;
     if (k == "rescored") return ctx->rescored;
+    if (k == "specialised") {
+        if (ctx->rb_gen < 0) return 0;
+        if (cudaEventSynchronize(ctx->ev_guard) != cudaSuccess) return -1;
+        return ctx->rb_waves - ctx->h_guard[0];
+    }
     if (k == "n_hidden") return ctx->n_hidden;
     if (k == "workspace_domains") return ctx->ws_cap;
     if (k.rfind("plan_density_pct_", 0) == 0) {
@@ -927,6 +1055,23 @@
     if (chunk > in->B) chunk = in->B;
     const bool resc = ctx->rescore && ctx->math == GNNB_MATH_TC_FP16X3;
     TRY(ensure_workspace(ctx, chunk, host || resc));
+    const bool guard = guarded(ctx);
+    const int n_guard = guard ? ctx->hidden_off[ctx->layers.size()] : 0;
+    if (guard) {
+        if (ctx->guard_cap < n_guard) {
+            CU(cudaDeviceSynchronize());
+            if (ctx->d_guard) cudaFree(ctx->d_guard);
+            if (ctx->h_guard) cudaFreeHost(ctx->h_guard);
+            ctx->d_guard = nullptr; ctx->h_guard = nullptr; ctx->guard_cap = 0; ctx->rb_gen = -2;
+            CU(cudaMalloc(&ctx->d_guard, (2 + (size_t)n_guard) * sizeof(int32_t)));
+            CU(cudaMallocHost(&ctx->h_guard, (1 + (size_t)n_guard) * sizeof(int32_t)));
+            if (!ctx->ev_guard) CU(cudaEventCreateWithFlags(&ctx->ev_guard, cudaEventDisableTiming));
+            ctx->guard_cap = n_guard;
+        }
+        CU(cudaMemsetAsync(ctx->d_guard + 1, 0, sizeof(int32_t), st));
+        CU(cudaMemsetAsync(ctx->d_guard + 2, 1, (size_t)n_guard * sizeof(int32_t), st));
+    }
+    const int64_t gen = ctx->spec ? ctx->spec_gen : -1;
     NanDoms nd{nullptr, nullptr, nullptr, 0};
     if (resc) {
         TRY(ensure_nan_doms(ctx, in->B));
@@ -993,6 +1138,19 @@
             reset_nan_doms(ctx, st);
             return rc;
         }
+    }
+    if (guard) {
+        if (ctx->rb_gen >= -1 && cudaEventQuery(ctx->ev_guard) == cudaSuccess &&
+            (!ctx->spec || (ctx->rb_gen == ctx->spec_gen && ctx->h_guard[0] > 0))) {
+            std::vector<uint8_t> dead(n_guard);
+            for (int i = 0; i < n_guard; ++i) dead[i] = ctx->h_guard[1 + i] != 0 && (!ctx->spec || ctx->spec->dead[i]);
+            if (ctx->spec) CU(cudaStreamSynchronize(st));
+            build_spec(ctx, dead);
+        }
+        CU(cudaMemcpyAsync(ctx->h_guard, ctx->d_guard + 1, (1 + (size_t)n_guard) * sizeof(int32_t), cudaMemcpyDeviceToHost, st));
+        CU(cudaEventRecord(ctx->ev_guard, st));
+        ctx->rb_gen = gen;
+        ctx->rb_waves = gen >= 0 ? wave : 0;
     }
     if (host) {
         if (!winners) {
diff --git a/gnn_branching_b200/csrc/gnnb_common.cuh b/gnn_branching_b200/csrc/gnnb_common.cuh
--- a/gnn_branching_b200/csrc/gnnb_common.cuh
+++ b/gnn_branching_b200/csrc/gnnb_common.cuh
@@ -66,6 +66,7 @@
     int ntiles = 0;
 };
 LayerTiling make_tiling(int C, int H, int W);
+void make_live_tiling(int C, int H, int W, const uint8_t* dead, LayerTiling* full, LayerTiling* live);
 
 struct NodeInputs {
     const float* lb;
@@ -105,10 +106,10 @@
                const int32_t* amb_base, float* mu_out, float* scores, RowMap map, int64_t score_stride, int64_t score_off, int64_t rows,
                unsigned long long* nan_count, const NanDoms& nan_doms, cudaStream_t st, int64_t* launches);
 struct PropPlan;
-void tc_fused(const GnnParams& g, const PropPlan* plan, const float* mu_in, bool backward, const float* lb, const float* ub,
-              const float* relax, const int32_t* amb_base, float* mu_out, float* scores, RowMap map, int64_t score_stride, int64_t score_off,
-              int64_t rows, unsigned long long* nan_count, const NanDoms& nan_doms, float* nb_dbg, bool input_layer, cudaStream_t st,
-              int64_t* launches);
+void tc_fused(const GnnParams& g, const PropPlan* plan, const PropPlan* plan_live, const int32_t* guard, const float* mu_in, bool backward,
+              const float* lb, const float* ub, const float* relax, const int32_t* amb_base, float* mu_out, float* scores, RowMap map,
+              int64_t score_stride, int64_t score_off, int64_t rows, unsigned long long* nan_count, const NanDoms& nan_doms, float* nb_dbg,
+              bool input_layer, cudaStream_t st, int64_t* launches);
 void amb_compact(const float* lb, const float* ub, RowMap map, int64_t rows, int32_t* cnt, int32_t* amb_base, int32_t* amb_rows,
                  cudaStream_t st, int64_t* launches);
 constexpr int AMB_MAX_LAYERS = 16;
@@ -124,6 +125,20 @@
     int n;
 };
 void amb_compact_all(AmbLayers a, cudaStream_t st, int64_t* launches);
+struct DeadGuard {
+    GnnParams g;
+    const float* lb[AMB_MAX_LAYERS];
+    const float* ub[AMB_MAX_LAYERS];
+    int off[AMB_MAX_LAYERS + 1];
+    int nl, Bc, per_y;
+    const uint8_t* dead;
+    int32_t* acc;
+    int32_t* guard;
+    int32_t* failed;
+    float* scores;
+    int64_t score_stride;
+};
+void tc_dead_guard(const DeadGuard& dg, cudaStream_t st, int64_t* launches);
 void tc_input_embed(const GnnParams& g, const float* lb0, const float* x, const float* ub0, float* mu0, RowMap map, int64_t rows,
                     cudaStream_t st, int64_t* launches);
 void tc_input_update(const GnnParams& g, const float* lb0, const float* ub0, const float* nb, float* mu0, RowMap map, int64_t rows,
@@ -159,7 +174,7 @@
 struct PropPlan;
 int prop_tc_init();
 PropPlan* prop_plan_build(const LayerDev& L, const float* host_weight, bool backward, bool normalise, const LayerTiling& out,
-                          const LayerTiling& in);
+                          const LayerTiling& in, const LayerTiling& ref_out, const LayerTiling& ref_in);
 void prop_plan_free(PropPlan* p);
 double prop_plan_density(const PropPlan* p);
 void prop_tc_run(const PropPlan* plan, const float* mu_in, float* nb_img, int Bc, cudaStream_t st, int64_t* launches);
diff --git a/gnn_branching_b200/csrc/gnnb_prop_tc.cu b/gnn_branching_b200/csrc/gnnb_prop_tc.cu
--- a/gnn_branching_b200/csrc/gnnb_prop_tc.cu
+++ b/gnn_branching_b200/csrc/gnnb_prop_tc.cu
@@ -289,35 +289,71 @@
     return tiles;
 }
 
-PropPlan* build_plan(const LayerTiling& out, const LayerTiling& in, const EdgeFn& edges) {
+PropPlan* build_plan(const LayerTiling& out, const LayerTiling& in, const EdgeFn& edges, const LayerTiling& ref_out,
+                     const LayerTiling& ref_in) {
     std::vector<int32_t> tile_ks0, ks_rows;
     std::vector<uint16_t> ks_w;
     std::vector<Edge> ev;
     std::vector<float> dense;
     double useful = 0.0, issued = 0.0;
+    std::map<int, std::vector<int>> lay_node;
+    std::map<int, std::map<int, int>> lay_pos;
+    auto layout = [&](int R) {
+        if (lay_node.count(R)) return;
+        std::map<int, int> col;
+        for (int m = 0; m < TILE; ++m) {
+            const int node = ref_out.node_of_slot[(size_t)R * TILE + m];
+            if (node < 0) continue;
+            ev.clear();
+            edges(node, ev);
+            for (const Edge& e : ev) col[ref_in.slot_of_node[e.in]] = e.in;
+        }
+        std::vector<int>& nodes = lay_node[R];
+        std::map<int, int>& pos = lay_pos[R];
+        for (const auto& kv : col) { pos[kv.second] = (int)nodes.size(); nodes.push_back(kv.second); }
+    };
     for (int t = 0; t < out.ntiles; ++t) {
         const int32_t* rows = &out.node_of_slot[(size_t)t * TILE];
         std::vector<std::vector<Edge>> row_edges(TILE);
-        std::map<int, int> col;
+        std::vector<int> ref_of_row(TILE, -1), refs;
         for (int m = 0; m < TILE; ++m) {
             if (rows[m] < 0) continue;
-            ev.clear();
-            edges(rows[m], ev);
-            for (Edge& e : ev) { e.in = in.slot_of_node[e.in]; col[e.in] = 0; }
-            row_edges[m] = ev;
-            useful += (double)ev.size();
-        }
-        int K = 0;
-        for (auto& kv : col) kv.second = K++;
+            const int R = ref_out.slot_of_node[rows[m]] / TILE;
+            ref_of_row[m] = R;
+            if (std::find(refs.begin(), refs.end(), R) == refs.end()) { refs.push_back(R); layout(R); }
+            edges(rows[m], row_edges[m]);
+        }
+        std::map<std::pair<int, int>, int> step_of;
+        std::vector<std::pair<int, int>> steps;
+        for (int R : refs) {
+            std::vector<char> used((lay_node[R].size() + 15) / 16, 0);
+            for (int m = 0; m < TILE; ++m)
+                if (ref_of_row[m] == R)
+                    for (const Edge& e : row_edges[m])
+                        if (in.slot_of_node[e.in] >= 0) { used[lay_pos[R][e.in] / 16] = 1; useful += 1.0; }
+            for (int j = 0; j < (int)used.size(); ++j)
+                if (used[j]) { step_of[{R, j}] = (int)steps.size(); steps.push_back({R, j}); }
+        }
+        const int nks = std::max(1, (int)steps.size());
+        const int K = nks * 16;
         dense.assign((size_t)TILE * K, 0.f);
         for (int m = 0; m < TILE; ++m)
-            for (const Edge& e : row_edges[m]) dense[(size_t)m * K + col[e.in]] += e.w;
-        const int nks = std::max(1, (K + 15) / 16);
+            for (const Edge& e : row_edges[m]) {
+                const int pos = lay_pos[ref_of_row[m]][e.in];
+                const auto it = step_of.find({ref_of_row[m], pos / 16});
+                if (it != step_of.end()) dense[(size_t)m * K + it->second * 16 + pos % 16] += e.w;
+            }
         issued += 128.0 * 16.0 * nks;
         tile_ks0.push_back((int32_t)(ks_rows.size() / 16));
         const size_t r0 = ks_rows.size(), w0 = ks_w.size();
-        ks_rows.resize(r0 + (size_t)nks * 16, -1);
-        for (const auto& kv : col) ks_rows[r0 + kv.second] = kv.first;
+        ks_rows.resize(r0 + (size_t)K, -1);
+        for (size_t s = 0; s < steps.size(); ++s) {
+            const std::vector<int>& nodes = lay_node[steps[s].first];
+            for (int q = 0; q < 16; ++q) {
+                const size_t k = (size_t)steps[s].second * 16 + q;
+                if (k < nodes.size()) ks_rows[r0 + s * 16 + q] = in.slot_of_node[nodes[k]];
+            }
+        }
         ks_w.resize(w0 + (size_t)nks * 4096, 0);
         for (int m = 0; m < TILE; ++m)
             for (int k = 0; k < K; ++k) {
@@ -357,14 +393,11 @@
     return p;
 }
 
-}
-
-LayerTiling make_tiling(int C, int H, int W) {
-    const std::vector<std::vector<int>> tiles = (H == 1 && W == 1) ? range_tiles(C) : grid_tiles(C, H, W);
+LayerTiling tiling_of(const std::vector<std::vector<int>>& tiles, int n) {
     LayerTiling t;
     t.ntiles = (int)tiles.size();
     t.node_of_slot.assign((size_t)t.ntiles * TILE, -1);
-    t.slot_of_node.assign((size_t)C * H * W, -1);
+    t.slot_of_node.assign((size_t)n, -1);
     for (int i = 0; i < t.ntiles; ++i)
         for (size_t m = 0; m < tiles[i].size(); ++m) {
             t.node_of_slot[(size_t)i * TILE + m] = tiles[i][m];
@@ -373,12 +406,37 @@
     return t;
 }
 
+std::vector<std::vector<int>> layer_tiles(int C, int H, int W) { return (H == 1 && W == 1) ? range_tiles(C) : grid_tiles(C, H, W); }
+
+}
+
+LayerTiling make_tiling(int C, int H, int W) { return tiling_of(layer_tiles(C, H, W), C * H * W); }
+
+void make_live_tiling(int C, int H, int W, const uint8_t* dead, LayerTiling* full, LayerTiling* live) {
+    std::vector<int> order[2];
+    for (const std::vector<int>& t : layer_tiles(C, H, W))
+        for (int node : t) order[dead[node] ? 1 : 0].push_back(node);
+    std::vector<std::vector<int>> tiles;
+    int nlive = 0;
+    for (int d = 0; d < 2; ++d) {
+        for (size_t r0 = 0; r0 < order[d].size(); r0 += TILE)
+            tiles.emplace_back(order[d].begin() + r0, order[d].begin() + std::min(order[d].size(), r0 + TILE));
+        if (d == 0) nlive = (int)tiles.size();
+    }
+    if (nlive == 0) nlive = 1;
+    *full = tiling_of(tiles, C * H * W);
+    *live = *full;
+    live->ntiles = nlive;
+    for (int node = 0; node < C * H * W; ++node)
+        if (dead[node]) live->slot_of_node[node] = -1;
+}
+
 int prop_tc_init() {
     return cudaFuncSetAttribute(k_tc_prop, cudaFuncAttributeMaxDynamicSharedMemorySize, (int)prop::PROP_SMEM);
 }
 
 PropPlan* prop_plan_build(const LayerDev& L, const float* w, bool backward, bool normalise, const LayerTiling& out,
-                          const LayerTiling& in) {
+                          const LayerTiling& in, const LayerTiling& ref_out, const LayerTiling& ref_in) {
     const int k = L.ksize, s = L.stride, p = L.pad;
     if (L.kind == GNNB_LAYER_CONV) {
         const int hw_in = L.h_in * L.w_in, hw_out = L.h_out * L.w_out;
@@ -396,7 +454,7 @@
                         }
                     }
             };
-            return build_plan(out, in, f);
+            return build_plan(out, in, f, ref_out, ref_in);
         }
         EdgeFn f = [=](int node, std::vector<Edge>& ev) {
             const int ci = node / hw_in, yi = (node % hw_in) / L.w_in, xi = node % L.w_in;
@@ -416,18 +474,18 @@
             if (normalise && taps > 0)
                 for (size_t i = first; i < ev.size(); ++i) ev[i].w = ev[i].w / (float)taps;
         };
-        return build_plan(out, in, f);
+        return build_plan(out, in, f, ref_out, ref_in);
     }
     if (!backward) {
         EdgeFn f = [=](int node, std::vector<Edge>& ev) {
             for (int i = 0; i < L.n_in; ++i) ev.push_back({i, w[(size_t)node * L.n_in + i]});
         };
-        return build_plan(out, in, f);
+        return build_plan(out, in, f, ref_out, ref_in);
     }
     EdgeFn f = [=](int node, std::vector<Edge>& ev) {
         for (int o = 0; o < L.n_out; ++o) ev.push_back({o, w[(size_t)o * L.n_in + node]});
     };
-    return build_plan(out, in, f);
+    return build_plan(out, in, f, ref_out, ref_in);
 }
 
 void prop_plan_free(PropPlan* p) {
diff --git a/gnn_branching_b200/csrc/gnnb_tc.cu b/gnn_branching_b200/csrc/gnnb_tc.cu
--- a/gnn_branching_b200/csrc/gnnb_tc.cu
+++ b/gnn_branching_b200/csrc/gnnb_tc.cu
@@ -495,6 +495,8 @@
 struct FusedArgs {
     UpdArgs u;
     PropPlanDev plan;
+    PropPlanDev plan_live;
+    const int32_t* guard;
     const uint16_t* mu_in;
     uint16_t* nb_dbg;
     int n_stages;
@@ -619,7 +621,6 @@
     using namespace fz;
     const UpdArgs& a = fa.u;
     const GnnParams& g = a.g;
-    const PropPlanDev& plan = fa.plan;
     const bool with_score = a.scores != nullptr;
     const uint32_t wbytes = with_score ? UPD_WBYTES : UPD_FN;
     const int NS = fa.n_stages;
@@ -669,19 +670,22 @@
     __syncthreads();
     pdl_trigger(); pdl_wait();
 
-    const int ntiles = plan.ntiles, npairs = (a.Bc + PD - 1) / PD;
+    const bool live = fa.guard != nullptr && *fa.guard == 0;
+#define PLAN(f) (live ? fa.plan_live.f : fa.plan.f)
+    const int ntiles = PLAN(ntiles), npairs = (a.Bc + PD - 1) / PD;
+#define TSTRIDE (a.map.nslots >> 7)
     const int rank = (int)blockIdx.x, nranks = (int)gridDim.x;
 
     if (warp == 0) {
         if (lane == 0) {
             uint32_t slot = 0, ph = 0;
             for (ItemCursor cur(rank, nranks, ntiles, npairs); cur.valid(); cur.next()) {
-                const int ks0 = plan.tile_ks0[cur.tile], ks1 = plan.tile_ks0[cur.tile + 1];
+                const int ks0 = PLAN(tile_ks0)[cur.tile], ks1 = PLAN(tile_ks0)[cur.tile + 1];
                 for (int ks = ks0; ks < ks1; ++ks) {
                     mbar_wait(smem_u32(&tl->empty[slot]), ph ^ 1u);
                     const uint32_t full = smem_u32(&tl->full[slot]);
                     mbar_expect_tx(full, W_KS);
-                    bulk_g2s(ring + slot * STAGE, plan.ks_w + (size_t)ks * (W_KS / 2), W_KS, full);
+                    bulk_g2s(ring + slot * STAGE, PLAN(ks_w) + (size_t)ks * (W_KS / 2), W_KS, full);
                     if (++slot == (uint32_t)NS) { slot = 0; ph ^= 1u; }
                 }
             }
@@ -703,7 +707,7 @@
 #define FTR_END(x)
 #endif
         for (ItemCursor cur(rank, nranks, ntiles, npairs); cur.valid(); cur.next(), ++it) {
-            const int ks0 = uniform(plan.tile_ks0[cur.tile]), ks1 = uniform(plan.tile_ks0[cur.tile + 1]);
+            const int ks0 = uniform(PLAN(tile_ks0)[cur.tile]), ks1 = uniform(PLAN(tile_ks0)[cur.tile + 1]);
             const uint32_t buf = it & 1u, bufph = (it >> 1) & 1u;
             FTR_BEGIN();
             mbar_wait(smem_u32(&tl->acc_empty[buf]), bufph ^ 1u);
@@ -755,19 +759,19 @@
         uint32_t slot = 0, ph = 0;
         int turn = 0;
         for (ItemCursor cur(rank, nranks, ntiles, npairs); cur.valid(); cur.next()) {
-            const int ks0 = __ldg(plan.tile_ks0 + cur.tile), ks1 = __ldg(plan.tile_ks0 + cur.tile + 1);
+            const int ks0 = __ldg(PLAN(tile_ks0) + cur.tile), ks1 = __ldg(PLAN(tile_ks0) + cur.tile + 1);
             const int dm0 = cur.pair * PD;
             const uint32_t jp = (uint32_t)(lane & 7);
-            const unsigned char* base0 = mu_bytes + (int64_t)dm0 * (plan.nslots_in >> 7) * (int64_t)ABUF + jp * 16u;
+            const unsigned char* base0 = mu_bytes + (int64_t)dm0 * (PLAN(nslots_in) >> 7) * (int64_t)ABUF + jp * 16u;
             const uint32_t sz0 = dm0 < a.Bc ? 16u : 0u, sz1 = dm0 + 1 < a.Bc ? 16u : 0u;
-            const unsigned char* base1 = sz1 ? base0 + (int64_t)(plan.nslots_in >> 7) * (int64_t)ABUF : base0;
+            const unsigned char* base1 = sz1 ? base0 + (int64_t)(PLAN(nslots_in) >> 7) * (int64_t)ABUF : base0;
             for (int ks = ks0; ks < ks1; ++ks) {
                 const uint32_t slot_ = slot, ph_ = ph;
                 const bool mine = turn == gw;
                 if (++slot == (uint32_t)NS) { slot = 0; ph ^= 1u; }
                 if (++turn == GW) turn = 0;
                 if (!mine) continue;
-                const int idx = __ldg(plan.ks_rows + (size_t)ks * 16 + (lane & 15));
+                const int idx = __ldg(PLAN(ks_rows) + (size_t)ks * 16 + (lane & 15));
                 const int off = idx < 0 ? -1 : (idx << 7) + ((idx >> 7) << 14);
 #ifdef GNNB_TRACE
                 const long long g0_ = clock64();
@@ -839,7 +843,7 @@
             const int d_ = cu.pair * PD + j;
             if (d_ >= a.Bc) return;
             if (node_ >= 0) { l_n = ldg1_now(lb + (int64_t)d_ * map.n + node_); u_n = ldg1_now(ub + (int64_t)d_ * map.n + node_); }
-            if (amb_base != nullptr) slot0_n = ldgi_now(amb_base + (int64_t)d_ * ntiles + cu.tile);
+            if (amb_base != nullptr) slot0_n = ldgi_now(amb_base + (int64_t)d_ * TSTRIDE + cu.tile);
         };
         ItemCursor cur(rank, nranks, ntiles, npairs), cur1 = cur, cur2 = cur;
         cur1.next();
@@ -869,7 +873,7 @@
                 if (h == 0 && c.t == 0) mbar_arrive(smem_u32(&tl->acc_empty[buf]));
                 return false;
             }
-            const int64_t tile = (int64_t)dom_ * ntiles + cu.tile;
+            const int64_t tile = (int64_t)dom_ * TSTRIDE + cu.tile;
             c.acol = ACC_COL + buf * ACC_WIN + 64u * (uint32_t)j;
             {
                 unsigned char* dbg = fa.nb_dbg ? reinterpret_cast<unsigned char*>(fa.nb_dbg) + tile * (int64_t)ABUF + (uint32_t)c.t * 16u : nullptr;
@@ -940,7 +944,7 @@
                 advance();
                 continue;
             }
-            const int64_t tile = (int64_t)dom * ntiles + cur.tile;
+            const int64_t tile = (int64_t)dom * TSTRIDE + cur.tile;
 #ifdef GNNB_TRACE
             c0_ = clock64(); ++c_tiles;
 #endif
@@ -1084,6 +1088,9 @@
     __syncthreads();
     if (warp == 0) tmem_dealloc(tmem_base, 512);
 }
+
+#undef PLAN
+#undef TSTRIDE
 
 __global__ void __launch_bounds__(fz::THREADS, 1) k_tc_fused(FusedArgs fa) { fused_body<false>(fa); }
 __global__ void __launch_bounds__(fz::THREADS, 1) k_tc_fused_input(FusedArgs fa) { fused_body<true>(fa); }
@@ -1441,6 +1448,36 @@
 }
 
 namespace {
+__global__ void __launch_bounds__(256) k_dead_guard(DeadGuard dg) {
+    __shared__ float zscore;
+    if (threadIdx.x == 0 && dg.dead != nullptr) {
+        const float* bf = dg.g.bias[FNODE];
+        const float* wf = dg.g.wt[FSCORE];
+        float half[2] = {0.f, 0.f};
+        for (int h = 0; h < 2; ++h)
+            for (int i = 32 * h; i < 32 * h + 32; ++i) half[h] = fmaf(relu_nan(0.f + bf[i] * ASCALE), wf[i] * 1.0f, half[h]);
+        zscore = fmaf(half[0] + half[1], AINV, dg.g.bias[FSCORE][0]);
+    }
+    __syncthreads();
+    const int h = blockIdx.x * blockDim.x + threadIdx.x;
+    if (h >= dg.off[dg.nl]) return;
+    int k = 0;
+    while (h >= dg.off[k + 1]) ++k;
+    const int node = h - dg.off[k], n = dg.off[k + 1] - dg.off[k];
+    const bool dead = dg.dead != nullptr && dg.dead[h] != 0;
+    bool live = false;
+    const int b1 = min(dg.Bc, (int)(blockIdx.y + 1) * dg.per_y);
+    for (int b = blockIdx.y * dg.per_y; b < b1; ++b) {
+        const Ratio q = compute_ratio(__ldg(dg.lb[k] + (int64_t)b * n + node), __ldg(dg.ub[k] + (int64_t)b * n + node));
+        live |= !(q.r0 == 0.0f);
+        if (dead) dg.scores[(int64_t)b * dg.score_stride + h] = zscore;
+    }
+    if (live) {
+        dg.acc[h] = 0;
+        if (dead && atomicExch(dg.guard, 1) == 0) atomicAdd(dg.failed, 1);
+    }
+}
+
 UpdArgs make_upd_args(const GnnParams& g, bool backward, const float* lb, const float* ub, const float* nb, const float* relax,
                       const int32_t* amb_base, float* mu_out, float* scores, RowMap map, int64_t score_stride, int64_t score_off,
                       int64_t rows, unsigned long long* nan_count, const NanDoms& nan_doms) {
@@ -1463,22 +1500,24 @@
     ++*launches;
 }
 
-void tc_fused(const GnnParams& g, const PropPlan* plan, const float* mu_in, bool backward, const float* lb, const float* ub,
-              const float* relax, const int32_t* amb_base, float* mu_out, float* scores, RowMap map, int64_t score_stride, int64_t score_off,
-              int64_t rows, unsigned long long* nan_count, const NanDoms& nan_doms, float* nb_dbg, bool input_layer, cudaStream_t st,
-              int64_t* launches) {
+void tc_fused(const GnnParams& g, const PropPlan* plan, const PropPlan* plan_live, const int32_t* guard, const float* mu_in, bool backward,
+              const float* lb, const float* ub, const float* relax, const int32_t* amb_base, float* mu_out, float* scores, RowMap map,
+              int64_t score_stride, int64_t score_off, int64_t rows, unsigned long long* nan_count, const NanDoms& nan_doms, float* nb_dbg,
+              bool input_layer, cudaStream_t st, int64_t* launches) {
     FusedArgs fa;
     fa.input_layer = input_layer ? 1 : 0;
     fa.u = make_upd_args(g, backward, lb, ub, nullptr, relax, amb_base, mu_out, scores, map, score_stride, score_off, rows, nan_count,
                          nan_doms);
     fa.plan = prop_plan_dev(plan);
+    fa.plan_live = prop_plan_dev(plan_live ? plan_live : plan);
+    fa.guard = plan_live ? guard : nullptr;
     fa.mu_in = reinterpret_cast<const uint16_t*>(mu_in);
     fa.nb_dbg = reinterpret_cast<uint16_t*>(nb_dbg);
     const uint32_t wbytes = scores ? UPD_WBYTES : UPD_FN;
     const int staging = mu_out == nullptr ? 0 : (scores ? 1 : 2);
     const int ns = (int)((fz::SMEM_MAX - fz::smem_for(wbytes, staging, 0)) / fz::STAGE);
     fa.n_stages = ns > fz::NS_MAX ? fz::NS_MAX : ns;
-    fa.mma_group = prop_plan_ksteps_per_tile(plan) >= 48.0 ? 4 : 2;
+    fa.mma_group = prop_plan_ksteps_per_tile(plan_live ? plan_live : plan) >= 48.0 ? 4 : 2;
     if (fa.mma_group > fa.n_stages / 2) fa.mma_group = fa.n_stages / 2;
     const int64_t nitems = (int64_t)fa.plan.ntiles * ((fa.u.Bc + fz::PD - 1) / fz::PD);
     launch_pdl(input_layer ? k_tc_fused_input : k_tc_fused, (int)(nitems < 1 ? 1 : (nitems < 148 ? nitems : 148)), fz::THREADS,
@@ -1486,6 +1525,15 @@
     ++*launches;
 }
 
+void tc_dead_guard(const DeadGuard& dg, cudaStream_t st, int64_t* launches) {
+    const int per_y = 16;
+    DeadGuard a = dg;
+    a.per_y = per_y;
+    const dim3 grid((unsigned)((dg.off[dg.nl] + 255) / 256), (unsigned)((dg.Bc + per_y - 1) / per_y));
+    k_dead_guard<<<grid, 256, 0, st>>>(a);
+    ++*launches;
+}
+
 void tc_input_embed(const GnnParams& g, const float* lb0, const float* x, const float* ub0, float* mu0, RowMap map, int64_t rows,
                     cudaStream_t st, int64_t* launches) {
     launch_pdl(k_tc_input_embed, grid_for(rows), 128 * NWG, smem_bytes(EMB_WBYTES, true), st, g, lb0, x, ub0, reinterpret_cast<uint16_t*>(mu0), map, rows);
```

New measurement: 99280, median of 6. 63.8% lower.
